# transferia/transferia

Hardware: AMD Instinct MI355X
Metric: ChangeItems/sec through CSV parse -> mask(ClientIP)+filter(EventDate) -> devnull, ClickBench hits, HBM-resident input (the PCIe-inclusive rate is `pcie_inclusive`) (higher is better)
Workload: dtype u8; 1 GPU; ClickBench hits-1M CSV parse -> mask(ip)+filter(EventDate) -> devnull (BASELINE.json configs[1]); columns=105, parallelism=row-range shard x1, no collective, rows_per_pass=1048576, csv_bytes_per_pass=838371857

## Files before the change

transferia_amd/csrc/tf_common.hpp:

```cpp
#pragma once
#include <hip/hip_runtime.h>

#include <cstdint>
#include <cstdio>
#include <cstring>
#include <memory>
#include <mutex>
#include <unordered_map>
#include <stdexcept>
#include <string>
#include <vector>

#include "../../include/tfgpu.h"

#ifndef TF_DYNAMIC_LDS
#define TF_DYNAMIC_LDS(type, name) extern __shared__ type name[]
#endif

#ifndef TF_GLOBAL_PTR
#define TF_GLOBAL_PTR(T, p) ((T *)(__attribute__((address_space(1))) T *)(p))
#endif

#ifndef TF_LOAD16_STREAM
__device__ __forceinline__ uint4 tf_load16_stream(const void *p) {
  typedef uint32_t v4u __attribute__((ext_vector_type(4)));
  const v4u t = __builtin_nontemporal_load(reinterpret_cast<const v4u *>(p));
  return make_uint4(t[0], t[1], t[2], t[3]);
}
#define TF_LOAD16_STREAM(p) tf_load16_stream(p)
#endif

#ifndef TF_CONST_PTR
#define TF_CONST_PTR(T, p) ((const __attribute__((address_space(4))) T *)(p))
#endif

#ifndef TF_KEEP
#define TF_KEEP(x) asm volatile("" ::"v"(x))
#endif
#ifndef TF_OPAQUE
#define TF_OPAQUE(x) asm volatile("" : "+v"(x))
#endif

struct tfgpu_dbatch;

namespace tf {

struct Error : std::runtime_error {
  int code;
  Error(int c, const std::string &m) : std::runtime_error(m), code(c) {}
};
void set_last_error(const std::string &m);
int fail(int code, const std::string &m);

#define TF_HIP(expr)                                                                              \
  do {                                                                                            \
    hipError_t e__ = (expr);                                                                      \
    if (e__ != hipSuccess)                                                                        \
      throw ::tf::Error(TFGPU_ERR_DEVICE, std::string(#expr) + ": " + hipGetErrorString(e__));    \
  } while (0)

struct ProfEntry {
  std::string name;
  int64_t launches = 0;
  double total_ms = 0;
  int64_t units = 0;
};

struct BlockCache {
  std::mutex mu;
  std::unordered_map<size_t, std::vector<void *>> free_;
  size_t cached = 0;
  void *get(size_t cls);
  void put(void *p, size_t cls);
  void trim();
};

struct Context {
  int device = -1;
  hipStream_t stream = nullptr;
  hipStream_t copy_stream = nullptr;
  BlockCache blocks;
  void *pin_base = nullptr;
  size_t pin_cap = 0, pin_off = 0;
  void *pin(size_t bytes);
  template <class T> T *pin_n(size_t n) { return reinterpret_cast<T *>(pin(n * sizeof(T))); }
  bool prof_on = false;
  std::vector<ProfEntry> prof;
  struct Pending { int idx; hipEvent_t a, b; int64_t units = 0; };
  std::vector<Pending> pending;
  std::vector<hipEvent_t> free_events;
  hipEvent_t dense_event = nullptr;
  std::mutex mu;
  int num_cus = 256;
  std::shared_ptr<struct DevMem> pow10tab;
  struct ConstEntry { uint64_t hash; std::vector<uint8_t> bytes; std::shared_ptr<struct DevMem> mem; uint64_t stamp; };
  std::vector<ConstEntry> consts;
  uint64_t const_clock = 0;
  double csv_hint_bpl = 0.0;
  int csv_hint_ncols = -1;

  hipEvent_t get_event();
  void prof_begin(const char *name, Pending &p);
  void prof_end(Pending &p);
  void prof_flush();
};
Context &ctx();
int bind_lane(int lane);
int current_lane();
int lane_device(int lane);
struct LaneScope {
  int prev;
  explicit LaneScope(int lane) : prev(bind_lane(lane)) {}
  ~LaneScope() { try { bind_lane(prev); } catch (...) {} }
};

struct KernelTimer {
  Context::Pending p{-1, nullptr, nullptr};
  bool on;
  explicit KernelTimer(const char *name, int64_t units = 0) : on(ctx().prof_on) { if (on) { ctx().prof_begin(name, p); p.units = units; } }
  ~KernelTimer() { if (on) ctx().prof_end(p); }
};

struct DevMem {
  void *p = nullptr;
  size_t bytes = 0, cls = 0;
  std::shared_ptr<DevMem> parent;
  struct BlockCache *owner = nullptr;
  int device = -1;
  explicit DevMem(size_t n);
  DevMem(std::shared_ptr<DevMem> owner, size_t off, size_t n);
  ~DevMem();
  DevMem(const DevMem &) = delete;
  DevMem &operator=(const DevMem &) = delete;
};
using Buf = std::shared_ptr<DevMem>;
Buf dalloc(size_t bytes);
Buf subbuf(const Buf &owner, size_t off, size_t bytes);
Buf dalloc_zero(size_t bytes);
template <class T> inline T *ptr(const Buf &b) { return b ? reinterpret_cast<T *>(b->p) : nullptr; }

void h2d(void *dst, const void *src, size_t n);
void h2d_small(void *dst, const void *src, size_t n);
Buf upload_small(const void *src, size_t n);
void dbatch_drop_src_row(struct ::tfgpu_dbatch *b);
Buf upload_const(const void *src, size_t n);
const uint32_t *d2h_u32(const void *dev, size_t n = 1);
struct PinScope { PinScope() {} };
void d2h(void *dst, const void *src, size_t n);
void d2d(void *dst, const void *src, size_t n);
void sync();

inline bool repr_is_var(int r) { return r == TFGPU_R_STRING || r == TFGPU_R_BYTES || r == TFGPU_R_JSONNUM || r == TFGPU_R_JSON; }
// ... 34 lines not shown
void ensure_text_offsets(const struct ::tfgpu_dbatch &b);
void dense(const struct ::tfgpu_dbatch *b, bool absent_ok = false);
void dense_locked(const struct ::tfgpu_dbatch &b);
int lanes_created();
uint64_t lane_generation();
std::unique_ptr<struct ::tfgpu_dbatch> snapshot(const struct ::tfgpu_dbatch &b);
bool has_absent(const struct ::tfgpu_dbatch &b);
Buf validity_minus_absent(const Buf &validity, const Buf &absent, int64_t nrows);
Buf find_device_block(const void *p);
void register_device_block(const Buf &b);

}

namespace tf {
struct PendingRows {
  std::shared_ptr<const struct ::tfgpu_dbatch> src;
  Buf sel;
};
}

struct tfgpu_dbatch {
  int64_t nrows = 0;
  std::vector<tf::DColumn> cols;
  std::shared_ptr<tf::PendingRows> pending;
  void *dense_done = nullptr;
  int dense_lane = -1;
  uint64_t dense_gen = 0;
  std::vector<tf::DColumn> replaced;
  std::vector<std::pair<std::string, int>> schema;
  std::vector<std::string> key_names;
  std::vector<tf::DColumn> old_keys;
  tf::Buf old_present;
  std::string ns, table;
  tf::Buf kind, src_row, part_id;
  tf::Buf col_order;
};

struct tfgpu_dbuf {
  tf::Buf mem;
  uint64_t size = 0;
};

namespace tf {
inline std::unique_ptr<tfgpu_dbatch> shallow_copy(const tfgpu_dbatch &in) { return std::make_unique<tfgpu_dbatch>(in); }
template <class F> void materialize_where(const tfgpu_dbatch &b, F pred) {
  std::vector<const DColumn *> need;
  for (auto &c : b.cols) if (pred(c)) need.push_back(&c);
  materialize(b, &need);
}
void exclusive_scan_u32(const uint32_t *in, uint32_t *out, int64_t n, bool with_total);
void exclusive_scan_u32_segments(uint32_t *inout, int64_t seg_len, int nseg, int64_t seg_stride);
void exclusive_scan_u32_segments(const uint32_t *in, uint32_t *out, int64_t seg_len, int nseg, int64_t seg_stride);
bool select_kept_u32(const uint32_t *keep, int64_t n, int32_t *sel, uint32_t *count);
const uint32_t *any_nonzero_to_host(const uint32_t *v, int64_t n);
const uint32_t *segment_totals_to_host(const uint32_t *scanned, int64_t seg_len, int nseg, int64_t seg_stride);
void sum_u32_segments_u64(const uint32_t *in, int64_t seg_len, int nseg, int64_t seg_stride, unsigned long long *totals);

}
```

transferia_amd/csrc/tf_csv.hip:

```cpp
#include <algorithm>
#include <cmath>
#include <cstdio>
#include <type_traits>

#include "tf_devfmt.hpp"
#include "tf_devparse.hpp"
#include "tf_devfloat.hpp"
#include "tf_segcopy.hpp"
#include "tf_textview.hpp"
#include "tf_wave.hpp"
#include "tf_swar.hpp"
#include "tf_gotime.hpp"
#include "tf_f64range.hpp"
#include "tf_plan.hpp"
#include "tf_strictcell.hpp"

#ifdef TF_CSV_ABLATE_BUILD
#define CSV_ABL(x) ((x).ablate)
#else
#define CSV_ABL(x) 0
#endif
namespace tf {

std::unique_ptr<tfgpu_dbatch> compact_rows(const tfgpu_dbatch &in, Buf keep);
// ... 74 lines not shown
  const int lane = threadIdx.x & 63, wv = threadIdx.x >> 6;
  for (int it = 0; it < NL_ITERS; it++) {
    uint64_t pos = tile + ((uint64_t)it * NL_THREADS + threadIdx.x) * 16;
    uint32_t m = pos < len ? nl_mask16(load16_guard(data, pos, len)) : 0;
    uint32_t c = __popc(m), inc = c;
    for (int d = 1; d < 64; d <<= 1) { uint32_t t = __shfl_up(inc, d, 64); if (lane >= d) inc += t; }
    if (lane == 63) wsum[wv] = inc;
    __syncthreads();
    uint32_t wbase = 0, tot = 0;
    for (int i = 0; i < NL_THREADS / 64; i++) { uint32_t s = wsum[i]; if (i < wv) wbase += s; tot += s; }
    __syncthreads();
    uint32_t k = base + wbase + inc - c;
    while (m) { int b = __ffs(m) - 1; m &= m - 1; row_start[++k] = (uint32_t)(pos + b + 1); }
    base += tot;
  }
}


template <class F> __device__ __forceinline__ uint32_t space_prefix(const F &f, uint32_t i, uint32_t end) {
  uint32_t c = f[i];
  if (c == ' ' || (c >= 9 && c <= 13)) return 1;
  if (c < 0xC2) return 0;
  uint32_t r = end - i;
  if (c == 0xC2 && r >= 2) { uint32_t d = f[i + 1]; return (d == 0x85 || d == 0xA0) ? 2 : 0; }
  if (r >= 3 && (c == 0xE1 || c == 0xE2 || c == 0xE3)) {
    uint32_t d = f[i + 1], e = f[i + 2];
    if (c == 0xE1) return (d == 0x9A && e == 0x80) ? 3 : 0;
    if (c == 0xE3) return (d == 0x80 && e == 0x80) ? 3 : 0;
    if (d == 0x80 && ((e >= 0x80 && e <= 0x8A) || e == 0xA8 || e == 0xA9 || e == 0xAF)) return 3;
    if (d == 0x81 && e == 0x9F) return 3;
  }
  return 0;
}
template <class F> __device__ __forceinline__ uint32_t space_suffix(const F &f, uint32_t a, uint32_t b) {
  uint32_t c = f[b - 1];
  if (c == ' ' || (c >= 9 && c <= 13)) return 1;
  if (c < 0x80) return 0;
  if (b - a >= 2 && f[b - 2] == 0xC2 && (c == 0x85 || c == 0xA0)) return 2;
  if (b - a >= 3 && space_prefix(f, b - 3, b) == 3) return 3;
  return 0;
}

struct CsvOpts {
  uint8_t delim, quote, escape, double_quote, include_missing, strings_can_be_null, quoted_strings_can_be_null, pad;
  int32_t n_null, n_true, n_false;
  const uint32_t *list_off;
  const uint8_t *list_data;
  GtSet user_tp;
  GtSet cast_tp;
  const uint8_t *dp;
  uint32_t dp_len;
  uint32_t multiline;
  const uint64_t *p128;
};

__device__ __forceinline__ bool any_quote(const uint32_t *qmask, uint32_t lo, uint32_t hi) {
  if (lo >= hi) return false;
  const uint32_t w0 = lo >> 5, w1 = (hi - 1) >> 5;
  for (uint32_t w = w0; w <= w1; w++) {
    uint32_t m = qmask[w];
    if (w == w0) m &= ~0u << (lo & 31);
    if (w == w1) m &= ~0u >> (31 - ((hi - 1) & 31));
    if (m) return true;
  }
  return false;
}

template <class F> __device__ __forceinline__ int sanitize(const CsvOpts &o, const F &f, uint32_t &a, uint32_t &b, uint32_t &npairs,
                                                           const uint32_t *qmask = nullptr, uint32_t qbase = 0) {
  a = 0; b = f.n; npairs = 0;
  uint32_t k;
  while (a < b && (k = space_prefix(f, a, b)) > 0) a += k;
  while (a < b && (k = space_suffix(f, a, b)) > 0) b -= k;
  if (o.quote == 0) return 0;
  if (b - a >= 1) {
    if (b - a == 1 && f[a] == o.quote) return TFGPU_ROW_QUOTE;
    if (f[a] == o.quote && f[b - 1] == o.quote) { a++; b--; }
  }
  if (qmask && !any_quote(qmask, qbase + a, qbase + b)) return 0;
  for (uint32_t i = a; i + 1 < b;) {
    if (f[i] == o.quote && f[i + 1] == o.quote) { npairs++; i += 2; } else i++;
  }
  if (!o.double_quote && npairs) return TFGPU_ROW_DOUBLE_QUOTE;
  return 0;
}

template <class F> __device__ __forceinline__ bool field_equals(const F &f, uint32_t a, uint32_t b, const uint8_t *s, uint32_t n) {
  if (b - a != n) return false;
  for (uint32_t i = 0; i < n; i++) if (f[a + i] != s[i]) return false;
  return true;
}
template <class F> __device__ __forceinline__ bool in_list(const CsvOpts &o, int first, int count, const F &f, uint32_t a, uint32_t b) {
  for (int i = 0; i < count; i++) {
    uint32_t s = o.list_off[first + i], e = o.list_off[first + i + 1];
    if (field_equals(f, a, b, o.list_data + s, e - s)) return true;
  }
  return false;
}

enum CsvKind : int32_t { CK_INT = SK_INT, CK_UINT = SK_UINT, CK_STR = SK_STR, CK_JSONNUM = SK_JSONNUM, CK_DATE = SK_TIME, CK_TIMESTAMP, CK_BOOL = SK_BOOL, CK_F32 = SK_F32, CK_DEFAULT,
                         CK_INTERVAL = SK_INTERVAL, CK_SYS  };
static_assert(CK_TIMESTAMP == 5 && CK_DEFAULT == 8 && CK_SYS == 10, "the tile kernels sort columns by these values");

struct CsvCol {
  int32_t field;
  int32_t kind;
  int32_t width;
  int32_t next;
  int64_t lo; uint64_t hi;
  void *values;
  int32_t *nanos;
  uint32_t *lens;
  uint32_t *fstart;
  uint32_t *patch;
};
static constexpr uint32_t PATCH_NONE = 0xFFFFFFFFu;

struct TCol {
  void *p0;
  void *p1;
  int16_t field;
  uint8_t kind;
  uint8_t width;
  int32_t ci;
};
static_assert(sizeof(TCol) == 24, "TCol is staged as three 8-byte words");

struct CsvParams {
  const uint8_t *data;
  uint64_t len;
  const uint32_t *row_start;
  const uint32_t *row_end;
  int64_t nrows;
  CsvOpts o;
  const CsvCol *cols;
  int32_t ncols;
  const int32_t *field_first;
  int32_t nfields_used;
  int32_t has_unmapped;
  const TCol *tcols;
  unsigned long long *dbg_phase;
  int32_t null_checks;
  uint8_t *err;
  int32_t *err_col;
  uint32_t *nerr;
  const uint32_t *gran_pre;
  int64_t ngran;
  uint32_t tile_bytes;
  int64_t ntiles;
  int64_t skip_rows;
  uint32_t *slow_n;
  uint32_t *slow_row;
  uint32_t *slow_end;
  uint32_t *last_end;
  int32_t ablate;
  uint32_t *gen_n;
  uint32_t *gen_tile;
  int32_t force_general;
  const struct CsvRun *runs;
  int32_t nruns;
  const struct CsvTask *tasks;
  const int32_t *wave_task;
  int32_t col_lanes;
  uint8_t *arena;
  const uint32_t *lcols;
  const uint32_t *lwave_ncols;
  uint32_t tile_cpt;
  uint32_t *spec;
  uint32_t cap_lines;
  uint32_t *ovf;
};

static constexpr uint32_t SP_AGG = 1u << 30, SP_INC = 2u << 30, SP_VAL = (1u << 30) - 1u;
__device__ __forceinline__ uint32_t spec_lookback(uint32_t *state, int64_t t, uint32_t own, int lane) {
  if (t == 0) { if (lane == 0) __atomic_store_n(&state[0], SP_INC | own, __ATOMIC_RELAXED); return 0u; }
  if (lane == 0) __atomic_store_n(&state[t], SP_AGG | own, __ATOMIC_RELAXED);
  uint32_t excl = 0;
  int64_t base = t - 1;
  for (;;) {
    const int64_t idx = base - lane;
    const uint32_t w = idx >= 0 ? __atomic_load_n(&state[idx], __ATOMIC_RELAXED) : SP_INC;
    const uint64_t inc = __ballot((w >> 30) == 2u), empty = __ballot((w >> 30) == 0u);
    const int fi = inc ? __ffsll((long long)inc) - 1 : 63;
    const uint64_t need = fi == 63 ? ~0ull : ((2ull << fi) - 1ull);
    if (empty & need) { __builtin_amdgcn_s_sleep(1); continue; }
    uint32_t v = lane <= fi ? (w & SP_VAL) : 0u;
    v = wave_scan_add(v);
    excl += (uint32_t)__shfl((int)v, 63, 64);
    if (inc) break;
    base -= 64;
  }
  if (lane == 0) __atomic_store_n(&state[t], SP_INC | ((excl + own) & SP_VAL), __ATOMIC_RELAXED);
  return excl;
}

__device__ __forceinline__ StrictOut strict_out(const CsvCol &c, int32_t kind) { return StrictOut{kind, c.width, c.lo, c.hi, c.values, c.nanos}; }
__device__ __forceinline__ void store_int(const CsvCol &c, int64_t r, int64_t v) { store_int(strict_out(c, c.kind), r, v); }

__device__ __forceinline__ void store_default(const CsvCol &c, int64_t r) {
  switch (c.kind) {
    case CK_SYS: break;
    case CK_STR: case CK_JSONNUM: c.lens[r] = (c.kind == CK_JSONNUM) ? 1u : 0u; c.fstart[r] = 0x7FFFFFFFu; if (c.kind == CK_JSONNUM) c.fstart[-1] = 1u; break;
    case CK_DATE: case CK_TIMESTAMP: store_default(strict_out(c, SK_TIME), r); break;
    default: store_default(strict_out(c, c.kind), r);
  }
}

template <class F>
__device__ __forceinline__ bool cell_is_null(const CsvOpts &o, const F &fv, uint32_t a, uint32_t b, uint32_t npairs) {
  if (o.quoted_strings_can_be_null) {
    uint32_t ta = a, tb = b;
    if (tb > ta && ((fv[ta] == '"' && fv[tb - 1] == '"') || (fv[ta] == '\'' && fv[tb - 1] == '\''))) { ta++; tb = tb > ta ? tb - 1 : ta; }
    return npairs == 0 && in_list(o, 0, o.n_null, fv, ta, tb);
  }
  if (o.strings_can_be_null) return npairs == 0 && in_list(o, 0, o.n_null, fv, a, b);
  return false;
}

template <class F> struct Patched {
  const F &f; uint32_t a, k, skip;
  __device__ __forceinline__ uint32_t operator[](uint32_t i) const { return i < k ? f[a + i] : i == k ? (uint32_t)'.' : f[a + i + skip - 1]; }
};
template <class T> __device__ int parsefloat_err(const T &t, uint32_t n) {
  if (n == 0) return 1;
  uint32_t p = 0;
  if (t[0] == '+' || t[0] == '-') p = 1;
  const uint32_t w = n - p;
  auto word = [&](const char *s, uint32_t l) { if (w != l) return false; for (uint32_t i = 0; i < l; i++) if (lower_(t[p + i]) != (uint32_t)s[i]) return false; return true; };
  if (word("inf", 3) || word("infinity", 8)) return 0;
  if (p == 0 && word("nan", 3)) return 0;
  for (uint32_t i = p; i < n; i++) if (t[i] == '_') return 2;
  if (w >= 2 && t[p] == '0' && lower_(t[p + 1]) == 'x') return 2;
  uint32_t nd = 0;
  while (p < n && dg(t[p])) { nd++; p++; }
  if (p < n && t[p] == '.') { p++; while (p < n && dg(t[p])) { nd++; p++; } }
  if (!nd) return 1;
  if (p < n && lower_(t[p]) == 'e') {
    p++;
    if (p < n && (t[p] == '+' || t[p] == '-')) p++;
    if (p >= n || !dg(t[p])) return 1;
    while (p < n && dg(t[p])) p++;
  }
  if (p != n) return 1;
  return jsonnum_overflow(t, n) ? 1 : 0;
}

template <class F>
__device__ int parse_cell(const CsvOpts &o, const CsvCol &c, int64_t r, const F &fv, uint32_t a, uint32_t b, uint32_t npairs, uint64_t abs_start) {
  switch (c.kind) {
    case CK_INT: case CK_UINT: case CK_INTERVAL:
      if (cell_is_null(o, fv, a, b, npairs)) { store_default(c, r); return 0; }
      if (npairs) return TFGPU_ROW_CAST;
      return strict_cell(strict_out(c, c.kind), o.cast_tp, o.p128, r, fv, a, b);
    case CK_STR: case CK_JSONNUM: {
      if (c.kind == CK_STR && cell_is_null(o, fv, a, b, npairs)) { c.lens[r] = 0; c.fstart[r] = 0x7FFFFFFFu; return 0; }
      if (c.kind == CK_JSONNUM && o.dp_len && !npairs && b - a >= o.dp_len) {
        uint32_t k = PATCH_NONE;
        for (uint32_t i = a; i + o.dp_len <= b && k == PATCH_NONE; i++) {
          bool eq = true;
          for (uint32_t j = 0; j < o.dp_len && eq; j++) eq = fv[i + j] == o.dp[j];
          if (eq) k = i - a;
        }
        if (k != PATCH_NONE) {
          const Patched<F> pt{fv, a, k, o.dp_len};
          const uint32_t pn = (b - a) - o.dp_len + 1;
          const int pe = parsefloat_err(pt, pn);
          if (pe == 2) return TFGPU_ROW_HOST_FALLBACK;
          if (pe == 0) {
            struct View { const Patched<F> &t; __device__ uint32_t operator[](uint32_t i) const { return t[i]; } } v{pt};
            if (!json_number_ok(v, 0, pn)) return TFGPU_ROW_CAST;
            c.lens[r] = pn; c.fstart[r] = (uint32_t)(abs_start + a); c.patch[r] = k;
            return 0;
          }
        }
      }
      if (c.kind == CK_JSONNUM && (npairs || !json_number_ok(fv, a, b))) return TFGPU_ROW_CAST;
      c.lens[r] = (b - a) - npairs;
      c.fstart[r] = (uint32_t)(abs_start + a) | (npairs ? 0x80000000u : 0u);
      if (npairs) c.fstart[-1] = 1u;
      return 0;
    }
    case CK_DATE: case CK_TIMESTAMP: {
      if (npairs) return TFGPU_ROW_CAST;
      int64_t sec = 0; int32_t ns = 0;
      if (c.kind == CK_TIMESTAMP ? parse_int64(fv, a, b, false, &sec) == 0
                                 : (o.user_tp.n && gotime_parse_any(o.user_tp, fv, a, b, &sec, &ns))) {
        ((int64_t *)c.values)[r] = sec;
        c.nanos[r] = ns;
        return 0;
      }
      return strict_cell(strict_out(c, SK_TIME), o.cast_tp, o.p128, r, fv, a, b);
    }
    case CK_BOOL: {
      int v;
      if (npairs) return TFGPU_ROW_CAST;
      if (o.strings_can_be_null && in_list(o, 0, o.n_null, fv, a, b)) v = 0;
      else if (in_list(o, o.n_null, o.n_true, fv, a, b)) v = 1;
      else if (in_list(o, o.n_null + o.n_true, o.n_false, fv, a, b)) v = 0;
      else return strict_cell(strict_out(c, c.kind), o.cast_tp, o.p128, r, fv, a, b);
      ((uint8_t *)c.values)[r] = (uint8_t)v;
      return 0;
    }
    case CK_F32: {
      if (npairs) return TFGPU_ROW_CAST;
      if (o.dp_len && b - a >= o.dp_len) {
        uint32_t k = PATCH_NONE;
        for (uint32_t i = a; i + o.dp_len <= b && k == PATCH_NONE; i++) {
          bool eq = true;
          for (uint32_t j = 0; j < o.dp_len && eq; j++) eq = fv[i + j] == o.dp[j];
          if (eq) k = i - a;
        }
        if (k != PATCH_NONE) {
          const Patched<F> pt{fv, a, k, o.dp_len};
          const uint32_t pn = (b - a) - o.dp_len + 1;
          const int pe = parsefloat_err(pt, pn);
          if (pe == 2) return TFGPU_ROW_HOST_FALLBACK;
          if (pe == 0) return strict_cell(strict_out(c, c.kind), o.cast_tp, o.p128, r, pt, 0, pn);
        }
      }
      return strict_cell(strict_out(c, c.kind), o.cast_tp, o.p128, r, fv, a, b);
    }
    default:
      return TFGPU_ROW_HOST_FALLBACK;
  }
}

__device__ void parse_line_hbm(const CsvParams &p, const bool have_row, const int64_t r, uint64_t pos, const uint64_t end ) {
  const uint64_t row0 = pos;
  MemBytes scan(p.data), fld(p.data);
  const CsvOpts &o = p.o;
  int rerr = 0, rerr_col = -1, miss_col = 0x7FFFFFFF, cerr = 0, cerr_col = 0x7FFFFFFF;
  const bool nil_line = have_row && (end - pos) <= 1;
  if (have_row && o.quote == 0) {
    for (uint64_t q = pos; q < end; q++) if (scan.at(q) == '"') { rerr = TFGPU_ROW_QUOTING_DISABLED; rerr_col = -1; break; }
  }
  if (have_row && o.multiline) {
    for (uint64_t q = pos; q + 2 < end; q++) if (scan.at(q) == '\n' && scan.at(q + 1) == '\n') { rerr = TFGPU_ROW_HOST_FALLBACK; rerr_col = -1; break; }
  }
  bool active = have_row && !nil_line;
  bool in_quotes = false; uint32_t prev = 0xFFFFFFFFu;
  int32_t nfields = 0;
  bool seen_delim = false;
  for (int32_t f = 0;; f++) {
    uint64_t fs = pos, fe = pos; bool last = false;
    if (active) {
      while (true) {
        if (pos >= end) { last = true; fe = end; break; }
        uint32_t ch = scan.at(pos);
        if (o.escape != 0 && prev == o.escape && in_quotes) { prev = ch; pos++; continue; }
        if (o.quote != 0 && ch == o.quote) { in_quotes = !in_quotes; prev = ch; pos++; continue; }
        if (ch == o.delim && !in_quotes) { fe = pos; pos++; seen_delim = true; prev = ch; break; }
        prev = ch; pos++;
      }
      if (last && !seen_delim) fs = row0 + 1 <= end ? row0 + 1 : end;
    }
    const bool has_field = active;
    if (!__any(has_field) && f >= p.nfields_used) break;
    Field fv{&fld, fs, (uint32_t)(fe - fs)};
    uint32_t a = 0, b = 0, npairs = 0;
    const int32_t first_col = f < p.nfields_used ? p.field_first[f] : -1;
    if (has_field) {
      int e = sanitize(o, fv, a, b, npairs);
      if (e && !rerr) { rerr = e; rerr_col = first_col; }
      nfields = f + 1;
    }
    for (int32_t ci = first_col; ci >= 0; ci = p.cols[ci].next) {
      const CsvCol &c = p.cols[ci];
      if (!have_row || rerr) continue;
      if (!has_field) {
        if (o.include_missing) store_default(c, r); else if (ci < miss_col) miss_col = ci;
        continue;
      }
      int err = parse_cell(o, c, r, fv, a, b, npairs, fs);
      if (err && ci < cerr_col) { cerr = err; cerr_col = ci; }
    }
    if (last) active = false;
  }
  if (!have_row) return;
  if (!rerr) {
    for (int32_t ci = 0; ci < p.ncols; ci++) {
      const CsvCol &c = p.cols[ci];
      if (c.field < 0) { store_default(c, r); continue; }
      if (c.field >= nfields) {
        if (c.field < p.nfields_used && !nil_line) continue;
        if (o.include_missing) store_default(c, r); else { if (ci < miss_col) miss_col = ci; break; }
      }
    }
  }
  int err = rerr, err_col = rerr_col;
  if (!err && miss_col != 0x7FFFFFFF) { err = TFGPU_ROW_MISSING_CELL; err_col = miss_col; }
  if (!err && cerr) { err = cerr; err_col = cerr_col; }
  p.err[r] = (uint8_t)err;
  if (err) { p.err_col[r] = err_col; atomicAdd(p.nerr, 1u); }
}

__global__ void __launch_bounds__(256) csv_parse_rows(CsvParams p) {
  const int64_t r = (int64_t)blockIdx.x * blockDim.x + threadIdx.x;
  const bool have_row = r < p.nrows;
  parse_line_hbm(p, have_row, r, have_row ? p.row_start[r] : 0, have_row ? (p.row_end ? p.row_end[r] : p.row_start[r + 1]) : 0);
}

__global__ void __launch_bounds__(64) csv_parse_listed(CsvParams p) {
  const uint32_t n = *p.slow_n;
  for (uint64_t base = (uint64_t)blockIdx.x * 64; base < n; base += (uint64_t)gridDim.x * 64) {
    const uint64_t i = base + threadIdx.x;
    const int64_t line = i < n ? (int64_t)p.slow_row[i] : -1;
    const bool have_row = i < n && line >= p.skip_rows;
    uint64_t end = 0, pos = 0;
    if (have_row) {
      end = (uint64_t)p.slow_end[i] + 1;
      pos = end - 1;
      MemBytes back(p.data);
      while (pos > 0 && back.at(pos - 1) != '\n') pos--;
    }
    parse_line_hbm(p, have_row, line - p.skip_rows, pos, end);
  }
}

#ifndef TF_CT_THREADS
#define TF_CT_THREADS 512
#endif
static constexpr int CT_THREADS = TF_CT_THREADS;
static constexpr uint32_t CT_WAVES = CT_THREADS / 64;
static_assert((CT_WAVES & (CT_WAVES - 1)) == 0, "wave count must be a power of two");
static constexpr int CT_T = NL_TILE;
static constexpr int CT_SPILL = 4096;
static constexpr int CT_BYTES = CT_T + CT_SPILL;
static constexpr int CT_CPT = CT_BYTES / 16 / CT_THREADS;
static constexpr int CT_FCAP = 4096;
static constexpr int CT_RCAP = 256;
static constexpr int CT_LCOLS = 192;
static_assert(CT_CPT * 16 * CT_THREADS == CT_BYTES, "tile must divide evenly");
static_assert(CT_BYTES <= 32768, "positions are 15-bit");

__device__ __forceinline__ bool starts_plain(const uint8_t *sb, uint32_t a, uint32_t end, uint32_t c, uint32_t quote) {
  if (c < 0x80) return c > 0x20 && c != 0x7F && c != quote;
  if (c != 0xC2 && c != 0xE1 && c != 0xE2 && c != 0xE3) return true;
  const uint32_t d = a + 1 < end ? sb[a + 1] : 0u, e = a + 2 < end ? sb[a + 2] : 0u;
  if (c == 0xC2) return !(d == 0x85 || d == 0xA0);
  if (c == 0xE1) return !(d == 0x9A && e == 0x80);
  if (c == 0xE3) return !(d == 0x80 && e == 0x80);
  return !((d == 0x80 && ((e >= 0x80 && e <= 0x8A) || e == 0xA8 || e == 0xA9 || e == 0xAF)) || (d == 0x81 && e == 0x9F));
}
__device__ __forceinline__ bool ends_plain(const uint8_t *sb, uint32_t a, uint32_t b, uint32_t c, uint32_t quote) {
  if (c < 0x80) return c > 0x20 && c != 0x7F && c != quote;
  if (c >= 0xC0) return true;
  const uint32_t d = b - a >= 2 ? sb[b - 2] : 0u, e = b - a >= 3 ? sb[b - 3] : 0u;
  if (d == 0xC2) return !(c == 0x85 || c == 0xA0);
  if (e == 0xE1) return !(d == 0x9A && c == 0x80);
  if (e == 0xE3) return !(d == 0x80 && c == 0x80);
  if (e == 0xE2) return !((d == 0x80 && ((c >= 0x80 && c <= 0x8A) || c == 0xA8 || c == 0xA9 || c == 0xAF)) || (d == 0x81 && c == 0x9F));
  return true;
}
__device__ __forceinline__ uint32_t count_quote_pairs(const uint32_t *qmask, uint32_t lo, uint32_t hi) {
  if (lo >= hi) return 0;
  uint32_t pairs = 0, prev = 0xFFFFFFF0u;
// ... 239 lines not shown
        }
      }
    }
    for (uint32_t i = tid; i < nr; i += CT_THREADS) slowf[i] = 0;
    __syncthreads();
    }
    if (CSV_ABL(p) == 3) { if (fpos[tid] == 0xFFFF && rowend[0] == 0xFFFF) p.err[0] = 1; return; }

    uint32_t next_bstart;
    if (skip_first) {
      uint32_t k = k_thread;
#pragma unroll
      for (int q = 0; q < CT_CPT; q++) {
        uint32_t m = fe[q];
        const int cpos = (base_chunk + q) * 16;
        while (m) {
          const int b = __ffs((int)m) - 1; m &= m - 1;
          if (k == kend) {
            fpos[0] = (uint16_t)(cpos + b);
            uint32_t slot = atomicAdd(p.slow_n, 1u);
            p.slow_row[slot] = line0 + jb;
            p.slow_end[slot] = (uint32_t)(g0 + cpos + b);
          }
          k++;
        }
      }
      __syncthreads();
      next_bstart = (uint32_t)fpos[0] + 1;
    } else {
      for (uint32_t jj = tid; jj < nr; jj += CT_THREADS) {
        const uint32_t k0 = jj ? (uint32_t)rowend[jj - 1] + 1 : kb, ke = rowend[jj];
        const uint32_t row_start = jj ? (uint32_t)(fpos[k0 - 1 - kb] & 0x7FFFu) + 1 : bstart;
        const uint32_t nl_pos = fpos[ke - kb] & 0x7FFFu;
        const uint32_t nf = (nl_pos == row_start) ? 0u : ke - k0 + 1;
        rinfo[jj] = (uint64_t)(k0 - kb) | ((uint64_t)nf << 16) | ((uint64_t)row_start << 32);
      }
      __syncthreads();
      const uint32_t total = (uint32_t)p.ncols * nr;
      const uint32_t inv_nr = nr > 1 ? 0xFFFFFFFFu / nr + 1 : 0;
      for (uint32_t it = tid; it < total; it += CT_THREADS) {
        uint32_t oi = nr > 1 ? __umulhi(it, inv_nr) : it;
        uint32_t jj = it - oi * nr;
        if (jj >= nr) { oi++; jj -= nr; }
        const int64_t r = (int64_t)line0 + jb + jj - p.skip_rows;
        if (r < 0) continue;
        TCol tc;
        if (cols_in_lds) { const uint64_t *q = tcol_lds + oi * 3; tc.p0 = (void *)q[0]; tc.p1 = (void *)q[1]; uint64_t m = q[2]; tc.field = (int16_t)m; tc.kind = (uint8_t)(m >> 16); tc.width = (uint8_t)(m >> 24); tc.ci = (int32_t)(m >> 32); }
        else tc = p.tcols[oi];
        const uint64_t ri = rinfo[jj];
        const uint32_t k0r = (uint32_t)ri & 0xFFFFu, nf = (uint32_t)(ri >> 16) & 0xFFFFu, row_start = (uint32_t)(ri >> 32);
        if (tc.field < 0 || (uint32_t)tc.field >= nf) {
          if (tc.field < 0 || o.include_missing) {
            CsvCol c{}; c.kind = tc.kind; c.width = tc.width; c.values = tc.p0; c.nanos = (int32_t *)tc.p1; c.lens = (uint32_t *)tc.p0; c.fstart = (uint32_t *)tc.p1;
            store_default(c, r);
          } else slowf[jj] = 1;
          continue;
        }
        const uint32_t kr = k0r + (uint32_t)tc.field;
        uint32_t fs = tc.field ? (uint32_t)(fpos[kr - 1] & 0x7FFFu) + 1 : row_start;
        const uint32_t fend = fpos[kr] & 0x7FFFu;
        if (nf == 1) fs = row_start + 1;
        const uint32_t n = fend - fs;
        if (CSV_ABL(p) == 6) { if (n == 0x7FFF) p.err[0] = 1; continue; }
        bool done = false;
        if (n == 0) {
          if (tc.kind == CK_STR) { ((uint32_t *)tc.p0)[r] = 0; ((uint32_t *)tc.p1)[r] = (uint32_t)(g0 + fs); done = true; }
        } else {
          const uint32_t sh = (fs & 7u) * 8;
          const uint64_t *w = reinterpret_cast<const uint64_t *>(sb + (fs & ~7u));
          const uint64_t w0 = w[0], w1 = w[1];
          const uint64_t b0 = sh ? (w0 >> sh) | (w1 << (64 - sh)) : w0;
          const uint32_t c_first = (uint32_t)b0 & 0xFFu, c_last = sb[fend - 1];
          if (tc.kind == CK_STR) {
            uint32_t a = fs, b = fend;
            bool ok = false;
            if (c_first == o.quote && c_last == o.quote && n >= 2) { a++; b--; ok = true; }
            else ok = c_first != o.quote && c_last != o.quote && starts_plain(sb, fs, fend, c_first, o.quote) && ends_plain(sb, fs, fend, c_last, o.quote);
            if (ok) {
              const uint32_t npairs = any_quote(qmask, a, b) ? count_quote_pairs(qmask, a, b) : 0u;
              if (!(npairs && !o.double_quote)) {
                ((uint32_t *)tc.p0)[r] = (b - a) - npairs;
                ((uint32_t *)tc.p1)[r] = (uint32_t)(g0 + a) | (npairs ? 0x80000000u : 0u);
                if (npairs) ((uint32_t *)tc.p1)[-1] = 1u;
                done = true;
              }
            }
          } else if (tc.kind == CK_INT || tc.kind == CK_UINT) {
            if (n <= 20) {
              const bool neg = c_first == '-';
              const uint32_t i0 = (c_first == '-' || c_first == '+') ? 1u : 0u;
              const uint32_t nd = n - i0;
              bool ok = nd >= 1 && nd <= 19 && !(nd > 1 && ((uint32_t)(b0 >> (8 * i0)) & 0xFFu) == '0');
              if (tc.kind == CK_UINT && tc.width == 8 && i0) ok = false;
              uint64_t b1 = 0, b2 = 0;
              if (__any(n > 8)) { const uint64_t w2 = w[2]; b1 = sh ? (w1 >> sh) | (w2 << (64 - sh)) : w1; if (__any(n > 16)) { const uint64_t w3 = w[3]; b2 = sh ? (w2 >> sh) | (w3 << (64 - sh)) : w2; } }
              uint64_t v;
              ok = digits_u64(b0, b1, b2, i0, n, &v) && ok;
              const int bits = tc.width * 8;
              if (tc.kind == CK_INT) ok = ok && v <= (neg ? (1ull << (bits - 1)) : (1ull << (bits - 1)) - 1);
              else ok = ok && !(neg && v != 0) && (tc.width == 8 || v <= (1ull << bits) - 1);
              if (ok && CSV_ABL(p) != 5) {
                const int64_t sv = neg ? (int64_t)(0 - v) : (int64_t)v;
                switch (tc.width) {
                  case 1: ((int8_t *)tc.p0)[r] = (int8_t)sv; break;
                  case 2: ((int16_t *)tc.p0)[r] = (int16_t)sv; break;
                  case 4: ((int32_t *)tc.p0)[r] = (int32_t)sv; break;
                  default: ((int64_t *)tc.p0)[r] = sv;
                }
              }
              done = ok;
            }
          } else if (tc.kind == CK_DATE || tc.kind == CK_TIMESTAMP) {
            const uint64_t w2 = w[2], w3 = w[3];
            const uint64_t b1 = sh ? (w1 >> sh) | (w2 << (64 - sh)) : w1, b2 = sh ? (w2 >> sh) | (w3 << (64 - sh)) : w2;
            const uint32_t i0 = (c_first == '-' || c_first == '+') ? 1u : 0u;
            uint64_t v = 0;
            if (tc.kind == CK_TIMESTAMP && n - i0 >= 1 && n - i0 <= 18 && digits_u64(b0, b1, b2, i0, n, &v)) {
              ((int64_t *)tc.p0)[r] = c_first == '-' ? -(int64_t)v : (int64_t)v; ((int32_t *)tc.p1)[r] = 0; done = true;
            } else if (n == 10 || n == 19) {
              bool ok = true;
              const uint32_t y = two_digits(b0, 0, &ok) * 100 + two_digits(b0, 2, &ok);
              const uint32_t mo = two_digits(b0, 5, &ok), d = two_digits(b1, 0, &ok);
              ok = ok && (((uint32_t)(b0 >> 32) & 0xFFu) == '-') && (((uint32_t)(b0 >> 56) & 0xFFu) == '-');
              uint32_t h = 0, mi = 0, se = 0;
              if (n == 19) {
                const uint32_t sep = (uint32_t)(b1 >> 16) & 0xFFu;
                ok = ok && (sep == ' ' || sep == 'T') && (((uint32_t)(b1 >> 40) & 0xFFu) == ':') && (((uint32_t)b2 & 0xFFu) == ':');
                h = two_digits(b1, 3, &ok); mi = two_digits(b1, 6, &ok); se = two_digits(b2, 1, &ok);
              }
              ok = ok && mo >= 1 && mo <= 12 && d >= 1 && d <= (uint32_t)dev::days_in_month((int)mo, (int64_t)y) && h <= 23 && mi <= 59 && se <= 59;
              if (ok) {
                ((int64_t *)tc.p0)[r] = dev::days_from_civil((int64_t)y, (int)mo, (int)d) * 86400 + h * 3600 + mi * 60 + se;
                ((int32_t *)tc.p1)[r] = 0;
                done = true;
              }
            }
// ... 16 lines not shown
          const uint32_t fend = fpos[kk] & 0x7FFFu;
          if (fend > fs && !(starts_plain(sb, fs, fend, sb[fs], o.quote) && ends_plain(sb, fs, fend, sb[fend - 1], o.quote) && !any_quote(qmask, fs, fend))) slowf[jj] = 1;
        }
      }
      __syncthreads();
      for (uint32_t jj = tid; jj < nr; jj += CT_THREADS) {
        const int64_t r = (int64_t)line0 + jb + jj - p.skip_rows;
        if (r < 0) continue;
        if (slowf[jj] || p.null_checks) {
          const uint32_t slot = atomicAdd(p.slow_n, 1u);
          p.slow_row[slot] = line0 + jb + jj;
          p.slow_end[slot] = (uint32_t)(g0 + (fpos[rowend[jj] - kb] & 0x7FFFu));
        } else p.err[r] = 0;
      }
      next_bstart = (uint32_t)(fpos[kend - kb] & 0x7FFFu) + 1;
    }
    __syncthreads();
    bstart = next_bstart;
    jb += nr; kb = kend + 1;
  }
  if (tid == 0) {
    atomicMax(p.last_end, (uint32_t)(g0 + bstart));
    if (p.spec) p.spec[2 + p.ntiles + gstart / (CT_T / CSV_GRAN)] = (uint32_t)(g0 + bstart);
  }
}

__global__ void __launch_bounds__(CT_THREADS, 6) csv_parse_tiles_general(CsvParams p) {
  const uint32_t n = *p.gen_n;
  for (uint32_t i = blockIdx.x; i < n; i += gridDim.x) {
    const bool sp = p.spec != nullptr;
    const uint32_t *e = p.gen_tile + (size_t)(sp ? 4 : 2) * i;
    parse_tile_general(p, (int64_t)e[0], (int64_t)e[1], sp ? e[2] : 0u, sp ? e[3] : 0u);
    __syncthreads();
  }
}

__device__ __forceinline__ int32_t days_from_civil32(uint32_t y, uint32_t m, uint32_t d) {
  const uint32_t yy = y + 400u - (m <= 2 ? 1u : 0u);
  const uint32_t era = yy / 400u, yoe = yy - era * 400u;
  const uint32_t doy = (153u * (m > 2 ? m - 3 : m + 9) + 2u) / 5u + d - 1u;
  const uint32_t doe = yoe * 365u + yoe / 4u - yoe / 100u + doy;
  return (int32_t)(era * 146097u + doe) - 719468 - 146097;
}
__device__ __forceinline__ uint32_t days_in_month32(uint32_t m, uint32_t y) {
  const uint32_t leap = ((y & 3u) == 0 && (y % 100u != 0 || y % 400u == 0)) ? 1u : 0u;
  return m == 2 ? 28u + leap : 30u + ((0x15AAu >> m) & 1u);
}

#ifndef TF_CR_FCAP
#define TF_CR_FCAP 4608
#endif
static constexpr int CR_FCAP = TF_CR_FCAP;
static constexpr int CR_LCOLS = 128;
static constexpr uint32_t CR_KDUMMY = CR_FCAP + 2;
struct CsvRun { int32_t kind, width, first, ncols; };
struct CsvTask { int32_t kind, width, first, ncols; };

struct RegTile {
  const uint8_t *sb; const uint16_t *fposx; const uint32_t *qmask; const uint16_t *qpre; const uint2 *keeptab; uint8_t *slowf; const uint64_t *colp0, *colp1; const uint16_t *colfield;
  uint32_t nr, NF, step_q, step_r; float inv_nr; int32_t row0; uint32_t g0; uint32_t quote; bool double_quote; int32_t ablate; int32_t col_mode;
};
struct RegCell { bool on; uint32_t col, jj, fs, fend; int32_t r; };
struct ItemIter { uint32_t it, oi, jj; };
__device__ __forceinline__ ItemIter item_first(const RegTile &t, uint32_t it) {
  uint32_t oi = (uint32_t)(__uint2float_rz(it) * t.inv_nr);
  uint32_t jj = it - __umul24(oi, t.nr);
  if (jj >= t.nr) { oi++; jj -= t.nr; }
  return ItemIter{it, oi, jj};
}
__device__ __forceinline__ void item_next(const RegTile &t, ItemIter &x) {
  x.it += 64u * CT_WAVES; x.oi += t.step_q; x.jj += t.step_r;
  if (x.jj >= t.nr) { x.jj -= t.nr; x.oi++; }
}
__device__ __forceinline__ RegCell reg_cell(const RegTile &t, uint32_t first_col, const ItemIter &x, uint32_t items) {
  RegCell c;
  c.col = first_col + x.oi; c.jj = x.jj;
  c.r = t.row0 + (int32_t)x.jj;
  c.on = x.it < items && c.r >= 0;
  const uint32_t kr = c.on ? __umul24(x.jj, t.NF) + (uint32_t)t.colfield[c.col] : CR_KDUMMY;
  uint32_t kr1 = kr + 1;
  TF_OPAQUE(kr1);
  c.fs = (uint32_t)t.fposx[kr] + 1; c.fend = t.fposx[kr1];
  return c;
}
#ifndef TF_CSV_PREFETCH
#define TF_CSV_PREFETCH 0
#endif
template <class Body> __device__ __forceinline__ void for_slots(const RegTile &t, const CsvRun &run, uint32_t sbase, int wv, int lane, Body body) {
  const uint32_t items = (uint32_t)run.ncols * t.nr, nslots = (items + 63) >> 6, end = sbase + nslots;
  const uint32_t s0 = sbase + (((uint32_t)wv - sbase) & (CT_WAVES - 1u));
  if (s0 >= end) return;
  ItemIter x = item_first(t, (s0 - sbase) * 64 + (uint32_t)lane);
#if TF_CSV_PREFETCH
  RegCell c = reg_cell(t, (uint32_t)run.first, x, items);
  for (uint32_t s = s0; s < end; s += CT_WAVES) {
    RegCell cn = c;
    if (s + CT_WAVES < end) { item_next(t, x); cn = reg_cell(t, (uint32_t)run.first, x, items); }
    body(c);
    c = cn;
  }
#else
  for (uint32_t s = s0; s < end; s += CT_WAVES, item_next(t, x)) body(reg_cell(t, (uint32_t)run.first, x, items));
#endif
}
template <class T> __device__ __forceinline__ T *global_ptr(uint64_t p) { return TF_GLOBAL_PTR(T, p); }
__device__ __forceinline__ uint32_t quotes_in(const RegTile &t, uint32_t a, uint32_t b) {
  const uint32_t ca = (uint32_t)t.qpre[a >> 5] + (uint32_t)__popc(t.qmask[a >> 5] & ((1u << (a & 31)) - 1u));
  const uint32_t cb = (uint32_t)t.qpre[b >> 5] + (uint32_t)__popc(t.qmask[b >> 5] & ((1u << (b & 31)) - 1u));
  return cb - ca;
}

template <int KIND, int W, class T> __device__ __forceinline__ void reg_int_body(const RegTile &t, const RegCell &c, T *const out) {
// ... 22 lines not shown
    const uint2 keep = t.keeptab[c.on ? n : 0u];
    const uint32_t tlo = (wlo ^ 0x30303030u) & keep.x, thi = (whi ^ 0x30303030u) & keep.y;
    bad = (((tlo + 0x76767676u) | tlo | (thi + 0x76767676u) | thi) & 0x80808080u) != 0;
    uint32_t v;
    if constexpr (W < 4) {
      v = __umul24(tlo >> 24, 10000u) + four_dot(thi);
      if constexpr (KIND == CK_INT) bad = bad || v > (1u << (W * 8 - 1)) - 1u; else bad = bad || v > (1u << (W * 8)) - 1u;
    } else v = __umul24(four_dot(tlo), 10000u) + four_dot(thi);
    if (c.on && !bad) out[c.r] = (T)v;
  } else if constexpr (W >= 4) {
    const bool neg = c0 == '-', sgn = neg || c0 == '+';
    const uint32_t nd = n - (sgn ? 1u : 0u);
    const uint32_t fd = sgn ? (uint32_t)t.sb[c.fs + 1] : c0;
    bool ok = nd - 1u < 19u && !(nd > 1 && fd == '0');
    if constexpr (KIND == CK_UINT && W == 8) ok = ok && !sgn;
    const uint32_t y = c.fend;
    const uint32_t *w = reinterpret_cast<const uint32_t *>(t.sb + (int)((y - 24u) & ~3u));
    const uint32_t d0 = w[0], d1 = w[1], d2 = w[2], d3 = w[3], d4 = w[4];
    const uint32_t w2lo = __builtin_amdgcn_alignbyte(d1, d0, y), w2hi = __builtin_amdgcn_alignbyte(d2, d1, y);
    const uint32_t w1lo = __builtin_amdgcn_alignbyte(d3, d2, y), w1hi = __builtin_amdgcn_alignbyte(d4, d3, y);
    const uint32_t ndc = min(nd, 24u), n0 = min(ndc, 8u), n1d = min(ndc - n0, 8u), n2d = min(ndc - n0 - n1d, 8u);
    const uint2 k0 = t.keeptab[n0], k1 = t.keeptab[n1d], k2 = t.keeptab[n2d];
    const uint32_t a0 = (wlo ^ 0x30303030u) & k0.x, b0 = (whi ^ 0x30303030u) & k0.y;
    const uint32_t a1 = (w1lo ^ 0x30303030u) & k1.x, b1 = (w1hi ^ 0x30303030u) & k1.y;
    const uint32_t a2 = (w2lo ^ 0x30303030u) & k2.x, b2 = (w2hi ^ 0x30303030u) & k2.y;
    const uint32_t nondigit = ((a0 + 0x76767676u) | a0 | (b0 + 0x76767676u) | b0 | (a1 + 0x76767676u) | a1 | (b1 + 0x76767676u) | b1 |
                               (a2 + 0x76767676u) | a2 | (b2 + 0x76767676u) | b2) & 0x80808080u;
    ok = ok && nondigit == 0;
    const uint32_t g0v = __umul24(four_dot(a0), 10000u) + four_dot(b0), g1v = __umul24(four_dot(a1), 10000u) + four_dot(b1);
    const uint32_t g2v = __umul24(four_dot(a2), 10000u) + four_dot(b2);
    const uint64_t v = ((uint64_t)g2v * 100000000ull + g1v) * 100000000ull + g0v;
    if constexpr (KIND == CK_INT) ok = ok && v <= (neg ? (1ull << (W * 8 - 1)) : (1ull << (W * 8 - 1)) - 1);
    else ok = ok && !(neg && v != 0) && (W == 8 || v <= (1ull << (W * 8 % 64)) - 1);
    if (c.on && ok) out[c.r] = (T)(neg ? (int64_t)(0 - v) : (int64_t)v);
    bad = !ok;
  } else {
    const bool neg = c0 == '-', sgn = neg || c0 == '+';
    const uint32_t nd = n - (sgn ? 1u : 0u);
    bool ok = nd - 1u < 19u && !(nd > 1 && t.sb[c.fend - min(nd, 24u)] == '0');
    uint32_t g0v = 0;
    ok = digits8_window<true>(wlo, whi, min(nd, 8u), &g0v) && ok;
    if constexpr (KIND == CK_INT) ok = ok && nd <= 5 && g0v <= (1u << (W * 8 - 1)) - (neg ? 0u : 1u);
    else ok = ok && nd <= 5 && g0v <= (1u << (W * 8)) - 1u && !(neg && g0v != 0);
    if (c.on && ok) out[c.r] = (T)(neg ? -(int32_t)g0v : (int32_t)g0v);
    bad = !ok;
  }
  if (c.on && bad) t.slowf[c.jj] = 1;
}
template <int KIND, int W> __device__ __forceinline__ void reg_cells_int(const RegTile &t, const CsvRun &run, uint32_t sbase, int wv, int lane) {
  using T = std::conditional_t<W == 1, int8_t, std::conditional_t<W == 2, int16_t, std::conditional_t<W == 4, int32_t, int64_t>>>;
  for_slots(t, run, sbase, wv, lane, [&](const RegCell &c) { reg_int_body<KIND, W, T>(t, c, global_ptr<T>(t.colp0[c.on ? c.col : (uint32_t)run.first])); });
}

__device__ __forceinline__ void reg_str_body(const RegTile &t, const RegCell &c, uint32_t *const lens, uint32_t *const fstart) {
  const uint32_t n = c.fend - c.fs;
  const uint32_t c_first = t.sb[c.fs], c_last = t.sb[c.fend - 1];
  const uint32_t qn = quotes_in(t, c.fs, c.fend);
  const bool plain = qn == 0 && c_first - 0x21u < 0x5Eu && c_last - 0x21u < 0x5Eu;
  const bool quoted = qn == 2 && c_first == t.quote && c_last == t.quote;
  if (wave_all(n == 0 || plain || quoted || !c.on)) {
    const uint32_t q1 = quoted ? 1u : 0u;
    if (c.on) { lens[c.r] = n - 2u * q1; fstart[c.r] = t.g0 + c.fs + q1; }
    return;
  }
  if (!c.on) return;
  if (n == 0) { lens[c.r] = 0; fstart[c.r] = t.g0 + c.fs; return; }
  bool done = false;
  if (n <= 0x7FFFu) {
    uint32_t a = c.fs, b = c.fend;
    bool ok = false;
    if (c_first == t.quote && c_last == t.quote && n >= 2) { a++; b--; ok = true; }
    else ok = c_first != t.quote && c_last != t.quote && starts_plain(t.sb, c.fs, c.fend, c_first, t.quote) && ends_plain(t.sb, c.fs, c.fend, c_last, t.quote);
    if (ok) {
      const uint32_t npairs = quotes_in(t, a, b) ? count_quote_pairs(t.qmask, a, b) : 0u;
      if (!(npairs && !t.double_quote)) {
        lens[c.r] = (b - a) - npairs;
        fstart[c.r] = (t.g0 + a) | (npairs ? 0x80000000u : 0u);
        if (npairs) fstart[-1] = 1u;
        done = true;
      }
    }
  }
  if (!done) t.slowf[c.jj] = 1;
}
__device__ __forceinline__ void reg_cells_str(const RegTile &t, const CsvRun &run, uint32_t sbase, int wv, int lane) {
  for_slots(t, run, sbase, wv, lane, [&](const RegCell &c) {
    const uint32_t col = c.on ? c.col : (uint32_t)run.first;
    reg_str_body(t, c, global_ptr<uint32_t>(t.colp0[col]), global_ptr<uint32_t>(t.colp1[col]));
  });
}

__device__ __forceinline__ uint32_t dig2(uint32_t w, int byte, uint32_t *bad) {
  const uint32_t a = ((w >> (8 * byte)) & 0xFFu) - '0', b = ((w >> (8 * byte + 8)) & 0xFFu) - '0';
  *bad |= (a > 9u) | (b > 9u);
  return a * 10 + b;
}
template <int KIND> __device__ __forceinline__ void reg_time_body(const RegTile &t, const RegCell &c, int64_t *const sec, int32_t *const nanos) {
  if (!c.on) return;
  const uint32_t n = c.fend - c.fs;
  bool done = false;
  if ((n == 10 || n == 19) && t.sb[c.fs + 4] == '-') {
    const uint32_t *w = reinterpret_cast<const uint32_t *>(t.sb + (c.fs & ~3u));
    const uint32_t x0 = w[0], x1 = w[1], x2 = w[2], x3 = w[3], x4 = w[4], x5 = w[5];
    const uint32_t w0 = __builtin_amdgcn_alignbyte(x1, x0, c.fs), w1 = __builtin_amdgcn_alignbyte(x2, x1, c.fs), w2 = __builtin_amdgcn_alignbyte(x3, x2, c.fs);
    uint32_t bad = 0;
    const uint32_t y = dig2(w0, 0, &bad) * 100 + dig2(w0, 2, &bad);
    const uint32_t mo = dig2(w1, 1, &bad), d = dig2(w2, 0, &bad);
    bad |= (w1 & 0xFF0000FFu) != 0x2D00002Du;
    uint32_t h = 0, mi = 0, se = 0;
    if (n == 19) {
      const uint32_t w3 = __builtin_amdgcn_alignbyte(x4, x3, c.fs), w4 = __builtin_amdgcn_alignbyte(x5, x4, c.fs);
      const uint32_t sep = (w2 >> 16) & 0xFFu;
      bad |= !(sep == ' ' || sep == 'T') | (((w3 >> 8) & 0xFFu) != ':') | ((w4 & 0xFFu) != ':');
      h = (((w2 >> 24) & 0xFFu) - '0') * 10 + ((w3 & 0xFFu) - '0');
      bad |= (((w2 >> 24) & 0xFFu) - '0' > 9u) | ((w3 & 0xFFu) - '0' > 9u);
      mi = dig2(w3, 2, &bad); se = dig2(w4, 1, &bad);
    }
    const bool ok = !bad && mo >= 1 && mo <= 12 && d >= 1 && d <= days_in_month32(mo, y) && h <= 23 && mi <= 59 && se <= 59;
    if (ok) {
      sec[c.r] = (int64_t)days_from_civil32(y, mo, d) * 86400 + (int64_t)(h * 3600 + mi * 60 + se);
      nanos[c.r] = 0;
      done = true;
    }
  } else if (KIND == CK_TIMESTAMP && n - 1u < 19u) {
    const uint32_t c0 = t.sb[c.fs];
    const bool neg = c0 == '-', sgn = neg || c0 == '+';
    const uint32_t nd = n - (sgn ? 1u : 0u);
    uint32_t g0v = 0, g1v = 0, g2v = 0;
    bool ok = nd - 1u < 18u;
    ok = digits8_end(t.sb, c.fend, min(nd, 8u), &g0v) && ok;
    if (nd > 8) ok = digits8_end(t.sb, c.fend - 8, min(nd - 8, 8u), &g1v) && ok;
    if (nd > 16) ok = digits8_end(t.sb, c.fend - 16, nd - 16, &g2v) && ok;
    if (ok) {
      const uint64_t v = ((uint64_t)g2v * 100000000ull + g1v) * 100000000ull + g0v;
      sec[c.r] = neg ? -(int64_t)v : (int64_t)v; nanos[c.r] = 0; done = true;
    }
  }
  if (!done) t.slowf[c.jj] = 1;
}
template <int KIND> __device__ __forceinline__ void reg_cells_time(const RegTile &t, const CsvRun &run, uint32_t sbase, int wv, int lane) {
  for_slots(t, run, sbase, wv, lane, [&](const RegCell &c) {
    if (!c.on) return;
    reg_time_body<KIND>(t, c, global_ptr<int64_t>(t.colp0[c.col]), global_ptr<int32_t>(t.colp1[c.col]));
  });
}

struct LaneCol { uint32_t g, ph, P; bool live; };
__device__ __forceinline__ LaneCol lane_col(const CsvTask &k, int lane, int mode) {
  const uint32_t G = (uint32_t)__builtin_amdgcn_readfirstlane(k.ncols), P = 64u / G;
  if (mode == 2) {
    const uint32_t g = (uint32_t)((uint32_t)lane * (65536u / P + 1u)) >> 16;
    return LaneCol{g, (uint32_t)lane - g * P, P, g < G};
  }
  const uint32_t ph = (uint32_t)((uint32_t)lane * (65536u / G + 1u)) >> 16;
  return LaneCol{(uint32_t)lane - ph * G, ph, P, ph < P};
}
__device__ __forceinline__ RegCell lane_cell(const RegTile &t, const LaneCol &lc, uint32_t jj0, uint32_t colfield) {
  RegCell c;
  c.jj = jj0 + lc.ph; c.col = 0;
  c.r = t.row0 + (int32_t)c.jj;
  c.on = lc.live && c.jj < t.nr && c.r >= 0;
  const uint32_t kr = c.on ? __umul24(c.jj, t.NF) + colfield : CR_KDUMMY;
  uint32_t kr1 = kr + 1;
  TF_OPAQUE(kr1);
  c.fs = (uint32_t)t.fposx[kr] + 1; c.fend = t.fposx[kr1];
  return c;
}
template <int KIND, int W> __device__ __forceinline__ void task_cells_int(const RegTile &t, const CsvTask &k, int lane) {
  using T = std::conditional_t<W == 1, int8_t, std::conditional_t<W == 2, int16_t, std::conditional_t<W == 4, int32_t, int64_t>>>;
  const LaneCol lc = lane_col(k, lane, t.col_mode);
  const uint32_t col = (uint32_t)k.first + (lc.live ? lc.g : 0u);
  const uint32_t colfield = t.colfield[col];
  T *const out = global_ptr<T>(t.colp0[col]);
  for (uint32_t jj0 = 0; jj0 < t.nr; jj0 += lc.P) reg_int_body<KIND, W, T>(t, lane_cell(t, lc, jj0, colfield), out);
}
__device__ __forceinline__ void task_cells_str(const RegTile &t, const CsvTask &k, int lane) {
  const LaneCol lc = lane_col(k, lane, t.col_mode);
  const uint32_t col = (uint32_t)k.first + (lc.live ? lc.g : 0u);
  const uint32_t colfield = t.colfield[col];
  uint32_t *const lens = global_ptr<uint32_t>(t.colp0[col]), *const fstart = global_ptr<uint32_t>(t.colp1[col]);
  for (uint32_t jj0 = 0; jj0 < t.nr; jj0 += lc.P) reg_str_body(t, lane_cell(t, lc, jj0, colfield), lens, fstart);
}
template <int KIND> __device__ __forceinline__ void task_cells_time(const RegTile &t, const CsvTask &k, int lane) {
  const LaneCol lc = lane_col(k, lane, t.col_mode);
  const uint32_t col = (uint32_t)k.first + (lc.live ? lc.g : 0u);
  const uint32_t colfield = t.colfield[col];
  int64_t *const sec = global_ptr<int64_t>(t.colp0[col]); int32_t *const nanos = global_ptr<int32_t>(t.colp1[col]);
  for (uint32_t jj0 = 0; jj0 < t.nr; jj0 += lc.P) reg_time_body<KIND>(t, lane_cell(t, lc, jj0, colfield), sec, nanos);
}
__device__ __forceinline__ bool task_kind(int kind) { return kind == CK_INT || kind == CK_UINT || kind == CK_STR || kind == CK_DATE || kind == CK_TIMESTAMP; }

template <bool COLS> __device__ __forceinline__ void csv_parse_regular_body(const CsvParams &p) {
  static_assert(CT_SPILL == 64 * CT_CPT * 16, "the look-behind window is exactly wave 0's bytes");
  __shared__ __attribute__((aligned(16))) uint8_t sbuf[32 + CT_BYTES + 48];
  __shared__ uint16_t fposx[CR_FCAP + 4];
  __shared__ uint2 keeptab[9];
  __shared__ uint32_t qmask[CT_BYTES / 32];
  __shared__ uint32_t nlbits[(CR_FCAP + 32) / 32];
  __shared__ uint16_t qpre[CT_BYTES / 32 + 2];
  __shared__ uint32_t wqc[CT_THREADS / 64];
  __shared__ uint8_t slowf[CT_RCAP];
  __shared__ uint64_t colp0[CR_LCOLS], colp1[CR_LCOLS];
  __shared__ uint16_t colfield[CR_LCOLS];
  __shared__ uint32_t wpar[CT_THREADS / 64];
  __shared__ uint32_t wcnt[CT_THREADS / 64];
  __shared__ uint32_t misc[4];
  __shared__ uint32_t spec_sh[2];
  uint8_t *const sb = sbuf + 32;
  const int tid = threadIdx.x, lane = tid & 63, wv = tid >> 6;
  const bool spec = p.spec != nullptr;

  int64_t tile;
  if (spec) {
    if (tid == 0) spec_sh[0] = atomicAdd(p.spec, 1u);
    __syncthreads();
    tile = (int64_t)spec_sh[0];
  } else {
    const int64_t per_xcd = (p.ntiles + 7) / 8;
    tile = (int64_t)(blockIdx.x & 7) * per_xcd + (blockIdx.x >> 3);
  }
  if (tile >= p.ntiles) return;
  constexpr int64_t GPT = CT_T / CSV_GRAN;
  const int64_t gr0 = tile * GPT, gr1 = min(gr0 + GPT, p.ngran);
  const auto *gpre = TF_CONST_PTR(uint32_t, p.gran_pre);
  uint32_t line0 = 0, line1 = 0, lines_all = 0, nlines = 0;
  if (!spec) {
    line0 = gpre[gr0]; line1 = gpre[gr1]; lines_all = gpre[p.ngran];
    nlines = line1 - line0;
    if (nlines == 0) return;
    if (p.ovf && line1 > p.cap_lines) { if (tid == 0) *p.ovf = 1u; return; }
  }
  const CsvOpts &o = p.o;
  const int64_t g0 = tile * CT_T - CT_SPILL;
  auto give_up = [&]() {
// ... 125 lines not shown
  {
    const uint32_t cex = cpre + cinc - cnt;
    uint32_t k = cex & 0xFFFFu;
#pragma unroll
    for (int h = 0; h < CT_CPT; h += 2) {
      uint32_t m = fe[h] | (fe[h + 1] << 16);
      const uint32_t nlh = nl[h] | (nl[h + 1] << 16);
      const uint32_t cpos = (uint32_t)(base_chunk + h) * 16;
      if (nlh) {
        uint32_t mm = nlh, j = (cex >> 16) + (h ? (uint32_t)__popc(nl[0] | (nl[1] << 16)) : 0u);
        while (mm) {
          const uint32_t b = (uint32_t)__ffs((int)mm) - 1; mm &= mm - 1;
          const uint32_t kk = k + (uint32_t)__popc(m & ((2u << b) - 1u));
          atomicOr(&nlbits[kk >> 5], 1u << (kk & 31));
          if (j == 0) misc[2] = kk;
          j++;
        }
      }
      while (m) {
        const uint32_t b = (uint32_t)__ffs((int)m) - 1; m &= m - 1;
        fposx[++k] = (uint16_t)(cpos + b);
      }
      if (o.escape != 0) {
        uint32_t mm = qm[h] | (qm[h + 1] << 16);
        while (mm) {
          const uint32_t b = (uint32_t)__ffs((int)mm) - 1; mm &= mm - 1;
          if (sb[(int)(cpos + b) - 1] == o.escape) misc[1] = 1u;
        }
      }
    }
    if (tid == 0) fposx[0] = (uint16_t)(frs - 1);
    for (uint32_t i = tid; i < nr; i += CT_THREADS) slowf[i] = 0;
    uint32_t qb = qinc - qc;
    for (int i = 0; i < wv; i++) qb += wqc[i];
    qpre[tid * 2] = (uint16_t)qb; qpre[tid * 2 + 1] = (uint16_t)(qb + qlo);
    if (tid == CT_THREADS - 1) qpre[CT_BYTES / 32] = (uint16_t)(qb + qc);
  }
  __syncthreads();
  phase(3);
  if (CSV_ABL(p) == 4) return;
  if (spec) {
    line0 = spec_sh[1]; line1 = line0 + nr;
    if (line1 > p.cap_lines) { if (tid == 0) p.spec[1] = 1u; return; }
  }
  const uint32_t NF = misc[2];
  if (NF < 2 || NF < (uint32_t)p.nfields_used || nr * NF > nfe) { give_up(); return; }
  for (uint32_t jj = tid; jj < nr; jj += CT_THREADS) {
    const uint32_t idx = (jj + 1) * NF;
    if (idx > nfe || !((nlbits[idx >> 5] >> (idx & 31)) & 1u)) misc[1] = 1u;
  }

  {
    RegTile t;
    t.sb = sb; t.fposx = fposx; t.qmask = qmask; t.qpre = qpre; t.keeptab = keeptab; t.slowf = slowf; t.colp0 = colp0; t.colp1 = colp1; t.colfield = colfield;
    t.nr = nr; t.NF = NF; t.step_q = 64u * CT_WAVES / nr; t.step_r = 64u * CT_WAVES - t.step_q * nr; t.inv_nr = __uint_as_float(__float_as_uint(1.0f / (float)nr) - 2u);
    t.row0 = (int32_t)((int64_t)line0 - p.skip_rows); t.g0 = (uint32_t)g0; t.quote = o.quote; t.double_quote = o.double_quote != 0; t.ablate = CSV_ABL(p); t.col_mode = p.col_lanes;
    if constexpr (COLS) {
      for (int ti = p.wave_task[wv]; ti < p.wave_task[wv + 1]; ti++) {
        const CsvTask k = p.tasks[ti];
        if (CSV_ABL(p) >= 10) {
          const int grp = (k.kind == CK_INT || k.kind == CK_UINT) ? 11 : k.kind == CK_STR ? 12 : 13;
          if (CSV_ABL(p) != grp && !(CSV_ABL(p) == 31 && grp == 11)) continue;
        }
        switch (k.kind) {
          case CK_INT:
            if (k.width == 1) task_cells_int<CK_INT, 1>(t, k, lane); else if (k.width == 2) task_cells_int<CK_INT, 2>(t, k, lane);
            else if (k.width == 4) task_cells_int<CK_INT, 4>(t, k, lane); else task_cells_int<CK_INT, 8>(t, k, lane);
            break;
          case CK_UINT:
            if (k.width == 1) task_cells_int<CK_UINT, 1>(t, k, lane); else if (k.width == 2) task_cells_int<CK_UINT, 2>(t, k, lane);
            else if (k.width == 4) task_cells_int<CK_UINT, 4>(t, k, lane); else task_cells_int<CK_UINT, 8>(t, k, lane);
            break;
          case CK_STR: task_cells_str(t, k, lane); break;
          case CK_DATE: task_cells_time<CK_DATE>(t, k, lane); break;
          default: task_cells_time<CK_TIMESTAMP>(t, k, lane);
        }
      }
    }
    uint32_t sbase = 0;
    for (int ri = 0; ri < p.nruns; ri++) {
      const CsvRun run = p.runs[ri];
      if (COLS && task_kind(run.kind)) continue;
      const uint32_t items = (uint32_t)run.ncols * nr, nslots = (items + 63) >> 6;
      if (CSV_ABL(p) >= 10) {
        const int grp = (run.kind == CK_INT || run.kind == CK_UINT) ? 11 : run.kind == CK_STR ? 12 : 13;
        if (CSV_ABL(p) != grp && !(CSV_ABL(p) == 31 && grp == 11)) { sbase += nslots; continue; }
      }
      switch (run.kind) {
        case CK_INT:
          if (run.width == 1) reg_cells_int<CK_INT, 1>(t, run, sbase, wv, lane); else if (run.width == 2) reg_cells_int<CK_INT, 2>(t, run, sbase, wv, lane);
          else if (run.width == 4) reg_cells_int<CK_INT, 4>(t, run, sbase, wv, lane); else reg_cells_int<CK_INT, 8>(t, run, sbase, wv, lane);
          break;
        case CK_UINT:
          if (run.width == 1) reg_cells_int<CK_UINT, 1>(t, run, sbase, wv, lane); else if (run.width == 2) reg_cells_int<CK_UINT, 2>(t, run, sbase, wv, lane);
          else if (run.width == 4) reg_cells_int<CK_UINT, 4>(t, run, sbase, wv, lane); else reg_cells_int<CK_UINT, 8>(t, run, sbase, wv, lane);
          break;
        case CK_STR: reg_cells_str(t, run, sbase, wv, lane); break;
        case CK_DATE: reg_cells_time<CK_DATE>(t, run, sbase, wv, lane); break;
        case CK_TIMESTAMP: reg_cells_time<CK_TIMESTAMP>(t, run, sbase, wv, lane); break;
        default:
          for (uint32_t s = sbase + (((uint32_t)wv - sbase) & (CT_WAVES - 1u)); s < sbase + nslots; s += CT_WAVES) {
            const uint32_t it = (s - sbase) * 64 + (uint32_t)lane;
            if (it >= items) continue;
            const uint32_t oi = it / nr, jj = it - oi * nr;
            const int32_t r = t.row0 + (int32_t)jj;
            if (r < 0) continue;
            if (run.kind < 0) {
              const TCol tc = p.tcols[run.first + oi];
              CsvCol c{}; c.kind = tc.kind; c.width = tc.width; c.values = tc.p0; c.nanos = (int32_t *)tc.p1; c.lens = (uint32_t *)tc.p0; c.fstart = (uint32_t *)tc.p1;
              store_default(c, r);
            } else slowf[jj] = 1;
          }
      }
      sbase += nslots;
    }
    if (p.has_unmapped || NF != (uint32_t)p.nfields_used) {
      const uint32_t tot2 = nr * NF;
      const uint32_t inv_nf = 0xFFFFFFFFu / NF + 1;
      for (uint32_t it = tid; it < tot2; it += CT_THREADS) {
        uint32_t jj = __umulhi(it, inv_nf);
        uint32_t f = it - jj * NF;
        if (f >= NF) { jj++; f -= NF; }
        if (t.row0 + (int32_t)jj < 0) continue;
        if (f < (uint32_t)p.nfields_used && p.field_first[f] >= 0) continue;
        const uint32_t fs = (uint32_t)fposx[it] + 1, fend = fposx[it + 1];
        if (fend > fs && !(starts_plain(sb, fs, fend, sb[fs], o.quote) && ends_plain(sb, fs, fend, sb[fend - 1], o.quote) && !any_quote(qmask, fs, fend))) slowf[jj] = 1;
      }
    }
  }
  phase(4);
  __syncthreads();
  phase(5);
  if (misc[1]) { give_up(); return; }
  for (uint32_t jj = tid; jj < nr; jj += CT_THREADS) {
    const int64_t r = (int64_t)line0 + jj - p.skip_rows;
    if (r < 0) continue;
    if (slowf[jj] || p.null_checks) {
      const uint32_t slot = atomicAdd(p.slow_n, 1u);
      p.slow_row[slot] = line0 + jj;
      p.slow_end[slot] = (uint32_t)(g0 + fposx[(jj + 1) * NF]);
    } else p.err[r] = 0;
  }
  if (tid == 0) { if (spec) p.spec[2 + p.ntiles + tile] = (uint32_t)(g0 + fposx[nr * NF] + 1); else if (line1 == lines_all) atomicMax(p.last_end, (uint32_t)(g0 + fposx[nr * NF] + 1)); }
  phase(6);
}

__global__ void __launch_bounds__(CT_THREADS, 6) csv_parse_regular(CsvParams p) { csv_parse_regular_body<false>(p); }
__global__ void __launch_bounds__(CT_THREADS, 6) csv_parse_cols(CsvParams p) { csv_parse_regular_body<true>(p); }

#include "tf_csv_lanes.inc"

__global__ void csv_zero_err_lens(const uint8_t *err, int64_t nrows, const CsvCol *cols, int32_t ncols, const uint32_t *lines_total, int64_t skip) {
  int64_t r = (int64_t)blockIdx.x * blockDim.x + threadIdx.x;
  if (lines_total) nrows = min(nrows, max((int64_t)*lines_total - skip, (int64_t)0));
  if (r >= nrows || !err[r]) return;
  for (int32_t ci = 0; ci < ncols; ci++) if (cols[ci].lens) cols[ci].lens[r] = 0;
}

static constexpr int FS_HDR = 4;
struct CopyCol { const uint32_t *offsets; const uint32_t *fstart; uint8_t *out; int32_t is_jsonnum; const uint32_t *patch; uint32_t dp_len; };
struct CopyParams { const uint8_t *data; int64_t nrows; const CopyCol *cols; int32_t ncols; uint8_t quote; };

__global__ void __launch_bounds__(256) csv_copy_strings(CopyParams p) {
// ... 215 lines not shown
  hipStream_t st = ctx().stream;
  const int64_t ntiles = (int64_t)((len + NL_TILE - 1) / NL_TILE), ngran = (int64_t)((len + CSV_GRAN - 1) / CSV_GRAN);
  uint32_t n = 0;
  Buf tile_counts = dalloc((size_t)(ngran + 1) * 4);
  if (ntiles) {
    { KernelTimer t("csv_count_newlines"); csv_count_newlines<<<(unsigned)ntiles, NL_THREADS, 0, st>>>(data, len, ptr<uint32_t>(tile_counts), ngran); }
    exclusive_scan_u32(ptr<uint32_t>(tile_counts), ptr<uint32_t>(tile_counts), ngran, true);
    const uint32_t *h = d2h_u32(ptr<uint32_t>(tile_counts) + ngran);
    tf::sync();
    n = *h;
  }
  *out = dalloc_zero((size_t)(n + 2) * 4);
  if (n) { KernelTimer t("csv_line_index"); csv_line_index<<<(unsigned)ntiles, NL_THREADS, 0, st>>>(data, len, ptr<uint32_t>(tile_counts), ptr<uint32_t>(*out)); }
  return n;
}

static void materialize_cols(const tfgpu_dbatch &b, const std::vector<const DColumn *> *only, const uint8_t *text) {
  hipStream_t st = ctx().stream;
  const int64_t nrows = b.nrows;
  struct Grp { const uint8_t *src; uint8_t quote; std::vector<CopyCol> all, lng, sht; };
  std::vector<Grp> groups;
  {
    bool need = false;
    auto look = [&](const DColumn &d) { if (d.lens_only() && !(only && std::find(only->begin(), only->end(), &d) == only->end())) need = true; };
    for (auto &d : b.cols) look(d);
    for (auto &d : b.old_keys) look(d);
    if (need) ensure_text_offsets(b);
  }
  auto visit = [&](const DColumn &d) {
    if (!d.lazy()) return;
    if (only && std::find(only->begin(), only->end(), &d) == only->end()) return;
    TextView &v = *d.view;
    const uint8_t *src = text ? text : ptr<uint8_t>(v.src);
    if (!src) throw Error(TFGPU_ERR_INVALID, "internal: text column " + d.name + " lost its source text");
    v.packed = dalloc(d.data_len + 8);
    CopyCol c{ptr<uint32_t>(d.offsets), ptr<uint32_t>(v.fstart), ptr<uint8_t>(v.packed), v.jsonnum ? 1 : 0, nullptr, 0};
    Grp *g = nullptr;
    for (auto &x : groups) if (x.src == src && x.quote == v.quote) g = &x;
    if (!g) { groups.push_back(Grp{src, v.quote, {}, {}, {}}); g = &groups.back(); }
    if (v.has_special) g->all.push_back(c);
    ((d.data_len >= (uint64_t)nrows * 8) ? g->lng : g->sht).push_back(c);
  };
  for (auto &d : b.cols) visit(d);
  for (auto &d : b.old_keys) visit(d);
  if (!nrows) return;
  for (auto &g : groups) {
    Buf ball = upload_small(g.all.data(), g.all.size() * sizeof(CopyCol));
    Buf blng = upload_small(g.lng.data(), g.lng.size() * sizeof(CopyCol)), bsht = upload_small(g.sht.data(), g.sht.size() * sizeof(CopyCol));
    KernelTimer t("csv_copy_words");
    if (!g.lng.empty()) { CopyParams cp{g.src, nrows, ptr<CopyCol>(blng), (int32_t)g.lng.size(), g.quote}; csv_copy_words<1><<<dim3((unsigned)((nrows + 255) / 256), (unsigned)g.lng.size()), 256, 0, st>>>(cp); }
    if (!g.sht.empty()) { CopyParams cp{g.src, nrows, ptr<CopyCol>(bsht), (int32_t)g.sht.size(), g.quote}; csv_copy_cells<<<dim3((unsigned)((nrows + 255) / 256), (unsigned)((g.sht.size() + CC_GROUP - 1) / CC_GROUP)), 256, 0, st>>>(cp); }
    if (!g.all.empty()) {
      CopyParams cp{g.src, nrows, ptr<CopyCol>(ball), (int32_t)g.all.size(), g.quote};
      csv_copy_special<<<dim3((unsigned)((nrows + 255) / 256), (unsigned)g.all.size()), 256, 0, st>>>(cp);
    }
  }
}
void materialize(const tfgpu_dbatch &b, const std::vector<const DColumn *> *only) { materialize_cols(b, only, nullptr); }
static void materialize_from(const tfgpu_dbatch &b, const uint8_t *text) { materialize_cols(b, nullptr, text); }

}

using namespace tf;

#define TF_API_BEGIN try {
#define TF_API_END                                                        \
  }                                                                       \
  catch (const tf::Error &e) { return tf::fail(e.code, e.what()); }       \
  catch (const std::bad_alloc &) { return tf::fail(TFGPU_ERR_NOMEM, "out of host memory"); } \
  catch (const std::exception &e) { return tf::fail(TFGPU_ERR_INVALID, e.what()); }

static inline unsigned blocks_for(int64_t n, int t) { return (unsigned)std::max<int64_t>(1, (n + t - 1) / t); }

namespace tf {
__global__ void __launch_bounds__(256) csv_split_count(const uint8_t *data, const uint32_t *row_start, int64_t nlines, uint32_t *quotes) {
  const int64_t i = (int64_t)blockIdx.x * blockDim.x + threadIdx.x;
  if (i >= nlines) return;
  MemBytes m(data);
  uint32_t c = 0;
  for (uint64_t k = row_start[i]; k < row_start[i + 1]; k++) c += m.at(k) == '"';
  quotes[i] = c;
}
__global__ void __launch_bounds__(256) csv_split_keep(const uint32_t *quotes_excl, const uint32_t *quotes, int64_t nlines, uint32_t *keep) {
  const int64_t i = (int64_t)blockIdx.x * blockDim.x + threadIdx.x;
  if (i < nlines) keep[i] = ((quotes_excl[i] + quotes[i]) & 1u) ? 0u : 1u;
}
__global__ void __launch_bounds__(256) csv_split_scatter(const uint32_t *keep_scan, const uint32_t *row_start, int64_t nlines, uint32_t *out) {
  const int64_t i = (int64_t)blockIdx.x * blockDim.x + threadIdx.x;
  if (i < nlines && keep_scan[i] != keep_scan[i + 1]) out[keep_scan[i]] = row_start[i + 1];
}
}

extern "C" int tfgpu_csv_split_rows(const void *bytes, uint64_t len, int mem, tfgpu_dbuf **row_ends, int64_t *nrows) {
  TF_API_BEGIN
  if (!row_ends || !nrows) return tf::fail(TFGPU_ERR_INVALID, "tfgpu_csv_split_rows: null argument");
  if (len >= 0x7FFFFFF0ull) return tf::fail(TFGPU_ERR_UNSUPPORTED, "tfgpu_csv_split_rows: chunk must be < 2 GiB");
  Context &cx = ctx();
  std::lock_guard<std::mutex> lk(cx.mu);
  hipStream_t st = cx.stream;
  Buf staged;
  const uint8_t *data;
  if (mem == TFGPU_MEM_HOST) {
    staged = dalloc(len + 64);
    h2d(staged->p, bytes, len);
    TF_HIP(hipMemsetAsync((char *)staged->p + len, 0, 64, st));
    data = ptr<uint8_t>(staged);
// ... 164 lines not shown
  auto carve = [&](size_t bytes) { Buf b = subbuf(arena, arena_off, bytes); arena_off += a256(bytes + 64); return b; };
  Buf lens_all = carve((size_t)std::max(nstr, 1) * (size_t)seg_stride * 4 + 16);
  const int64_t fstride = ((std::max<int64_t>(nrows, 1) + 3) / 4) * 4 + FS_HDR;
  Buf fstart_all = carve((size_t)std::max(nstr, 1) * (size_t)fstride * 4);
  int max_field = -1;
  int si = 0;
  std::vector<int> str_col_index;
  std::vector<int> sys_cols;
  for (int i = 0; i < ncols; i++) {
    const tfgpu_colschema &sc = schema->cols[i];
    CsvCol &c = cols[(size_t)i];
    std::memset(&c, 0, sizeof c);
    const std::string cname = sc.name ? sc.name : "";
    const int sys = cname == "__file_name" ? 1 : cname == "__row_index" ? 2 : 0;
    if (sys) {
      c.field = -1; c.next = -1; c.kind = CK_SYS;
      DColumn d;
      d.name = cname; d.dtype = sc.dtype; d.repr = sys == 1 ? TFGPU_R_STRING : TFGPU_R_UINT64;
      sys_cols.push_back(i);
      db->cols.push_back(std::move(d));
      continue;
    }
    const char *path = sc.path ? sc.path : "";
    char *endp = nullptr;
    long idx = std::strtol(path, &endp, 10);
    if (endp == path || *endp) return tf::fail(TFGPU_ERR_CONFIG, std::string("csv: column ") + (sc.name ? sc.name : "") + ": ColSchema.Path is not an integer (strconv.Atoi)");
    c.field = (int32_t)idx; c.next = -1;
    DColumn d;
    d.name = sc.name ? sc.name : ""; d.dtype = sc.dtype;
    StrictOut so{};
    d.repr = strict_describe(sc.dtype, so);
    if (d.repr == TFGPU_R_INVALID) return tf::fail(TFGPU_ERR_CONFIG, "csv: cannot strictify value of unknown type");
    c.kind = sc.dtype == TFGPU_T_TIMESTAMP ? (int32_t)CK_TIMESTAMP : so.kind; c.width = so.width; c.lo = so.lo; c.hi = so.hi;
    if (c.kind == CK_STR || c.kind == CK_JSONNUM) {
      c.lens = ptr<uint32_t>(lens_all) + (int64_t)si * seg_stride;
      c.fstart = ptr<uint32_t>(fstart_all) + (int64_t)si * fstride + FS_HDR;
      str_col_index.push_back(i);
      si++;
    } else {
      d.values = carve((size_t)std::max<int64_t>(nrows, 1) * (size_t)c.width);
      c.values = d.values->p;
      if (d.repr == TFGPU_R_TIME) { d.nanos = carve((size_t)std::max<int64_t>(nrows, 1) * 4); c.nanos = ptr<int32_t>(d.nanos); }
    }
    if (c.field > max_field) max_field = c.field;
    db->cols.push_back(std::move(d));
  }
  std::vector<int32_t> field_first((size_t)std::max(max_field + 1, 1), -1);
  for (int i = ncols - 1; i >= 0; i--) {
    int f = cols[(size_t)i].field;
    if (f < 0) continue;
    cols[(size_t)i].next = field_first[(size_t)f];
    field_first[(size_t)f] = i;
  }
  std::vector<uint32_t> loff{0}; std::string ldata;
  auto add_list = [&](int n, const char *const *v) { for (int i = 0; i < n; i++) { ldata += v[i] ? v[i] : ""; loff.push_back((uint32_t)ldata.size()); } };
  add_list(opts->n_null_values, opts->null_values); add_list(opts->n_true_values, opts->true_values); add_list(opts->n_false_values, opts->false_values);
  auto up = [&](const void *src, size_t bytes) { return upload_const(src, bytes); };
  Buf bcols = up(cols.data(), cols.size() * sizeof(CsvCol)), bff = up(field_first.data(), field_first.size() * 4);
  Buf bloff = up(loff.data(), loff.size() * 4), bldata = up(ldata.data(), ldata.size());
  std::vector<GtOp> gops; std::string glits; std::vector<uint16_t> gstart_user{0}, gstart_cast;
  for (int i = 0; i < opts->n_timestamp_parsers; i++) { gotime_compile(opts->timestamp_parsers[i] ? opts->timestamp_parsers[i] : "", gops, glits); gstart_user.push_back((uint16_t)gops.size()); }
  append_cast_layouts(gops, glits, gstart_cast);
  Buf bgops = up(gops.data(), gops.size() * sizeof(GtOp)), bglits = up(glits.data(), glits.size());
  Buf bgsu = up(gstart_user.data(), gstart_user.size() * 2), bgsc = up(gstart_cast.data(), gstart_cast.size() * 2), bdp = up(dp.data(), dp.size());
  Buf patch_all;
  if (!dp.empty()) {
    int nf = 0;
    for (auto &c : cols) if (c.kind == CK_JSONNUM) nf++;
    patch_all = dalloc((size_t)std::max(nf, 1) * (size_t)std::max<int64_t>(nrows, 1) * 4);
    TF_HIP(hipMemsetAsync(patch_all->p, 0xFF, patch_all->bytes, st));
    int k = 0;
    for (auto &c : cols) if (c.kind == CK_JSONNUM) c.patch = ptr<uint32_t>(patch_all) + (size_t)(k++) * (size_t)std::max<int64_t>(nrows, 1);
    bcols = up(cols.data(), cols.size() * sizeof(CsvCol));
  }
  Buf err = dalloc((size_t)nrows + 16), err_col = dalloc((size_t)nrows * 4 + 16), nerr = dalloc(4);

  const int64_t slow_cap = (int64_t)nlines + 5 * (ngran + 1) + 8;
  Buf slow = dalloc((size_t)(2 * slow_cap + 2) * 4);
  Buf gen = dalloc((size_t)(4 * (ngran + 2) + 2) * 4);
  const uint32_t tile_bytes = CT_T;
  const int64_t rtiles = (int64_t)((len + tile_bytes - 1) / tile_bytes);
  Buf spec_state;
  if (spec) { spec_state = dalloc((size_t)(2 * rtiles + 2) * 4); TF_HIP(hipMemsetAsync(spec_state->p, 0, (size_t)(2 * rtiles + 2) * 4, st)); }
  CsvParams pp;
  std::memset(&pp, 0, sizeof pp);
  pp.data = data; pp.len = len; pp.row_start = rs; pp.nrows = nrows;
  pp.row_end = multiline ? ptr<uint32_t>(ml_end) + skip : nullptr;
  pp.gran_pre = ptr<uint32_t>(tile_counts); pp.ngran = ngran; pp.tile_bytes = tile_bytes; pp.ntiles = rtiles; pp.skip_rows = skip;
  pp.slow_n = ptr<uint32_t>(slow); pp.last_end = ptr<uint32_t>(slow) + 1;
  pp.slow_row = ptr<uint32_t>(slow) + 2; pp.slow_end = ptr<uint32_t>(slow) + 2 + slow_cap;
  pp.o.delim = opts->delimiter; pp.o.quote = opts->quote_char; pp.o.escape = opts->escape_char; pp.o.double_quote = opts->double_quote;
  pp.o.include_missing = opts->include_missing_columns; pp.o.strings_can_be_null = opts->strings_can_be_null;
  pp.o.quoted_strings_can_be_null = opts->quoted_strings_can_be_null; pp.o.pad = 0;
  pp.o.n_null = opts->n_null_values; pp.o.n_true = opts->n_true_values; pp.o.n_false = opts->n_false_values;
  pp.o.list_off = ptr<uint32_t>(bloff); pp.o.list_data = ptr<uint8_t>(bldata);
  pp.o.user_tp = GtSet{ptr<GtOp>(bgops), ptr<uint8_t>(bglits), ptr<uint16_t>(bgsu), opts->n_timestamp_parsers};
  pp.o.cast_tp = GtSet{ptr<GtOp>(bgops), ptr<uint8_t>(bglits), ptr<uint16_t>(bgsc), N_CAST_LAYOUTS};
  pp.o.dp = ptr<uint8_t>(bdp); pp.o.dp_len = (uint32_t)dp.size(); pp.o.multiline = multiline ? 1u : 0u;
  pp.o.p128 = nullptr;
  for (auto &c : cols) if (c.kind == CK_F32) pp.o.p128 = reinterpret_cast<const uint64_t *>(pow10_table() + 632);
  pp.cols = ptr<CsvCol>(bcols); pp.ncols = ncols; pp.field_first = ptr<int32_t>(bff); pp.nfields_used = max_field + 1;
  pp.err = ptr<uint8_t>(err); pp.err_col = ptr<int32_t>(err_col); pp.nerr = ptr<uint32_t>(nerr);
#ifdef TF_CSV_ABLATE_BUILD
  static const int ablate = [] { const char *e = std::getenv("TFGPU_CSV_ABLATE"); return e ? std::atoi(e) : 0; }();
#else
  static const int ablate = [] { const char *e = std::getenv("TFGPU_CSV_ABLATE"); if (e && std::atoi(e)) std::fprintf(stderr, "tfgpu: TFGPU_CSV_ABLATE needs the ablate build of tf_csv.hip (tools/build_variant.sh ablate tf_csv.hip -DTF_CSV_ABLATE_BUILD=1); ignored\n"); return 0; }();
#endif
  pp.ablate = ablate;
  static const bool force_general = [] { const char *e = std::getenv("TFGPU_CSV_GENERAL"); return e && e[0] == '1'; }();
  pp.gen_n = ptr<uint32_t>(gen); pp.gen_tile = ptr<uint32_t>(gen) + 1; pp.force_general = force_general ? 1 : 0;
  pp.spec = spec ? ptr<uint32_t>(spec_state) : nullptr; pp.cap_lines = cap_lines;
  Buf ahead_ovf;
  if (ahead) { ahead_ovf = dalloc(4); pp.ovf = ptr<uint32_t>(ahead_ovf); }
  csv_zero_flags<<<1, 64, 0, st>>>(ptr<uint32_t>(fstart_all), fstride, nstr, ptr<uint32_t>(slow), ptr<uint32_t>(gen), ptr<uint32_t>(nerr), pp.ovf);
  pp.has_unmapped = 0;
  for (int f = 0; f <= max_field; f++) if (field_first[(size_t)f] < 0) pp.has_unmapped = 1;
  std::vector<int32_t> order((size_t)ncols);
  for (int i = 0; i < ncols; i++) order[(size_t)i] = i;
  std::stable_sort(order.begin(), order.end(), [&](int x, int y) {
    const CsvCol &a = cols[(size_t)x], &b = cols[(size_t)y];
    return a.kind != b.kind ? a.kind < b.kind : a.width != b.width ? a.width < b.width : a.field < b.field;
  });
  std::vector<TCol> tcols((size_t)ncols);
  for (int i = 0; i < ncols; i++) {
    const CsvCol &c = cols[(size_t)order[(size_t)i]];
    TCol &t = tcols[(size_t)i];
    const bool text = c.kind == CK_STR || c.kind == CK_JSONNUM;
    t.p0 = text ? (void *)c.lens : c.values; t.p1 = text ? (void *)c.fstart : (void *)c.nanos;
    if (c.field > 32767) return tf::fail(TFGPU_ERR_UNSUPPORTED, "csv: ColSchema.Path above 32767");
    t.field = (int16_t)c.field; t.kind = (uint8_t)c.kind; t.width = (uint8_t)c.width; t.ci = order[(size_t)i];
  }
  Buf btcols = up(tcols.data(), tcols.size() * sizeof(TCol));
  pp.tcols = ptr<TCol>(btcols);
  static const bool phases = [] { const char *e = std::getenv("TFGPU_CSV_PHASES"); return e && e[0] == '1'; }();
  Buf bphase;
  if (phases) { bphase = dalloc_zero(8 * 8); pp.dbg_phase = ptr<unsigned long long>(bphase); }
  std::vector<CsvRun> runs;
  for (int i = 0; i < ncols; i++) {
    const TCol &t = tcols[(size_t)i];
    const int kind = t.field < 0 ? -1 : (int)t.kind, width = t.field < 0 ? 0 : (int)t.width;
    if (!runs.empty() && runs.back().kind == kind && runs.back().width == width && runs.back().first + runs.back().ncols == i) runs.back().ncols++;
    else runs.push_back(CsvRun{kind, width, i, 1});
  }
  Buf bruns = up(runs.data(), runs.size() * sizeof(CsvRun));
  pp.runs = ptr<CsvRun>(bruns); pp.nruns = (int32_t)runs.size();
  static const int col_lanes = [] { const char *e = std::getenv("TFGPU_CSV_COL_LANES"); return e ? std::atoi(e) : 0; }();
  std::vector<CsvTask> tasks; std::vector<int32_t> wave_task(CT_THREADS / 64 + 1, 0);
  if (col_lanes) {
    struct Pending { CsvTask k; int cost; };
    std::vector<Pending> pend;
    for (auto &r : runs) {
      if (!(r.kind == CK_INT || r.kind == CK_UINT || r.kind == CK_STR || r.kind == CK_DATE || r.kind == CK_TIMESTAMP)) continue;
      const int unit = (r.kind == CK_INT || r.kind == CK_UINT) ? (r.width == 8 ? 5 : r.width == 4 ? 3 : 2) : r.kind == CK_STR ? 4 : 6;
      static const int piece = [] { const char *e = std::getenv("TFGPU_CSV_COL_PIECE"); return e ? std::max(1, std::min(64, std::atoi(e))) : 16; }();
      const int pieces = r.ncols <= piece + piece / 3 ? 1 : (r.ncols + piece - 1) / piece;
      for (int q = 0, at = 0; q < pieces; q++) {
        const int n = (r.ncols - at + (pieces - q) - 1) / (pieces - q);
        pend.push_back({CsvTask{r.kind, r.width, r.first + at, n}, n * unit});
        at += n;
      }
    }
    std::stable_sort(pend.begin(), pend.end(), [](const Pending &a, const Pending &b) { return a.cost > b.cost; });
    const int nw = CT_THREADS / 64;
    std::vector<int> load((size_t)nw, 0); std::vector<std::vector<CsvTask>> per((size_t)nw);
    for (auto &q : pend) { int w = 0; for (int i = 1; i < nw; i++) if (load[(size_t)i] < load[(size_t)w]) w = i; load[(size_t)w] += q.cost; per[(size_t)w].push_back(q.k); }
    for (int w = 0; w < nw; w++) { wave_task[(size_t)w] = (int32_t)tasks.size(); for (auto &k : per[(size_t)w]) tasks.push_back(k); }
    wave_task[(size_t)nw] = (int32_t)tasks.size();
  }
  if (tasks.empty()) tasks.push_back(CsvTask{0, 0, 0, 1});
  Buf btasks = up(tasks.data(), std::max<size_t>(tasks.size(), 1) * sizeof(CsvTask)), bwt = up(wave_task.data(), wave_task.size() * 4);
  pp.tasks = ptr<CsvTask>(btasks); pp.wave_task = ptr<int32_t>(bwt); pp.col_lanes = col_lanes;
  pp.null_checks = (opts->strings_can_be_null || opts->quoted_strings_can_be_null) ? 1 : 0;

  static const bool lanes_on = [] { const char *e = std::getenv("TFGPU_CSV_LANES"); return e && e[0] == '1'; }();
  bool use_lanes = lanes_on && !rowpath && ncols <= CL_MAXCOLS && nlines > 0;
// ... 8 lines not shown
    for (int w = 0; w < CL_WAVES && ci < ncols; w++) {
      const int share = (total - spent + (CL_WAVES - w) - 1) / (CL_WAVES - w);
      int got = 0, s = 0;
      while (ci < ncols && s < CL_WCOLS && (s == 0 || got + cost(tcols[(size_t)ci]) <= share || ncols - ci > (CL_WAVES - w - 1) * CL_WCOLS)) {
        const TCol &t = tcols[(size_t)ci];
        const uint64_t o0 = t.p0 ? (uint64_t)((uint8_t *)t.p0 - (uint8_t *)arena->p) : 0, o1 = t.p1 ? (uint64_t)((uint8_t *)t.p1 - (uint8_t *)arena->p) : 0;
        if ((o0 | o1) & 3) { use_lanes = false; break; }
        lcols[(size_t)w * 64 + 4 * s] = (uint32_t)(o0 >> 2); lcols[(size_t)w * 64 + 4 * s + 1] = (uint32_t)(o1 >> 2);
        lcols[(size_t)w * 64 + 4 * s + 2] = (uint32_t)(uint16_t)t.field | ((uint32_t)t.kind << 16) | ((uint32_t)t.width << 24);
        got += cost(t); s++; ci++;
      }
      lwn[(size_t)w] = (uint32_t)s; spent += got;
    }
    if (ci < ncols) use_lanes = false;
    if (use_lanes) {
      const double avg_row = (double)len / (double)nlines, nf_est = std::max<double>(max_field + 1, 1);
      uint32_t cpt = 1;
      for (uint32_t c = CL_CPT_MAX; c >= 1; c--) {
        const double lines = cl_tile(c) / avg_row;
        if (lines * nf_est <= 0.88 * CL_FCAP && lines <= 0.88 * CL_RCAP) { cpt = c; break; }
      }
      pp.tile_cpt = cpt;
      ltiles = (int64_t)((len + cl_tile(cpt) - 1) / cl_tile(cpt));
      pp.ntiles = ltiles;
      pp.arena = (uint8_t *)arena->p;
      blcols = up(lcols.data(), lcols.size() * 4); blwn = up(lwn.data(), lwn.size() * 4);
      pp.lcols = ptr<uint32_t>(blcols); pp.lwave_ncols = ptr<uint32_t>(blwn);
    }
  }

  if (ablate) {
    TF_HIP(hipMemsetAsync(lens_all->p, 0, (size_t)std::max(nstr, 1) * (size_t)seg_stride * 4, st));
    TF_HIP(hipMemsetAsync(fstart_all->p, 0, (size_t)std::max(nstr, 1) * (size_t)fstride * 4, st));
    TF_HIP(hipMemsetAsync(err->p, 0, (size_t)nrows + 16, st));
    for (auto &d : db->cols) { if (d.values) TF_HIP(hipMemsetAsync(d.values->p, 0, d.values->bytes, st)); if (d.nanos) TF_HIP(hipMemsetAsync(d.nanos->p, 0, d.nanos->bytes, st)); }
  }
  if (nrows && rowpath) {
    KernelTimer t("csv_parse_rows");
    csv_parse_rows<<<blocks_for(nrows, 256), 256, 0, st>>>(pp);
  } else if (nlines) {
    if (use_lanes) {
      const int64_t per_xcd = (ltiles + 7) / 8;
      KernelTimer t("csv_parse_lanes");
      csv_parse_lanes<<<(unsigned)(per_xcd * 8), CL_THREADS, 0, st>>>(pp);
    } else {
      const int64_t per_xcd = (rtiles + 7) / 8;
      KernelTimer t("csv_parse_regular");
      if (pp.col_lanes) csv_parse_cols<<<(unsigned)(spec ? rtiles : per_xcd * 8), CT_THREADS, 0, st>>>(pp);
      else csv_parse_regular<<<(unsigned)(spec ? rtiles : per_xcd * 8), CT_THREADS, 0, st>>>(pp);
    }
    { KernelTimer t("csv_parse_tiles_general"); csv_parse_tiles_general<<<(unsigned)std::min<int64_t>(ntiles + rtiles, 2048), CT_THREADS, 0, st>>>(pp); }
    { KernelTimer t("csv_parse_listed"); csv_parse_listed<<<(unsigned)std::min<int64_t>(blocks_for(slow_cap, 64), 1024), 64, 0, st>>>(pp); }
  }
  Buf src_block = staged ? staged : find_device_block(data);
  static const bool force_eager = [] { const char *e = std::getenv("TFGPU_CSV_EAGER"); return e && e[0] == '1'; }();
  static const bool scan_eager = [] { const char *e = std::getenv("TFGPU_CSV_SCAN_EAGER"); return e && e[0] == '1'; }();
  const bool lens_state = !rowpath && src_block && !force_eager && !scan_eager;
  if (lens_state) {
  } else if (nrows && nstr) {
    csv_zero_err_lens<<<blocks_for(nrows, 256), 256, 0, st>>>(ptr<uint8_t>(err), nrows, ptr<CsvCol>(bcols), ncols, ahead ? ptr<uint32_t>(tile_counts) + ngran : nullptr, skip);
    exclusive_scan_u32_segments(ptr<uint32_t>(lens_all), nrows, nstr, seg_stride);
  } else if (nstr) {
    TF_HIP(hipMemsetAsync(lens_all->p, 0, (size_t)nstr * (size_t)seg_stride * 4, st));
  }
  Buf summary = dalloc((size_t)(2 * nstr + 4) * 4);
  csv_collect<<<1, 64, 0, st>>>(ptr<uint32_t>(nerr), rowpath ? ptr<uint32_t>(row_start) + nlines : pp.last_end, lens_state ? nullptr : ptr<uint32_t>(lens_all),
                                seg_stride, nrows, nstr, ptr<uint32_t>(fstart_all), fstride, ptr<uint32_t>(summary), pp.spec, rtiles, skip,
                                ptr<uint32_t>(tile_counts) + (spec ? 0 : ngran), pp.ovf);
  const uint32_t *hsum = d2h_u32(summary->p, (size_t)(2 * nstr) + 4);
  tf::sync();
  const uint32_t hnerr = hsum[0], last = hsum[1];
  if (spec || ahead) {
    const uint32_t nl_true = hsum[2 + 2 * nstr], overflow = hsum[3 + 2 * nstr];
    if (overflow || nl_true > cap_lines || (int64_t)nl_true < skip || (nl_true && !last)) { *retry = true; return TFGPU_OK; }
    nlines = nl_true; nlogical = nl_true; nrows = (int64_t)nl_true - skip;
    db->nrows = nrows;
  }
  if (!rowpath && nlines >= 16 && last) { cx.csv_hint_bpl = (double)last / (double)nlines; cx.csv_hint_ncols = schema->ncols; }
  if (phases && !rowpath) {
    unsigned long long ph[8]; d2h(ph, bphase->p, sizeof ph); tf::sync();
    std::fprintf(stderr, "tfgpu csv phases (s_memtime ticks per workgroup, %lld tiles): stage %.0f classify %.0f fields %.0f index %.0f cells(wave 0) %.0f cells-barrier %.0f epilogue %.0f\n", (long long)rtiles,
                 (double)ph[0] / rtiles, (double)ph[1] / rtiles, (double)ph[2] / rtiles, (double)ph[3] / rtiles, (double)ph[4] / rtiles, (double)ph[5] / rtiles, (double)ph[6] / rtiles);
  }
  static const bool debug = [] { const char *e = std::getenv("TFGPU_CSV_DEBUG"); return e && e[0] == '1'; }();
  if (debug && !rowpath) {
    uint32_t g = 0, sl = 0;
    d2h(&g, gen->p, 4); d2h(&sl, slow->p, 4);
    tf::sync();
    std::fprintf(stderr, "tfgpu csv: %s, %lld tiles of %u KiB, %u general pieces; %u lines, %u per-row\n", use_lanes ? "lanes" : "regular", (long long)(use_lanes ? ltiles : rtiles), (use_lanes ? cl_tile(pp.tile_cpt) : tile_bytes) / 1024u, g, nlines, sl);
  }

  for (int s = 0; s < nstr; s++) {
    DColumn &d = db->cols[(size_t)str_col_index[(size_t)s]];
    if (!lens_state) {
      d.data_len = hsum[2 + s];
      d.offsets = subbuf(lens_all, (size_t)s * (size_t)seg_stride * 4, (size_t)(nrows + 1) * 4);
    }
    if (rowpath) continue;
    auto v = std::make_shared<TextView>();
    v->src = src_block ? src_block : nullptr;
    v->fstart = subbuf(fstart_all, ((size_t)s * (size_t)fstride + FS_HDR) * 4, (size_t)std::max<int64_t>(nrows, 1) * 4);
    v->has_special = hsum[2 + nstr + s] != 0;
    v->quote = opts->quote_char; v->jsonnum = d.repr == TFGPU_R_JSONNUM;
    if (lens_state) v->lens = subbuf(lens_all, (size_t)s * (size_t)seg_stride * 4, (size_t)nrows * 4);
    d.view = std::move(v);
  }
  if (nstr && rowpath) {
    std::vector<CopyCol> cc;
    for (int s = 0; s < nstr; s++) {
      DColumn &d = db->cols[(size_t)str_col_index[(size_t)s]];
      d.data = dalloc(d.data_len + 8);
      const CsvCol &hc = cols[(size_t)str_col_index[(size_t)s]];
      cc.push_back(CopyCol{ptr<uint32_t>(d.offsets), hc.fstart, ptr<uint8_t>(d.data), d.repr == TFGPU_R_JSONNUM ? 1 : 0, hc.patch, dp.empty() ? 0u : (uint32_t)dp.size()});
    }
    Buf bcc = up(cc.data(), cc.size() * sizeof(CopyCol));
    if (nrows) {
      CopyParams cp{data, nrows, ptr<CopyCol>(bcc), nstr, opts->quote_char};
      KernelTimer t("csv_copy_strings");
      csv_copy_strings<<<blocks_for(nrows, 256), 256, 0, st>>>(cp);
    }
  } else if (nstr && (!src_block || force_eager)) {
    materialize_from(*db, data);
  }

  for (int i : sys_cols) {
    std::string detail;
    const int rc = fill_system_column(db->cols[(size_t)i], nrows, opts->file_name, opts->row_number_base, nullptr, opts->hide_system_cols, &detail);
    if (rc) return tf::fail(rc, "csv: " + detail);
  }

  std::unique_ptr<tfgpu_dbatch> result;
  int64_t ne = 0;
  if (hnerr) {
    std::vector<uint8_t> he((size_t)nrows); std::vector<int32_t> hc((size_t)nrows);
    d2h(he.data(), err->p, (size_t)nrows); d2h(hc.data(), err_col->p, (size_t)nrows * 4);
    Buf keep = dalloc((size_t)(nrows + 1) * 4);
    csv_keep_from_err<<<blocks_for(nrows, 256), 256, 0, st>>>(ptr<uint8_t>(err), nrows, ptr<uint32_t>(keep));
    tf::sync();
    for (int64_t r = 0; r < nrows; r++)
      if (he[(size_t)r]) { if (errs && ne < errs_cap) errs[ne] = tfgpu_row_error{r, he[(size_t)r], 0, hc[(size_t)r]}; ne++; }
    result = compact_rows(*db, keep);
  } else {
    result = std::move(db);
  }
  uint64_t consumed_raw = last;
  if (decoded) {
    Buf lp = dalloc_zero(4);
    if (raw_len) csv_last_newline<<<blocks_for((int64_t)raw_len, 256), 256, 0, st>>>(raw_data, raw_len, ptr<uint32_t>(lp));
    const uint32_t *h = d2h_u32(lp->p);
    tf::sync();
    consumed_raw = *h;
  }
  if (consumed) *consumed = consumed_raw;
  if (nerrs) *nerrs = ne;
  *out = result.release();
// ... 12 lines not shown
```

transferia_amd/csrc/tf_csv_lanes.inc:

```
static constexpr int CL_THREADS = 1024;
static constexpr int CL_WAVES = CL_THREADS / 64;
static constexpr int CL_CPT_MAX = 3;
static constexpr int CL_BYTES = CL_CPT_MAX * 16 * CL_THREADS;
static constexpr int CL_FCAP = 7168;
static constexpr int CL_RCAP = 512;
static constexpr uint32_t CL_KDUMMY = CL_FCAP + 2;
static constexpr int CL_WCOLS = 16;
static constexpr int CL_MAXCOLS = CL_WAVES * CL_WCOLS;
static_assert(CL_BYTES <= 65536, "positions are 16-bit");
__host__ __device__ constexpr uint32_t cl_staged(uint32_t cpt) { return cpt * 16u * CL_THREADS; }
__host__ __device__ constexpr uint32_t cl_behind(uint32_t cpt) { return cpt * 16u * 64u; }
__host__ __device__ constexpr uint32_t cl_tile(uint32_t cpt) { return cl_staged(cpt) - cl_behind(cpt); }
static_assert(cl_tile(1) % CSV_GRAN == 0, "tiles are whole granules");

struct LaneTile {
  const uint8_t *sb; const uint16_t *fposx; const uint2 *qinfo; const uint2 *keeptab;
  uint32_t g0, quote; bool double_quote;
};
template <class T> __device__ __forceinline__ void lane_store(uint8_t *base, uint32_t byte_off, T v) {
  *reinterpret_cast<T *>(TF_GLOBAL_PTR(uint8_t, base) + (uint64_t)byte_off) = v;
}
__device__ __forceinline__ uint32_t window4(const uint8_t *sb, uint32_t y) {
  const uint32_t *w = reinterpret_cast<const uint32_t *>(sb + (int)((y & ~3u) - 4u));
  return __builtin_amdgcn_alignbyte(w[1], w[0], y);
// ... 365 lines not shown
  const uint32_t NF = misc[2];
  if (NF < 2 || NF < (uint32_t)p.nfields_used || nr * NF > nfe) { give_up(); return; }
  for (uint32_t jj = tid; jj < nr; jj += CL_THREADS) {
    const uint32_t idx = (jj + 1) * NF;
    if (idx > nfe || !((nlbits[idx >> 5] >> (idx & 31)) & 1u)) misc[1] = 1u;
  }

  {
    LaneTile t;
    t.sb = sb; t.fposx = fposx; t.qinfo = qinfo; t.keeptab = keeptab;
    t.g0 = (uint32_t)g0; t.quote = o.quote; t.double_quote = o.double_quote != 0;
    const int32_t row0 = (int32_t)((int64_t)line0 - p.skip_rows);
    uint8_t *const arena = p.arena;
    for (uint32_t jb = 0; jb < nr; jb += 64) {
      const uint32_t jown = jb + (uint32_t)lane;
      const uint64_t am = __ballot(jown < nr && row0 + (int32_t)jown >= 0);
      if (!am) continue;
      const uint32_t jj = ((am >> lane) & 1ull) ? jown : jb + (uint32_t)(__ffsll((long long)am) - 1);
      const uint32_t row = (uint32_t)(row0 + (int32_t)jj), k0 = __umul24(jj, NF);
      uint32_t slow = 0, yprev = 0;
      int fprev = -2;
      for (uint32_t s = 0; s < wave_ncols; s++) {
        const uint32_t o0 = (uint32_t)__builtin_amdgcn_readlane((int)vtab, (int)(4 * s)), o1 = (uint32_t)__builtin_amdgcn_readlane((int)vtab, (int)(4 * s + 1));
        const uint32_t meta = (uint32_t)__builtin_amdgcn_readlane((int)vtab, (int)(4 * s + 2));
        uint8_t *const p0 = arena + ((uint64_t)o0 << 2), *const p1 = arena + ((uint64_t)o1 << 2);
        const int f = (int)(int16_t)(uint16_t)meta, kind = f < 0 ? -1 : (int)((meta >> 16) & 0xFFu), width = (int)(meta >> 24);
        if (CSV_ABL(p) >= 10) {
          const int grp = (kind == CK_INT || kind == CK_UINT) ? 11 : kind == CK_STR ? 12 : 13;
          if (CSV_ABL(p) != grp) continue;
        }
        uint32_t x = yprev, y = 0;
        if (f >= 0) {
          const uint32_t ka = k0 + (uint32_t)f;
          uint32_t kb = ka + 1;
          TF_OPAQUE(kb);
          if (f != fprev + 1) x = fposx[ka];
          y = fposx[kb];
          yprev = y; fprev = f;
        }
        switch (kind) {
          case CK_INT:
            if (width == 1) lane_cells_int<CK_INT, 1>(t, p0, x, y, row, slow); else if (width == 2) lane_cells_int<CK_INT, 2>(t, p0, x, y, row, slow);
            else if (width == 4) lane_cells_int<CK_INT, 4>(t, p0, x, y, row, slow); else lane_cells_int<CK_INT, 8>(t, p0, x, y, row, slow);
            break;
          case CK_UINT:
            if (width == 1) lane_cells_int<CK_UINT, 1>(t, p0, x, y, row, slow); else if (width == 2) lane_cells_int<CK_UINT, 2>(t, p0, x, y, row, slow);
            else if (width == 4) lane_cells_int<CK_UINT, 4>(t, p0, x, y, row, slow); else lane_cells_int<CK_UINT, 8>(t, p0, x, y, row, slow);
            break;
          case CK_STR: lane_cells_str(t, p0, p1, x, y, row, slow); break;
          case CK_DATE: lane_cells_time<CK_DATE>(t, p0, p1, x, y, row, slow); break;
          case CK_TIMESTAMP: lane_cells_time<CK_TIMESTAMP>(t, p0, p1, x, y, row, slow); break;
          default:
            if (kind < 0) {
              CsvCol c{}; c.kind = (int32_t)((meta >> 16) & 0xFFu); c.width = width; c.values = (void *)p0; c.nanos = (int32_t *)p1; c.lens = (uint32_t *)p0; c.fstart = (uint32_t *)p1;
              store_default(c, (int64_t)row);
            } else slow |= 0x80000000u;
        }
      }
      if (slow & 0x80808080u) slowf[jj] = 1;
    }
    if (p.has_unmapped || NF != (uint32_t)p.nfields_used) {
      const uint32_t tot2 = nr * NF;
      const uint32_t inv_nf = 0xFFFFFFFFu / NF + 1;
      for (uint32_t it = tid; it < tot2; it += CL_THREADS) {
        uint32_t jj = __umulhi(it, inv_nf);
        uint32_t f = it - jj * NF;
        if (f >= NF) { jj++; f -= NF; }
        if (row0 + (int32_t)jj < 0) continue;
        if (f < (uint32_t)p.nfields_used && p.field_first[f] >= 0) continue;
        const uint32_t fs = (uint32_t)fposx[it] + 1, fend = fposx[it + 1];
        if (fend > fs && !(starts_plain(sb, fs, fend, sb[fs], o.quote) && ends_plain(sb, fs, fend, sb[fend - 1], o.quote) && quotes_before(t, fend) == quotes_before(t, fs))) slowf[jj] = 1;
      }
    }
  }
  __syncthreads();
  if (misc[1]) { give_up(); return; }
  for (uint32_t jj = tid; jj < nr; jj += CL_THREADS) {
    const int64_t r = (int64_t)line0 + jj - p.skip_rows;
    if (r < 0) continue;
    if (slowf[jj] || p.null_checks) {
      const uint32_t slot = atomicAdd(p.slow_n, 1u);
      p.slow_row[slot] = line0 + jj;
      p.slow_end[slot] = (uint32_t)(g0 + fposx[(jj + 1) * NF]);
    } else p.err[r] = 0;
  }
  if (tid == 0 && line1 == lines_all) atomicMax(p.last_end, (uint32_t)(g0 + fposx[nr * NF] + 1));
}
```

transferia_amd/csrc/tf_rows.hip:

```cpp
#include <chrono>
#include <thread>

#include "tf_rows.hpp"
#include "tf_devrow.hpp"
#include "tf_segcopy.hpp"
#include "tf_textview.hpp"

namespace tf {
__global__ void __launch_bounds__(256) build_selection_kernel(const uint32_t *__restrict__ keep_scan, int64_t n, int32_t *__restrict__ sel) {
  int64_t i = (int64_t)blockIdx.x * blockDim.x + threadIdx.x;
  if (i >= n) return;
  uint32_t a = keep_scan[i], b = keep_scan[i + 1];
  if (a != b) sel[a] = (int32_t)i;
}

struct GFix { const void *in; void *out; int32_t width; int32_t pad; };
template <class T> __device__ __forceinline__ void gather_run(const GFix *__restrict__ a, int lo, int hi, int32_t s, int64_t k) {
  constexpr int U = 8;
  int i = lo;
  for (; i + U <= hi; i += U) {
    T v[U];
#pragma unroll
    for (int q = 0; q < U; q++) v[q] = TF_GLOBAL_PTR(const T, a[i + q].in)[s];
#pragma unroll
// ... 204 lines not shown
  std::vector<DColumn *> cols;
  for (auto &c : b.cols) if (c.lens_only()) cols.push_back(const_cast<DColumn *>(&c));
  for (auto &c : b.old_keys) if (c.lens_only()) cols.push_back(const_cast<DColumn *>(&c));
  if (cols.empty()) return;
  std::lock_guard<std::mutex> tl(g_text_mu);
  const int64_t n = b.nrows;
  std::vector<TextView *> todo;
  for (auto *c : cols) {
    TextView *v = c->view.get();
    if ((int64_t)(v->lens->bytes / 4) != n) throw Error(TFGPU_ERR_INVALID, "internal: text column " + c->name + " holds lengths of another row count");
    if (!v->offsets && std::find(todo.begin(), todo.end(), v) == todo.end()) todo.push_back(v);
  }
  if (!todo.empty() && n == 0) {
    for (auto *v : todo) { v->total = 0; v->offsets = dalloc_zero(16); }
  } else if (!todo.empty()) {
    std::sort(todo.begin(), todo.end(), [](const TextView *x, const TextView *y) { return x->lens->p < y->lens->p; });
    struct Run { size_t first; int nseg; int64_t stride; Buf out; const uint32_t *tot; };
    std::vector<Run> runs;
    const int64_t own_stride = ((n + 1 + 3) / 4) * 4;
    for (size_t i = 0; i < todo.size();) {
      Run r{i, 1, own_stride, nullptr, nullptr};
      if (i + 1 < todo.size()) {
        const int64_t d = ptr<uint32_t>(todo[i + 1]->lens) - ptr<uint32_t>(todo[i]->lens);
        if (d >= n + 1 && d % 4 == 0 && d <= 2 * own_stride + 64) {
          r.stride = d;
          while (r.first + (size_t)r.nseg < todo.size() && ptr<uint32_t>(todo[r.first + (size_t)r.nseg]->lens) - ptr<uint32_t>(todo[r.first + (size_t)r.nseg - 1]->lens) == d) r.nseg++;
        }
      }
      i += (size_t)r.nseg;
      runs.push_back(r);
    }
    for (auto &r : runs) {
      r.out = dalloc((size_t)r.nseg * (size_t)r.stride * 4 + 16);
      exclusive_scan_u32_segments(ptr<uint32_t>(todo[r.first]->lens), ptr<uint32_t>(r.out), n, r.nseg, r.stride);
      r.tot = segment_totals_to_host(ptr<uint32_t>(r.out), n, r.nseg, r.stride);
    }
    sync();
    for (auto &r : runs)
      for (int s = 0; s < r.nseg; s++) {
        TextView *v = todo[r.first + (size_t)s];
        v->total = r.tot[s];
        v->offsets = subbuf(r.out, (size_t)s * (size_t)r.stride * 4, (size_t)(n + 1) * 4);
      }
  }
  for (auto *c : cols) { c->data_len = c->view->total; c->offsets = c->view->offsets; }
}

std::unique_ptr<tfgpu_dbatch> gather_rows(const tfgpu_dbatch &in, const Buf &sel, int64_t m) { return gather_batch(in, sel, m); }

static bool lazy_rows_on() {
  static const bool off = [] { const char *e = std::getenv("TFGPU_LAZY_ROWS"); return e && e[0] == '0'; }();
  return !off;
}
std::unique_ptr<tfgpu_dbatch> compact(const tfgpu_dbatch &in, Buf keep , bool lazy) {
  int64_t n = in.nrows;
  Buf sel = dalloc((size_t)n * 4 + 4);
  const uint32_t *hm;
  if (select_kept_u32(ptr<uint32_t>(keep), n, ptr<int32_t>(sel), ptr<uint32_t>(keep) + n)) hm = d2h_u32(ptr<uint32_t>(keep) + n);
  else {
    exclusive_scan_u32(ptr<uint32_t>(keep), ptr<uint32_t>(keep), n, true);
    hm = d2h_u32(ptr<uint32_t>(keep) + n);
    if (n) build_selection_kernel<<<grid_for(n, 256), 256, 0, ctx().stream>>>(ptr<uint32_t>(keep), n, ptr<int32_t>(sel));
  }
  sync();
  const uint32_t m = *hm;
  if ((int64_t)m == n) return shallow_copy(in);
  if (lazy && lazy_rows_on() && !in.pending && m) {
    auto out = std::make_unique<tfgpu_dbatch>();
    out->nrows = m; out->ns = in.ns; out->table = in.table; out->schema = in.schema; out->key_names = in.key_names;
    auto pr = std::make_shared<PendingRows>();
    pr->src = std::make_shared<const tfgpu_dbatch>(in);
    pr->sel = sel;
    out->pending = std::move(pr);
    return out;
  }
  return gather_batch(in, sel, m);
}

static std::mutex g_dense_mu;
static void dense_hold() {
  static const int ms = [] { const char *e = std::getenv("TFGPU_DENSE_HOLD_MS"); return e ? std::atoi(e) : 0; }();
  if (ms > 0) std::this_thread::sleep_for(std::chrono::milliseconds(ms));
}
static void wait_dense_nolock(const tfgpu_dbatch &b) {
  if (b.dense_done && b.dense_lane != current_lane() && b.dense_gen == lane_generation()) TF_HIP(hipStreamWaitEvent(ctx().stream, (hipEvent_t)b.dense_done, 0));
}
std::unique_ptr<tfgpu_dbatch> snapshot(const tfgpu_dbatch &b) {
  std::unique_ptr<tfgpu_dbatch> c;
  { std::lock_guard<std::mutex> dl(g_dense_mu); c = std::make_unique<tfgpu_dbatch>(b); }
  if (c->pending) dense_hold();
  return c;
}
void dense_locked(const tfgpu_dbatch &b) {
  std::lock_guard<std::mutex> dl(g_dense_mu);
  if (!b.pending) { wait_dense_nolock(b); return; }
  tfgpu_dbatch &mb = const_cast<tfgpu_dbatch &>(b);
  std::shared_ptr<PendingRows> pr = b.pending;
  std::unique_ptr<tfgpu_dbatch> g = gather_batch(*pr->src, pr->sel, b.nrows, b.replaced.empty() ? nullptr : &b.replaced);
  mb.cols = std::move(g->cols); mb.old_keys = std::move(g->old_keys); mb.old_present = g->old_present;
  mb.kind = g->kind; mb.src_row = g->src_row; mb.part_id = g->part_id;
  mb.replaced.clear();
  if (lanes_created() > 1) {
    Context &cx = ctx();
    if (!cx.dense_event) TF_HIP(hipEventCreateWithFlags(&cx.dense_event, hipEventDisableTiming));
    TF_HIP(hipEventRecord(cx.dense_event, cx.stream));
    mb.dense_done = (void *)cx.dense_event;
    mb.dense_lane = current_lane();
    mb.dense_gen = lane_generation();
  }
  mb.pending.reset();
}
bool has_absent(const tfgpu_dbatch &b) {
  std::lock_guard<std::mutex> dl(g_dense_mu);
  if (b.col_order) return true;
  for (auto &c : (b.pending ? b.pending->src->cols : b.cols)) if (c.absent) return true;
  return false;
}
void wait_dense(const tfgpu_dbatch &b) { std::lock_guard<std::mutex> dl(g_dense_mu); wait_dense_nolock(b); }
// ... 48 lines not shown
```

transferia_amd/csrc/tf_rows.hpp:

```cpp
#pragma once
#include "tf_common.hpp"

namespace tf {
std::unique_ptr<tfgpu_dbatch> gather_rows(const tfgpu_dbatch &in, const Buf &sel, int64_t m);
std::unique_ptr<tfgpu_dbatch> compact(const tfgpu_dbatch &in, Buf keep, bool lazy = false);
std::unique_ptr<tfgpu_dbatch> compact_rows(const tfgpu_dbatch &in, Buf keep);
std::unique_ptr<tfgpu_dbatch> partition_rows(const tfgpu_dbatch &in, int nparts, int64_t *counts);
void refuse_absent(const tfgpu_dbatch &b);
void wait_dense(const tfgpu_dbatch &b);
}
```

transferia_amd/csrc/tf_runtime.hip:

```cpp
#include <algorithm>
#include <atomic>
#include <cstdlib>

#include "tf_common.hpp"

namespace tf {

void executor_shutdown();
static thread_local std::string g_last_error;
static constexpr int MAX_LANES = 32;
static std::unique_ptr<Context> g_lanes[MAX_LANES];
static thread_local int g_lane = 0;
static std::vector<int> g_devices;
static std::vector<int> g_device_cus;
static std::mutex g_init_mu;
static std::atomic<int> g_lane_count{0};
static std::atomic<uint64_t> g_generation{1};
uint64_t lane_generation() { return g_generation.load(std::memory_order_acquire); }
static int lane_device_index(int lane) { return g_devices.empty() ? 0 : lane % (int)g_devices.size(); }
#define g_ctx g_lanes[0]

void set_last_error(const std::string &m) { g_last_error = m; }
int fail(int code, const std::string &m) { g_last_error = m; return code; }

static thread_local int t_device = -1;
static void ensure_device(int device) {
  if (t_device == device) return;
  TF_HIP(hipSetDevice(device));
  t_device = device;
}
Context &ctx() {
  if (!g_ctx) throw Error(TFGPU_ERR_DEVICE, "tfgpu_init() has not been called (or no gfx950 device): no CPU fallback exists");
  Context *c = g_lanes[g_lane].get();
  if (!c) throw Error(TFGPU_ERR_INVALID, "this thread is bound to a lane that no longer exists");
  ensure_device(c->device);
  return *c;
}
static std::unique_ptr<Context> make_lane(int lane) {
  auto c = std::make_unique<Context>();
  c->device = g_devices[(size_t)lane_device_index(lane)];
  c->num_cus = g_device_cus[(size_t)lane_device_index(lane)];
  ensure_device(c->device);
  TF_HIP(hipStreamCreateWithFlags(&c->stream, hipStreamNonBlocking));
  c->pin_cap = 8u << 20;
  TF_HIP(hipHostMalloc(&c->pin_base, c->pin_cap, g_devices.size() > 1 ? hipHostMallocPortable : hipHostMallocDefault));
  return c;
}
int bind_lane(int lane) {
  if (lane < 0 || lane >= MAX_LANES) throw Error(TFGPU_ERR_INVALID, "lane out of range");
  std::lock_guard<std::mutex> lk(g_init_mu);
  if (!g_ctx) throw Error(TFGPU_ERR_DEVICE, "tfgpu_init() has not been called");
  if (!g_lanes[lane]) {
    g_lanes[lane] = make_lane(lane);
    g_lane_count.fetch_add(1);
    for (int i = 0; i < MAX_LANES; i++)
      if (i != lane && g_lanes[i]) { ensure_device(g_lanes[i]->device); TF_HIP(hipStreamSynchronize(g_lanes[i]->stream)); }
  }
  ensure_device(g_lanes[lane]->device);
  const int prev = g_lane;
  g_lane = lane;
  return prev;
}
int current_lane() { return g_lane; }
int lane_device(int lane) { return (lane < 0 || g_devices.empty()) ? -1 : g_devices[(size_t)lane_device_index(lane)]; }
static void destroy_lane(std::unique_ptr<Context> &c) {
  if (!c) return;
  t_device = -1;
  hipSetDevice(c->device);
  hipStreamSynchronize(c->stream);
  for (auto &p : c->pending) { hipEventDestroy(p.a); hipEventDestroy(p.b); }
  for (auto e : c->free_events) hipEventDestroy(e);
  if (c->dense_event) hipEventDestroy(c->dense_event);
  c->pow10tab.reset();
  c->consts.clear();
  c->blocks.trim();
  if (c->pin_base) hipHostFree(c->pin_base);
  hipStreamDestroy(c->stream);
  c.reset();
}

hipEvent_t Context::get_event() {
  if (!free_events.empty()) { hipEvent_t e = free_events.back(); free_events.pop_back(); return e; }
  hipEvent_t e;
  TF_HIP(hipEventCreate(&e));
  return e;
}
void Context::prof_begin(const char *name, Pending &p) {
  int idx = -1;
  for (size_t i = 0; i < prof.size(); i++) if (prof[i].name == name) { idx = (int)i; break; }
  if (idx < 0) { prof.push_back(ProfEntry{name, 0, 0, 0}); idx = (int)prof.size() - 1; }
  p.idx = idx; p.a = get_event(); p.b = get_event();
  TF_HIP(hipEventRecord(p.a, stream));
}
void Context::prof_end(Pending &p) {
  hipEventRecord(p.b, stream);
  pending.push_back(p);
  if (pending.size() > 4096) prof_flush();
}
void Context::prof_flush() {
  if (pending.empty()) return;
  hipStreamSynchronize(stream);
  for (auto &p : pending) {
    float ms = 0;
    if (hipEventElapsedTime(&ms, p.a, p.b) == hipSuccess) { prof[p.idx].launches++; prof[p.idx].total_ms += ms; prof[p.idx].units += p.units; }
    free_events.push_back(p.a); free_events.push_back(p.b);
  }
  pending.clear();
}

static inline size_t size_class(size_t n) {
  if (n <= 256) return 256;
  int hi = 63 - __builtin_clzll((unsigned long long)n);
  size_t step = (size_t)1 << (hi > 3 ? hi - 3 : 0);
  return (n + step - 1) & ~(step - 1);
}
void *BlockCache::get(size_t cls) {
  {
    std::lock_guard<std::mutex> lk(mu);
    auto it = free_.find(cls);
    if (it != free_.end() && !it->second.empty()) { void *p = it->second.back(); it->second.pop_back(); cached -= cls; return p; }
  }
  void *p = nullptr;
  hipError_t e = hipMalloc(&p, cls);
  if (e != hipSuccess) {
    (void)hipGetLastError();
    trim();
    e = hipMalloc(&p, cls);
  }
  if (e != hipSuccess) throw Error(TFGPU_ERR_NOMEM, std::string("hipMalloc(") + std::to_string(cls) + "): " + hipGetErrorString(e));
// ... 468 lines not shown
```

transferia_amd/csrc/tf_scan.hip:

```cpp
#include "tf_common.hpp"
#include "tf_wave.hpp"

namespace tf {

static constexpr int SCAN_THREADS = 256;
static constexpr int SCAN_WAVES = SCAN_THREADS / 64;
static constexpr int SCAN_ITEMS = 16;
static constexpr int SCAN_TILE = SCAN_THREADS * SCAN_ITEMS;
static constexpr int64_t RAW_SUMS_MAX = 1024;

__device__ __forceinline__ void scan_load16(const uint32_t *__restrict__ src, int64_t base, int64_t n, bool fast, uint32_t v[SCAN_ITEMS]) {
  if (fast) {
    const uint4 *p = reinterpret_cast<const uint4 *>(src + base);
#pragma unroll
    for (int i = 0; i < SCAN_ITEMS / 4; i++) { uint4 q = p[i]; v[4 * i] = q.x; v[4 * i + 1] = q.y; v[4 * i + 2] = q.z; v[4 * i + 3] = q.w; }
  } else {
#pragma unroll
    for (int i = 0; i < SCAN_ITEMS; i++) v[i] = (base + i < n) ? src[base + i] : 0;
  }
}

__global__ void __launch_bounds__(SCAN_THREADS) scan_reduce_kernel(const uint32_t *__restrict__ in, uint32_t *__restrict__ sums,
                                                                  int64_t n, int64_t seg_stride, int64_t nblocks) {
  __shared__ uint32_t lds[SCAN_WAVES];
  const uint32_t *src = in + (int64_t)blockIdx.y * seg_stride;
  const int lane = threadIdx.x & 63, w = threadIdx.x >> 6;
  const int64_t base = (int64_t)blockIdx.x * SCAN_TILE + (int64_t)threadIdx.x * SCAN_ITEMS;
  uint32_t v[SCAN_ITEMS];
  scan_load16(src, base, n, base + SCAN_ITEMS <= n && ((reinterpret_cast<uintptr_t>(src + base) & 15) == 0), v);
  uint32_t s = 0;
#pragma unroll
  for (int i = 0; i < SCAN_ITEMS; i++) s += v[i];
  s = wave_scan_add(s);
  if (lane == 63) lds[w] = s;
  __syncthreads();
  if (threadIdx.x == 0) {
    uint32_t tot = 0;
#pragma unroll
    for (int i = 0; i < SCAN_WAVES; i++) tot += lds[i];
    sums[(int64_t)blockIdx.y * nblocks + blockIdx.x] = tot;
  }
}

template <bool SELECT>
__global__ void __launch_bounds__(SCAN_THREADS) scan_apply_kernel(const uint32_t *__restrict__ in, uint32_t *__restrict__ out,
                                                                 const uint32_t *__restrict__ block_base, int64_t n,
                                                                 int64_t seg_stride, int64_t nblocks, int write_total, int raw_sums, uint32_t *__restrict__ count) {
  __shared__ uint32_t lds[2][SCAN_WAVES];
  const int lane = threadIdx.x & 63, w = threadIdx.x >> 6;
  const uint32_t *src = in + (int64_t)blockIdx.y * seg_stride;
  uint32_t *dst = out + (int64_t)blockIdx.y * seg_stride;
  const int64_t base = (int64_t)blockIdx.x * SCAN_TILE + (int64_t)threadIdx.x * SCAN_ITEMS;
  uint32_t v[SCAN_ITEMS];
  const bool fast = base + SCAN_ITEMS <= n && ((reinterpret_cast<uintptr_t>(src + base) & 15) == 0);
  scan_load16(src, base, n, fast, v);
  uint32_t part = 0;
  if (block_base) {
    const uint32_t *bs = block_base + (int64_t)blockIdx.y * nblocks;
    if (raw_sums) { for (int64_t i = threadIdx.x; i < (int64_t)blockIdx.x; i += SCAN_THREADS) part += bs[i]; }
    else if (threadIdx.x == 0) part = bs[blockIdx.x];
  }
  uint32_t s = 0;
#pragma unroll
  for (int i = 0; i < SCAN_ITEMS; i++) s += v[i];
  const uint32_t inc = wave_scan_add(s);
  part = wave_scan_add(part);
  if (lane == 63) { lds[0][w] = inc; lds[1][w] = part; }
  __syncthreads();
  uint32_t ex = inc - s;
#pragma unroll
  for (int i = 0; i < SCAN_WAVES; i++) { ex += lds[1][i]; if (i < w) ex += lds[0][i]; }
  if (SELECT) {
#pragma unroll
    for (int i = 0; i < SCAN_ITEMS; i++) { const uint32_t t = v[i]; if (t) out[ex] = (uint32_t)(base + i); ex += t; }
    if (base <= n - 1 && n - 1 < base + SCAN_ITEMS) *count = ex;
    return;
  }
#pragma unroll
  for (int i = 0; i < SCAN_ITEMS; i++) { uint32_t t = v[i]; v[i] = ex; ex += t; }
  if (fast) {
    uint4 *p = reinterpret_cast<uint4 *>(dst + base);
#pragma unroll
    for (int i = 0; i < SCAN_ITEMS / 4; i++) p[i] = make_uint4(v[4 * i], v[4 * i + 1], v[4 * i + 2], v[4 * i + 3]);
  } else {
#pragma unroll
    for (int i = 0; i < SCAN_ITEMS; i++) if (base + i < n) dst[base + i] = v[i];
  }
  if (write_total && base <= n - 1 && n - 1 < base + SCAN_ITEMS) dst[n] = ex;
}

static void scan_impl(const uint32_t *in, uint32_t *out, int64_t n, int64_t seg_stride, int nseg, bool with_total) {
  if (n <= 0) {
    if (with_total) for (int s = 0; s < nseg; s++) TF_HIP(hipMemsetAsync(out + (int64_t)s * seg_stride, 0, 4, ctx().stream));
    return;
  }
  hipStream_t st = ctx().stream;
  int64_t nblocks = (n + SCAN_TILE - 1) / SCAN_TILE;
  dim3 grid((unsigned)nblocks, (unsigned)nseg);
  if (nblocks == 1) {
    scan_apply_kernel<false><<<grid, SCAN_THREADS, 0, st>>>(in, out, nullptr, n, seg_stride, 1, with_total ? 1 : 0, 0, nullptr);
    return;
  }
  Buf sums = dalloc((size_t)nblocks * nseg * 4 + 4);
  scan_reduce_kernel<<<grid, SCAN_THREADS, 0, st>>>(in, ptr<uint32_t>(sums), n, seg_stride, nblocks);
  const bool raw = nblocks <= RAW_SUMS_MAX;
  if (!raw) scan_impl(ptr<uint32_t>(sums), ptr<uint32_t>(sums), nblocks, nblocks, nseg, false);
  scan_apply_kernel<false><<<grid, SCAN_THREADS, 0, st>>>(in, out, ptr<uint32_t>(sums), n, seg_stride, nblocks, with_total ? 1 : 0, raw ? 1 : 0, nullptr);
}

bool select_kept_u32(const uint32_t *keep, int64_t n, int32_t *sel, uint32_t *count) {
  const int64_t nblocks = (n + SCAN_TILE - 1) / SCAN_TILE;
  if (n <= 0 || nblocks > RAW_SUMS_MAX) return false;
  KernelTimer t("scan_u32");
  hipStream_t st = ctx().stream;
  Buf sums;
  if (nblocks > 1) {
    sums = dalloc((size_t)nblocks * 4 + 4);
    scan_reduce_kernel<<<(unsigned)nblocks, SCAN_THREADS, 0, st>>>(keep, ptr<uint32_t>(sums), n, 0, nblocks);
  }
  scan_apply_kernel<true><<<(unsigned)nblocks, SCAN_THREADS, 0, st>>>(keep, reinterpret_cast<uint32_t *>(sel), ptr<uint32_t>(sums), n, 0, nblocks, 0, 1, count);
  return true;
}

__global__ void __launch_bounds__(SCAN_THREADS) sum_u64_kernel(const uint32_t *__restrict__ in, int64_t n, int64_t seg_stride, unsigned long long *totals) {
  const uint32_t *src = in + (int64_t)blockIdx.y * seg_stride;
  unsigned long long s = 0;
  for (int64_t i = (int64_t)blockIdx.x * SCAN_THREADS + threadIdx.x; i < n; i += (int64_t)gridDim.x * SCAN_THREADS) s += src[i];
  for (int d = 32; d; d >>= 1) s += __shfl_down(s, d, 64);
  if ((threadIdx.x & 63) == 0 && s) atomicAdd(totals + blockIdx.y, s);
}

void sum_u32_segments_u64(const uint32_t *in, int64_t seg_len, int nseg, int64_t seg_stride, unsigned long long *totals) {
  if (nseg <= 0 || seg_len <= 0) return;
  const int64_t nb = std::min<int64_t>((seg_len + SCAN_THREADS * 8 - 1) / (SCAN_THREADS * 8), 1024);
  sum_u64_kernel<<<dim3((unsigned)nb, (unsigned)nseg), SCAN_THREADS, 0, ctx().stream>>>(in, seg_len, seg_stride, totals);
}

__global__ void segment_totals_kernel(const uint32_t *lens_all, int64_t seg_stride, int64_t n, int nseg, uint32_t *out) {
  for (int t = threadIdx.x; t < nseg; t += blockDim.x) out[t] = lens_all[(int64_t)t * seg_stride + n];
}
const uint32_t *segment_totals_to_host(const uint32_t *scanned, int64_t seg_len, int nseg, int64_t seg_stride) {
  if (nseg <= 0) return nullptr;
  Buf out = dalloc((size_t)nseg * 4);
  segment_totals_kernel<<<1, 256, 0, ctx().stream>>>(scanned, seg_stride, seg_len, nseg, ptr<uint32_t>(out));
  return d2h_u32(out->p, (size_t)nseg);
}

__global__ void __launch_bounds__(256) any_nonzero_kernel(const uint32_t *v, int64_t n, uint32_t *flag) {
  bool hit = false;
  for (int64_t i = (int64_t)blockIdx.x * 256 + threadIdx.x; i < n; i += (int64_t)gridDim.x * 256) hit |= v[i] != 0;
  if (__ballot(hit) && (threadIdx.x & 63) == 0) atomicOr(flag, 1u);
}
const uint32_t *any_nonzero_to_host(const uint32_t *v, int64_t n) {
  Buf flag = dalloc_zero(4);
  if (n > 0) any_nonzero_kernel<<<(unsigned)std::min<int64_t>((n + 255) / 256, 1024), 256, 0, ctx().stream>>>(v, n, ptr<uint32_t>(flag));
  return d2h_u32(flag->p, 1);
}

void exclusive_scan_u32(const uint32_t *in, uint32_t *out, int64_t n, bool with_total) {
  KernelTimer t("scan_u32");
  scan_impl(in, out, n, 0, 1, with_total);
}

void exclusive_scan_u32_segments(uint32_t *inout, int64_t seg_len, int nseg, int64_t seg_stride) {
  if (nseg <= 0) return;
  KernelTimer t("scan_u32_segments");
  scan_impl(inout, inout, seg_len, seg_stride, nseg, true);
}
void exclusive_scan_u32_segments(const uint32_t *in, uint32_t *out, int64_t seg_len, int nseg, int64_t seg_stride) {
  if (nseg <= 0) return;
  KernelTimer t("scan_u32_segments");
  scan_impl(in, out, seg_len, seg_stride, nseg, true);
}

// ... 2 lines not shown
```

transferia_amd/csrc/tf_transform.hip:

```cpp
#include "tf_plan.hpp"
#include "tf_rows.hpp"
#include "tf_devrow.hpp"

namespace tf {

std::vector<int> chain_sequence(const tfgpu_plan *const *plans, int n, std::vector<std::vector<int>> *hopped) {
  static const bool off = [] { const char *e = std::getenv("TFGPU_CHAIN_REORDER"); return e && e[0] == '0'; }();
  std::vector<int> seq((size_t)n);
  for (int i = 0; i < n; i++) seq[(size_t)i] = i;
  if (hopped) hopped->assign((size_t)n, {});
  if (off) return seq;
  for (int j = 1; j < n; j++) {
    if (plans[seq[(size_t)j]]->kind != PK_FILTER_ROWS) continue;
    const tfgpu_plan &f = *plans[seq[(size_t)j]];
    int k = j;
    std::vector<int> over;
    while (k > 0 && plans[seq[(size_t)k - 1]]->kind == PK_MASK) {
      const tfgpu_plan &m = *plans[seq[(size_t)k - 1]];
      bool reads = false;
      for (auto &e : f.exprs) for (auto &t : e.terms) if (m.mask_has(t.attr)) reads = true;
      if (reads) break;
      over.insert(over.begin(), seq[(size_t)k - 1]);
      std::swap(seq[(size_t)k - 1], seq[(size_t)k]);
      k--;
    }
    if (hopped) (*hopped)[(size_t)k] = over;
  }
  return seq;
}

struct DTerm {
  int32_t col;
  int32_t op, vtype, is_list;
  int32_t nvals;
  int32_t ioff;
  int32_t soff;
};
struct FilterParams {
  const DCol *cols;
  int32_t ncols;
  const DTerm *terms;
  const int32_t *expr_start;
  int32_t nexpr;
  const int64_t *ints;
  const double *floats;
  const uint32_t *str_off;
  const uint8_t *str_data;
  const uint8_t *kind;
  int64_t nrows;
  const uint8_t *const *absent;
  uint32_t *keep;
  uint8_t *err;
  int32_t *err_term;
  uint32_t *nerr;
};

__device__ __forceinline__ int cmp_op_i(int64_t a, int64_t b, int op) {
  switch (op) { case F_EQ: return a == b; case F_NE: return a != b; case F_LT: return a < b; case F_LE: return a <= b; case F_GT: return a > b; case F_GE: return a >= b; }
  return -1;
}
__device__ __forceinline__ int cmp_op_f(double a, double b, int op) {
  switch (op) { case F_EQ: return a == b; case F_NE: return a != b; case F_LT: return a < b; case F_LE: return a <= b; case F_GT: return a > b; case F_GE: return a >= b; }
  return -1;
}
__device__ __forceinline__ bool bytes_contains(const uint8_t *h, uint32_t hn, const uint8_t *n, uint32_t nn) {
  if (nn == 0) return true;
  if (nn > hn) return false;
  for (uint32_t i = 0; i + nn <= hn; i++) {
    uint32_t k = 0;
    while (k < nn && h[i + k] == n[k]) k++;
    if (k == nn) return true;
  }
  return false;
}

__device__ __forceinline__ bool is_dg(uint8_t c) { return c >= '0' && c <= '9'; }
__device__ int parse_time_subset(const uint8_t *s, uint32_t n, int64_t *sec, int32_t *nsec) {
  if (n < 10) return 0;
  if (!(is_dg(s[0]) && is_dg(s[1]) && is_dg(s[2]) && is_dg(s[3]) && s[4] == '-' && is_dg(s[5]) && is_dg(s[6]) && s[7] == '-' && is_dg(s[8]) && is_dg(s[9]))) return 0;
  int64_t y = (s[0] - '0') * 1000 + (s[1] - '0') * 100 + (s[2] - '0') * 10 + (s[3] - '0');
  int mo = (s[5] - '0') * 10 + (s[6] - '0'), d = (s[8] - '0') * 10 + (s[9] - '0');
  int h = 0, mi = 0, se = 0; int64_t ns = 0; int off = 0;
  uint32_t k = 10;
  if (n > 10) {
    if (!(s[10] == 'T' || s[10] == ' ')) return 0;
    bool tform = s[10] == 'T';
    if (n < 19) return 0;
    if (!(is_dg(s[11]) && is_dg(s[12]) && s[13] == ':' && is_dg(s[14]) && is_dg(s[15]) && s[16] == ':' && is_dg(s[17]) && is_dg(s[18]))) return 0;
    h = (s[11] - '0') * 10 + (s[12] - '0'); mi = (s[14] - '0') * 10 + (s[15] - '0'); se = (s[17] - '0') * 10 + (s[18] - '0');
    k = 19;
    if (k + 1 < n && (s[k] == '.' || s[k] == ',') && is_dg(s[k + 1])) {
      k++; int nd = 0;
      while (k < n && is_dg(s[k])) { if (nd < 9) { ns = ns * 10 + (s[k] - '0'); nd++; } k++; }
      while (nd < 9) { ns *= 10; nd++; }
    }
    if (k < n) {
      if (!tform) return 0;
      if (s[k] == 'Z') k++;
      else if ((s[k] == '+' || s[k] == '-') && k + 6 <= n && is_dg(s[k + 1]) && is_dg(s[k + 2]) && s[k + 3] == ':' && is_dg(s[k + 4]) && is_dg(s[k + 5])) {
        int hh = (s[k + 1] - '0') * 10 + (s[k + 2] - '0'), mm = (s[k + 4] - '0') * 10 + (s[k + 5] - '0');
        if (hh > 24 || mm > 60) return 0;
        off = (s[k] == '-' ? -1 : 1) * (hh * 3600 + mm * 60);
        k += 6;
      } else return 0;
      if (k != n) return 0;
    }
  }
// ... 40 lines not shown
        }
        res = cmp_op_f(float1, (double)p.ints[t.ioff], t.op); return res < 0 ? -TFGPU_ROW_TYPE_PAIR : res;
      }
      break;
    case FV_FLOAT:
      if (maybeFloat && !isInt1) return -TFGPU_ROW_HOST_FALLBACK;
      if (isInt1 || isFloat1) {
        double a = isInt1 ? (double)int1 : float1;
        if (is_set) { bool f = false; for (int i = 0; i < t.nvals; i++) f = f || p.floats[t.ioff + i] == a; return t.op == F_IN ? f : !f; }
        res = cmp_op_f(a, p.floats[t.ioff], t.op); return res < 0 ? -TFGPU_ROW_TYPE_PAIR : res;
      }
      break;
    case FV_BOOL:
      if (valid && c.repr == TFGPU_R_BOOL) {
        res = cmp_op_i(((const uint8_t *)c.values)[r] ? 1 : 0, p.ints[t.ioff], t.op); return res < 0 ? -TFGPU_ROW_TYPE_PAIR : res;
      }
      break;
    case FV_STRING:
      if (valid && (c.repr == TFGPU_R_BYTES || c.repr == TFGPU_R_STRING)) {
        const uint8_t *a = c.data + c.offsets[r]; uint32_t an = c.offsets[r + 1] - c.offsets[r];
        const uint32_t *so = p.str_off + t.soff;
        if (t.op == F_MATCH || t.op == F_NOTMATCH) { bool m = bytes_contains(a, an, p.str_data + so[0], so[1] - so[0]); return t.op == F_MATCH ? m : !m; }
        if (is_set) {
          bool f = false;
          for (int i = 0; i < t.nvals; i++) { uint32_t bn = so[i + 1] - so[i]; if (bn == an && bytes_compare(a, an, p.str_data + so[i], bn) == 0) f = true; }
          return t.op == F_IN ? f : !f;
        }
        int cr = bytes_compare(a, an, p.str_data + so[0], so[1] - so[0]);
        res = cmp_op_i(cr, 0, t.op); return res < 0 ? -TFGPU_ROW_TYPE_PAIR : res;
      }
      break;
    case FV_TIME: {
      int64_t us1 = 0; bool have = false;
      if (valid && c.repr == TFGPU_R_TIME) { us1 = ((const int64_t *)c.values)[r] * 1000000 + (c.nanos ? c.nanos[r] : 0) / 1000; have = true; }
      else if (valid && c.repr == TFGPU_R_STRING) {
        int64_t s; int32_t ns;
        if (!parse_time_subset(c.data + c.offsets[r], c.offsets[r + 1] - c.offsets[r], &s, &ns)) return -TFGPU_ROW_HOST_FALLBACK;
        us1 = s * 1000000 + ns / 1000; have = true;
      }
      if (have) {
        if (is_set) { bool f = false; for (int i = 0; i < t.nvals; i++) f = f || p.ints[t.ioff + i] == us1; return t.op == F_IN ? f : !f; }
        res = cmp_op_i(us1, p.ints[t.ioff], t.op); return res < 0 ? -TFGPU_ROW_TYPE_PAIR : res;
      }
      break;
    }
    case FV_NULL:
      if (t.op == F_EQ) return !valid;
      if (t.op == F_NE) return valid;
      break;
  }
  return -TFGPU_ROW_TYPE_PAIR;
}

__global__ void __launch_bounds__(256) filter_eval_kernel(FilterParams p) {
  int64_t r = (int64_t)blockIdx.x * blockDim.x + threadIdx.x;
  if (r >= p.nrows) return;
  int kind = p.kind ? p.kind[r] : TFGPU_K_INSERT;
  uint32_t keep = 0; int err = 0, eterm = -1;
  if (kind == TFGPU_K_UPDATE || kind == TFGPU_K_DELETE) err = TFGPU_ROW_UNSUPPORTED_KIND;
  else if (kind != TFGPU_K_INSERT || p.nexpr < 0) keep = 1;
  else {
    for (int e = 0; e < p.nexpr && !keep && !err; e++) {
      bool ok = true;
      for (int k = p.expr_start[e]; k < p.expr_start[e + 1] && ok && !err; k++) {
        const DTerm &t = p.terms[k];
        if (p.ncols == 0) continue;
        if (p.absent) {
          bool any = false;
          for (int c = 0; c < p.ncols && !any; c++) any = !(p.absent[c] && ((p.absent[c][r >> 3] >> (r & 7)) & 1));
          if (!any) continue;
          if (t.col >= 0 && p.absent[t.col] && ((p.absent[t.col][r >> 3] >> (r & 7)) & 1)) { err = TFGPU_ROW_COLUMN_NOT_FOUND; eterm = k; break; }
        }
        if (t.col < 0) { err = TFGPU_ROW_COLUMN_NOT_FOUND; eterm = k; break; }
        int m = match_value(p, t, r);
        if (m < 0) { err = -m; eterm = k; } else if (!m) ok = false;
      }
      if (!err && ok) keep = 1;
    }
  }
  p.keep[r] = err ? 0 : keep;
  p.err[r] = (uint8_t)err;
  if (err) { p.err_term[r] = eterm; atomicAdd(p.nerr, 1u); }
}

static void collect_row_errors(const Buf &err, const Buf &err_term, int64_t n, ApplyCtx &ax) {
  std::vector<uint8_t> he((size_t)n);
  std::vector<int32_t> ht((size_t)n);
  d2h(he.data(), err->p, (size_t)n);
  if (err_term) d2h(ht.data(), err_term->p, (size_t)n * 4);
  sync();
  for (int64_t r = 0; r < n; r++) if (he[(size_t)r]) ax.errs.push_back(tfgpu_row_error{r, he[(size_t)r], ax.step, err_term ? ht[(size_t)r] : -1});
}

static std::unique_ptr<tfgpu_dbatch> apply_filter_rows(const tfgpu_plan &p, const tfgpu_dbatch &in, ApplyCtx &ax) {
  if (!p.tables.match_table(in.ns, in.table) || is_system_table(in.table)) {
    if (!in.kind) return shallow_copy(in);
  }
  const bool table_applies = p.tables.match_table(in.ns, in.table) && !is_system_table(in.table);
  return run_filter(p.exprs, table_applies, true, in, ax);
}
std::unique_ptr<tfgpu_dbatch> run_filter(const std::vector<FExpr> &p_exprs, bool table_applies, bool check_kinds, const tfgpu_dbatch &in, ApplyCtx &ax) {
  int64_t n = in.nrows;
  hipStream_t st = ctx().stream;
  std::vector<DTerm> terms; std::vector<int32_t> expr_start{0};
  std::vector<int64_t> ints; std::vector<double> floats; std::vector<uint32_t> soff; std::string sdata;
  if (table_applies) {
    for (auto &e : p_exprs) {
      for (auto &t : e.terms) {
        DTerm d{};
        d.col = -1;
        for (size_t i = 0; i < in.cols.size(); i++) if (in.cols[i].name == t.attr) { d.col = (int32_t)i; break; }
        d.op = t.op; d.vtype = t.vtype; d.is_list = t.is_list;
        switch (t.vtype) {
          case FV_FLOAT: d.nvals = (int32_t)t.floats.size(); d.ioff = (int32_t)floats.size(); floats.insert(floats.end(), t.floats.begin(), t.floats.end()); break;
          case FV_STRING:
            d.nvals = (int32_t)t.strs.size(); d.soff = (int32_t)soff.size();
            for (auto &s : t.strs) { soff.push_back((uint32_t)sdata.size()); sdata += s; }
            soff.push_back((uint32_t)sdata.size());
            break;
          default: d.nvals = (int32_t)t.ints.size(); d.ioff = (int32_t)ints.size(); ints.insert(ints.end(), t.ints.begin(), t.ints.end());
        }
        terms.push_back(d);
      }
      expr_start.push_back((int32_t)terms.size());
    }
  }
  {
    std::vector<const DColumn *> need;
    for (auto &t : terms) if (t.col >= 0) need.push_back(&in.cols[(size_t)t.col]);
    materialize(in, &need);
  }
  std::vector<DCol> cols;
  for (auto &c : in.cols) {
    if (c.lazy() || c.lens_only()) { DColumn shell = c; shell.view = nullptr; cols.push_back(dcol_of(shell)); }
    else cols.push_back(dcol_of(c));
  }
  auto up = [&](const void *src, size_t bytes) { return upload_const(src, bytes); };
  Buf bcols = up(cols.data(), cols.size() * sizeof(DCol)), bterms = up(terms.data(), terms.size() * sizeof(DTerm));
  Buf bexpr = up(expr_start.data(), expr_start.size() * 4), bints = up(ints.data(), ints.size() * 8), bfl = up(floats.data(), floats.size() * 8);
  Buf bsoff = up(soff.data(), soff.size() * 4), bsd = up(sdata.data(), sdata.size());
  Buf keep = dalloc((size_t)(n + 1) * 4), err = dalloc((size_t)n + 1), eterm = dalloc((size_t)n * 4 + 4), nerr = dalloc_zero(4);
  FilterParams fp;
  fp.cols = ptr<DCol>(bcols); fp.ncols = (int32_t)cols.size(); fp.terms = ptr<DTerm>(bterms); fp.expr_start = ptr<int32_t>(bexpr);
  fp.nexpr = table_applies ? (int32_t)p_exprs.size() : 0;
  fp.ints = ptr<int64_t>(bints); fp.floats = ptr<double>(bfl); fp.str_off = ptr<uint32_t>(bsoff); fp.str_data = ptr<uint8_t>(bsd);
  fp.absent = nullptr;
  Buf babs;
  {
    std::vector<const uint8_t *> abs;
    bool any = false;
    for (auto &c : in.cols) { abs.push_back(ptr<uint8_t>(c.absent)); any = any || c.absent; }
    if (any) { babs = up(abs.data(), abs.size() * sizeof(const uint8_t *)); fp.absent = reinterpret_cast<const uint8_t *const *>(babs->p); }
  }
  fp.kind = check_kinds ? ptr<uint8_t>(in.kind) : nullptr; fp.nrows = n; fp.keep = ptr<uint32_t>(keep); fp.err = ptr<uint8_t>(err); fp.err_term = ptr<int32_t>(eterm); fp.nerr = ptr<uint32_t>(nerr);
  if (!table_applies) fp.nexpr = -1;
  {
    KernelTimer t("filter_rows_eval");
    if (n) filter_eval_kernel<<<grid_for(n, 256), 256, 0, st>>>(fp);
  }
  const uint32_t *hn = d2h_u32(nerr->p);
  auto out = compact(in, keep, true);
  if (*hn) collect_row_errors(err, eterm, n, ax);
  return out;
}

__global__ void kind_keep_kernel(const uint8_t *kind, int64_t n, uint32_t skip_mask, uint32_t *keep) {
  int64_t r = (int64_t)blockIdx.x * blockDim.x + threadIdx.x;
  if (r < n) keep[r] = ((skip_mask >> kind[r]) & 1u) ? 0u : 1u;
}
static std::unique_ptr<tfgpu_dbatch> apply_skip_events(const tfgpu_plan &p, const tfgpu_dbatch &in) {
  uint32_t mask = (p.skip[0] ? 1u : 0) | (p.skip[1] ? 2u : 0) | (p.skip[2] ? 4u : 0);
  int64_t n = in.nrows;
  if (!in.kind) {
    if (!(mask & 1u)) return shallow_copy(in);
    Buf sel = dalloc(4);
    return gather_rows(in, sel, 0);
  }
  Buf keep = dalloc((size_t)(n + 1) * 4);
  if (n) kind_keep_kernel<<<grid_for(n, 256), 256, 0, ctx().stream>>>(ptr<uint8_t>(in.kind), n, mask, ptr<uint32_t>(keep));
  return compact(in, keep, true);
}

__global__ void __launch_bounds__(256) tostring_len_kernel(DCol c, int64_t n, uint32_t *len, int nil_empty) {
  int64_t r = (int64_t)blockIdx.x * blockDim.x + threadIdx.x;
  if (r >= n) return;
  uint8_t buf[64]; const uint8_t *ext;
  if (nil_empty && c.validity && !((c.validity[r >> 3] >> (r & 7)) & 1)) { len[r] = 0; return; }
  len[r] = (uint32_t)serialize_small(c, r, buf, &ext);
}
__global__ void __launch_bounds__(256) tostring_write_kernel(DCol c, int64_t n, const uint32_t *off, uint8_t *data, int nil_empty) {
  int64_t r = (int64_t)blockIdx.x * blockDim.x + threadIdx.x;
  if (r >= n) return;
  uint8_t buf[64]; const uint8_t *ext;
  if (nil_empty && c.validity && !((c.validity[r >> 3] >> (r & 7)) & 1)) return;
  int len = serialize_small(c, r, buf, &ext);
  uint8_t *dst = data + off[r];
  const uint8_t *src = ext ? ext : buf;
  struct __attribute__((packed, aligned(1))) U64 { uint64_t v; };
  int i = 0;
  for (; i + 8 <= len; i += 8) reinterpret_cast<U64 *>(dst + i)->v = reinterpret_cast<const U64 *>(src + i)->v;
  for (; i < len; i++) dst[i] = src[i];
}

DColumn column_to_string(const DColumn &c, int64_t n, bool to_bytes, int max_len_hint, int nil_empty) {
  hipStream_t st = ctx().stream;
  DColumn o;
  o.name = c.name; o.dtype = to_bytes ? TFGPU_T_BYTES : TFGPU_T_UTF8; o.repr = to_bytes ? TFGPU_R_BYTES : TFGPU_R_STRING;
  o.offsets = dalloc((size_t)(n + 1) * 4);
  DCol dc = dcol_of(c);
  KernelTimer t("to_string");
  if (n) tostring_len_kernel<<<grid_for(n, 256), 256, 0, st>>>(dc, n, ptr<uint32_t>(o.offsets), nil_empty);
  exclusive_scan_u32(ptr<uint32_t>(o.offsets), ptr<uint32_t>(o.offsets), n, true);
  uint64_t cap = repr_is_var(c.repr) ? c.data_len + (uint64_t)n * 5 : (uint64_t)n * (uint64_t)max_len_hint;
  o.data = dalloc(cap);
  if (n) tostring_write_kernel<<<grid_for(n, 256), 256, 0, st>>>(dc, n, ptr<uint32_t>(o.offsets), ptr<uint8_t>(o.data), nil_empty);
// ... 302 lines not shown
```

Measured before the change: 1.038 billion rows/s.

## Fold CSV control flags and filter error counts into pinned readbacks and fused scans

```diff
diff --git a/transferia_amd/csrc/tf_common.hpp b/transferia_amd/csrc/tf_common.hpp
--- a/transferia_amd/csrc/tf_common.hpp
+++ b/transferia_amd/csrc/tf_common.hpp
@@ -75,6 +75,7 @@
   void trim();
 };
 
+#define TF_CSV_CTL_BYTES 2048
 struct Context {
   int device = -1;
   hipStream_t stream = nullptr;
@@ -98,6 +99,9 @@
   uint64_t const_clock = 0;
   double csv_hint_bpl = 0.0;
   int csv_hint_ncols = -1;
+  void *csv_ctl = nullptr;
+  int csv_ctl_set = 0;
+  bool csv_ctl_dirty = false;
 
   hipEvent_t get_event();
   void prof_begin(const char *name, Pending &p);
@@ -238,6 +242,9 @@
 void exclusive_scan_u32_segments(uint32_t *inout, int64_t seg_len, int nseg, int64_t seg_stride);
 void exclusive_scan_u32_segments(const uint32_t *in, uint32_t *out, int64_t seg_len, int nseg, int64_t seg_stride);
 bool select_kept_u32(const uint32_t *keep, int64_t n, int32_t *sel, uint32_t *count);
+static constexpr int KEPT_TOTALS_ROWS = 256;
+bool kept_totals_fit(int64_t n);
+void select_kept_totals_u32(const uint32_t *keep, int64_t n, int32_t *sel, const uint32_t *totals, uint32_t *host_pair);
 const uint32_t *any_nonzero_to_host(const uint32_t *v, int64_t n);
 const uint32_t *segment_totals_to_host(const uint32_t *scanned, int64_t seg_len, int nseg, int64_t seg_stride);
 void sum_u32_segments_u64(const uint32_t *in, int64_t seg_len, int nseg, int64_t seg_stride, unsigned long long *totals);
diff --git a/transferia_amd/csrc/tf_csv.hip b/transferia_amd/csrc/tf_csv.hip
--- a/transferia_amd/csrc/tf_csv.hip
+++ b/transferia_amd/csrc/tf_csv.hip
@@ -150,6 +150,7 @@
   uint32_t dp_len;
   uint32_t multiline;
   const uint64_t *p128;
+  uint32_t *flag_base;
 };
 
 __device__ __forceinline__ bool any_quote(const uint32_t *qmask, uint32_t lo, uint32_t hi) {
@@ -210,6 +211,8 @@
   int32_t *nanos;
   uint32_t *lens;
   uint32_t *fstart;
+  uint32_t *flag;
+  int64_t tpos;
   uint32_t *patch;
 };
 static constexpr uint32_t PATCH_NONE = 0xFFFFFFFFu;
@@ -267,7 +270,15 @@
   uint32_t *spec;
   uint32_t cap_lines;
   uint32_t *ovf;
+  uint32_t *ctl;
+  uint32_t *ctl_other;
+  uint32_t *colflags;
+  uint32_t *ctl_sum;
+  const uint32_t *lines_total;
 };
+enum CsvCtl : int { CTL_SLOW_N = 0, CTL_LAST_END, CTL_GEN_N, CTL_OVF, CTL_FLAGS, CTL_SET_WORDS = CTL_FLAGS + 128 };
+enum CsvSum : int { SUM_NERR = 0 , SUM_LAST, SUM_LINES, SUM_OVF, SUM_FLAGS };
+static_assert(2 * CTL_SET_WORDS * 4 <= TF_CSV_CTL_BYTES, "Context::csv_ctl holds both sets");
 
 static constexpr uint32_t SP_AGG = 1u << 30, SP_INC = 2u << 30, SP_VAL = (1u << 30) - 1u;
 __device__ __forceinline__ uint32_t spec_lookback(uint32_t *state, int64_t t, uint32_t own, int lane) {
@@ -295,10 +306,11 @@
 __device__ __forceinline__ StrictOut strict_out(const CsvCol &c, int32_t kind) { return StrictOut{kind, c.width, c.lo, c.hi, c.values, c.nanos}; }
 __device__ __forceinline__ void store_int(const CsvCol &c, int64_t r, int64_t v) { store_int(strict_out(c, c.kind), r, v); }
 
-__device__ __forceinline__ void store_default(const CsvCol &c, int64_t r) {
+__device__ __forceinline__ uint32_t *col_flag(const CsvOpts &o, const CsvCol &c) { return o.flag_base ? o.flag_base + c.tpos : c.flag; }
+__device__ __forceinline__ void store_default(const CsvCol &c, int64_t r, uint32_t *flag) {
   switch (c.kind) {
     case CK_SYS: break;
-    case CK_STR: case CK_JSONNUM: c.lens[r] = (c.kind == CK_JSONNUM) ? 1u : 0u; c.fstart[r] = 0x7FFFFFFFu; if (c.kind == CK_JSONNUM) c.fstart[-1] = 1u; break;
+    case CK_STR: case CK_JSONNUM: c.lens[r] = (c.kind == CK_JSONNUM) ? 1u : 0u; c.fstart[r] = 0x7FFFFFFFu; if (c.kind == CK_JSONNUM) *flag = 1u; break;
     case CK_DATE: case CK_TIMESTAMP: store_default(strict_out(c, SK_TIME), r); break;
     default: store_default(strict_out(c, c.kind), r);
   }
@@ -347,7 +359,7 @@
 __device__ int parse_cell(const CsvOpts &o, const CsvCol &c, int64_t r, const F &fv, uint32_t a, uint32_t b, uint32_t npairs, uint64_t abs_start) {
   switch (c.kind) {
     case CK_INT: case CK_UINT: case CK_INTERVAL:
-      if (cell_is_null(o, fv, a, b, npairs)) { store_default(c, r); return 0; }
+      if (cell_is_null(o, fv, a, b, npairs)) { store_default(c, r, col_flag(o, c)); return 0; }
       if (npairs) return TFGPU_ROW_CAST;
       return strict_cell(strict_out(c, c.kind), o.cast_tp, o.p128, r, fv, a, b);
     case CK_STR: case CK_JSONNUM: {
@@ -375,7 +387,7 @@
       if (c.kind == CK_JSONNUM && (npairs || !json_number_ok(fv, a, b))) return TFGPU_ROW_CAST;
       c.lens[r] = (b - a) - npairs;
       c.fstart[r] = (uint32_t)(abs_start + a) | (npairs ? 0x80000000u : 0u);
-      if (npairs) c.fstart[-1] = 1u;
+      if (npairs) *col_flag(o, c) = 1u;
       return 0;
     }
     case CK_DATE: case CK_TIMESTAMP: {
@@ -466,7 +478,7 @@
       const CsvCol &c = p.cols[ci];
       if (!have_row || rerr) continue;
       if (!has_field) {
-        if (o.include_missing) store_default(c, r); else if (ci < miss_col) miss_col = ci;
+        if (o.include_missing) store_default(c, r, col_flag(o, c)); else if (ci < miss_col) miss_col = ci;
         continue;
       }
       int err = parse_cell(o, c, r, fv, a, b, npairs, fs);
@@ -478,10 +490,10 @@
   if (!rerr) {
     for (int32_t ci = 0; ci < p.ncols; ci++) {
       const CsvCol &c = p.cols[ci];
-      if (c.field < 0) { store_default(c, r); continue; }
+      if (c.field < 0) { store_default(c, r, col_flag(o, c)); continue; }
       if (c.field >= nfields) {
         if (c.field < p.nfields_used && !nil_line) continue;
-        if (o.include_missing) store_default(c, r); else { if (ci < miss_col) miss_col = ci; break; }
+        if (o.include_missing) store_default(c, r, col_flag(o, c)); else { if (ci < miss_col) miss_col = ci; break; }
       }
     }
   }
@@ -489,7 +501,7 @@
   if (!err && miss_col != 0x7FFFFFFF) { err = TFGPU_ROW_MISSING_CELL; err_col = miss_col; }
   if (!err && cerr) { err = cerr; err_col = cerr_col; }
   p.err[r] = (uint8_t)err;
-  if (err) { p.err_col[r] = err_col; atomicAdd(p.nerr, 1u); }
+  if (err) { p.err_col[r] = err_col; if (p.ctl_sum) p.ctl_sum[SUM_NERR] = 1u; else atomicAdd(p.nerr, 1u); }
 }
 
 __global__ void __launch_bounds__(256) csv_parse_rows(CsvParams p) {
@@ -500,6 +512,14 @@
 
 __global__ void __launch_bounds__(64) csv_parse_listed(CsvParams p) {
   const uint32_t n = *p.slow_n;
+  if (p.ctl && blockIdx.x == 0) {
+    const int i = threadIdx.x;
+    if (i == SUM_LAST) p.ctl_sum[SUM_LAST] = p.ctl[CTL_LAST_END];
+    if (i == SUM_LINES) p.ctl_sum[SUM_LINES] = *p.lines_total;
+    if (i == SUM_OVF && p.ctl[CTL_OVF]) p.ctl_sum[SUM_OVF] = 1u;
+    for (int c = i; c < p.ncols; c += 64) if (p.colflags[c]) p.ctl_sum[SUM_FLAGS + c] = 1u;
+    for (int w = i; w < CTL_SET_WORDS; w += 64) p.ctl_other[w] = 0;
+  }
   for (uint64_t base = (uint64_t)blockIdx.x * 64; base < n; base += (uint64_t)gridDim.x * 64) {
     const uint64_t i = base + threadIdx.x;
     const int64_t line = i < n ? (int64_t)p.slow_row[i] : -1;
@@ -845,7 +865,8 @@
         if (tc.field < 0 || (uint32_t)tc.field >= nf) {
           if (tc.field < 0 || o.include_missing) {
             CsvCol c{}; c.kind = tc.kind; c.width = tc.width; c.values = tc.p0; c.nanos = (int32_t *)tc.p1; c.lens = (uint32_t *)tc.p0; c.fstart = (uint32_t *)tc.p1;
-            store_default(c, r);
+            c.flag = p.colflags ? p.colflags + oi : (uint32_t *)tc.p1 - 1;
+            store_default(c, r, c.flag);
           } else slowf[jj] = 1;
           continue;
         }
@@ -874,7 +895,7 @@
               if (!(npairs && !o.double_quote)) {
                 ((uint32_t *)tc.p0)[r] = (b - a) - npairs;
                 ((uint32_t *)tc.p1)[r] = (uint32_t)(g0 + a) | (npairs ? 0x80000000u : 0u);
-                if (npairs) ((uint32_t *)tc.p1)[-1] = 1u;
+                if (npairs) *(p.colflags ? p.colflags + oi : (uint32_t *)tc.p1 - 1) = 1u;
                 done = true;
               }
             }
@@ -997,12 +1018,13 @@
 #endif
 static constexpr int CR_FCAP = TF_CR_FCAP;
 static constexpr int CR_LCOLS = 128;
+static_assert(CTL_SET_WORDS - CTL_FLAGS >= CR_LCOLS, "a set of the control block holds a flag word for every column the tile parser stages");
 static constexpr uint32_t CR_KDUMMY = CR_FCAP + 2;
 struct CsvRun { int32_t kind, width, first, ncols; };
 struct CsvTask { int32_t kind, width, first, ncols; };
 
 struct RegTile {
-  const uint8_t *sb; const uint16_t *fposx; const uint32_t *qmask; const uint16_t *qpre; const uint2 *keeptab; uint8_t *slowf; const uint64_t *colp0, *colp1; const uint16_t *colfield;
+  const uint8_t *sb; const uint16_t *fposx; const uint32_t *qmask; const uint16_t *qpre; const uint2 *keeptab; uint8_t *slowf; const uint64_t *colp0, *colp1; const uint16_t *colfield; uint32_t *colflags;
   uint32_t nr, NF, step_q, step_r; float inv_nr; int32_t row0; uint32_t g0; uint32_t quote; bool double_quote; int32_t ablate; int32_t col_mode;
 };
 struct RegCell { bool on; uint32_t col, jj, fs, fend; int32_t r; };
@@ -1131,7 +1153,7 @@
   for_slots(t, run, sbase, wv, lane, [&](const RegCell &c) { reg_int_body<KIND, W, T>(t, c, global_ptr<T>(t.colp0[c.on ? c.col : (uint32_t)run.first])); });
 }
 
-__device__ __forceinline__ void reg_str_body(const RegTile &t, const RegCell &c, uint32_t *const lens, uint32_t *const fstart) {
+__device__ __forceinline__ void reg_str_body(const RegTile &t, const RegCell &c, uint32_t *const lens, uint32_t *const fstart, const uint32_t col) {
   const uint32_t n = c.fend - c.fs;
   const uint32_t c_first = t.sb[c.fs], c_last = t.sb[c.fend - 1];
   const uint32_t qn = quotes_in(t, c.fs, c.fend);
@@ -1155,7 +1177,7 @@
       if (!(npairs && !t.double_quote)) {
         lens[c.r] = (b - a) - npairs;
         fstart[c.r] = (t.g0 + a) | (npairs ? 0x80000000u : 0u);
-        if (npairs) fstart[-1] = 1u;
+        if (npairs) *(t.colflags ? t.colflags + col : fstart - 1) = 1u;
         done = true;
       }
     }
@@ -1165,7 +1187,7 @@
 __device__ __forceinline__ void reg_cells_str(const RegTile &t, const CsvRun &run, uint32_t sbase, int wv, int lane) {
   for_slots(t, run, sbase, wv, lane, [&](const RegCell &c) {
     const uint32_t col = c.on ? c.col : (uint32_t)run.first;
-    reg_str_body(t, c, global_ptr<uint32_t>(t.colp0[col]), global_ptr<uint32_t>(t.colp1[col]));
+    reg_str_body(t, c, global_ptr<uint32_t>(t.colp0[col]), global_ptr<uint32_t>(t.colp1[col]), col);
   });
 }
 
@@ -1258,7 +1280,7 @@
   const uint32_t col = (uint32_t)k.first + (lc.live ? lc.g : 0u);
   const uint32_t colfield = t.colfield[col];
   uint32_t *const lens = global_ptr<uint32_t>(t.colp0[col]), *const fstart = global_ptr<uint32_t>(t.colp1[col]);
-  for (uint32_t jj0 = 0; jj0 < t.nr; jj0 += lc.P) reg_str_body(t, lane_cell(t, lc, jj0, colfield), lens, fstart);
+  for (uint32_t jj0 = 0; jj0 < t.nr; jj0 += lc.P) reg_str_body(t, lane_cell(t, lc, jj0, colfield), lens, fstart, col);
 }
 template <int KIND> __device__ __forceinline__ void task_cells_time(const RegTile &t, const CsvTask &k, int lane) {
   const LaneCol lc = lane_col(k, lane, t.col_mode);
@@ -1490,7 +1512,7 @@
 
   {
     RegTile t;
-    t.sb = sb; t.fposx = fposx; t.qmask = qmask; t.qpre = qpre; t.keeptab = keeptab; t.slowf = slowf; t.colp0 = colp0; t.colp1 = colp1; t.colfield = colfield;
+    t.sb = sb; t.fposx = fposx; t.qmask = qmask; t.qpre = qpre; t.keeptab = keeptab; t.slowf = slowf; t.colp0 = colp0; t.colp1 = colp1; t.colfield = colfield; t.colflags = p.colflags;
     t.nr = nr; t.NF = NF; t.step_q = 64u * CT_WAVES / nr; t.step_r = 64u * CT_WAVES - t.step_q * nr; t.inv_nr = __uint_as_float(__float_as_uint(1.0f / (float)nr) - 2u);
     t.row0 = (int32_t)((int64_t)line0 - p.skip_rows); t.g0 = (uint32_t)g0; t.quote = o.quote; t.double_quote = o.double_quote != 0; t.ablate = CSV_ABL(p); t.col_mode = p.col_lanes;
     if constexpr (COLS) {
@@ -1546,7 +1568,8 @@
             if (run.kind < 0) {
               const TCol tc = p.tcols[run.first + oi];
               CsvCol c{}; c.kind = tc.kind; c.width = tc.width; c.values = tc.p0; c.nanos = (int32_t *)tc.p1; c.lens = (uint32_t *)tc.p0; c.fstart = (uint32_t *)tc.p1;
-              store_default(c, r);
+              c.flag = p.colflags ? p.colflags + run.first + oi : (uint32_t *)tc.p1 - 1;
+              store_default(c, r, c.flag);
             } else slowf[jj] = 1;
           }
       }
@@ -1868,6 +1891,7 @@
     if (!g.sht.empty()) { CopyParams cp{g.src, nrows, ptr<CopyCol>(bsht), (int32_t)g.sht.size(), g.quote}; csv_copy_cells<<<dim3((unsigned)((nrows + 255) / 256), (unsigned)((g.sht.size() + CC_GROUP - 1) / CC_GROUP)), 256, 0, st>>>(cp); }
     if (!g.all.empty()) {
       CopyParams cp{g.src, nrows, ptr<CopyCol>(ball), (int32_t)g.all.size(), g.quote};
+      KernelTimer ts("csv_copy_special");
       csv_copy_special<<<dim3((unsigned)((nrows + 255) / 256), (unsigned)g.all.size()), 256, 0, st>>>(cp);
     }
   }
@@ -2138,6 +2162,30 @@
     cols[(size_t)i].next = field_first[(size_t)f];
     field_first[(size_t)f] = i;
   }
+  std::vector<int32_t> order((size_t)ncols);
+  for (int i = 0; i < ncols; i++) order[(size_t)i] = i;
+  std::stable_sort(order.begin(), order.end(), [&](int x, int y) {
+    const CsvCol &a = cols[(size_t)x], &b = cols[(size_t)y];
+    return a.kind != b.kind ? a.kind < b.kind : a.width != b.width ? a.width < b.width : a.field < b.field;
+  });
+  Buf src_block = staged ? staged : find_device_block(data);
+  static const bool ctl_blockers = [] {
+    for (const char *n : {"TFGPU_CSV_ABLATE", "TFGPU_CSV_PHASES", "TFGPU_CSV_LANES", "TFGPU_CSV_COL_LANES", "TFGPU_CSV_DEBUG", "TFGPU_CSV_EAGER", "TFGPU_CSV_SCAN_EAGER"}) { const char *e = std::getenv(n); if (e && e[0] && e[0] != '0') return true; }
+    return false;
+  }();
+  const bool use_ctl = !rowpath && !spec && !ctl_blockers && src_block && nlines > 0 && ncols <= CR_LCOLS && cx.csv_ctl;
+  if (use_ctl) cx.csv_ctl_set ^= 1;
+  uint32_t *const ctl = use_ctl ? static_cast<uint32_t *>(cx.csv_ctl) + cx.csv_ctl_set * CTL_SET_WORDS : nullptr;
+  uint32_t *const ctl_sum = use_ctl ? cx.pin_n<uint32_t>((size_t)(SUM_FLAGS + ncols)) : nullptr;
+  if (use_ctl && !ctl_sum) throw Error(TFGPU_ERR_NOMEM, "pinned read-back arena exhausted");
+  if (use_ctl) std::memset(ctl_sum, 0, (size_t)(SUM_FLAGS + ncols) * 4);
+  std::vector<int32_t> tpos((size_t)ncols, 0);
+  for (int i = 0; i < ncols; i++) {
+    CsvCol &c = cols[(size_t)order[(size_t)i]];
+    tpos[(size_t)order[(size_t)i]] = i;
+    c.tpos = i;
+    if ((c.kind == CK_STR || c.kind == CK_JSONNUM) && !ctl) c.flag = c.fstart - 1;
+  }
   std::vector<uint32_t> loff{0}; std::string ldata;
   auto add_list = [&](int n, const char *const *v) { for (int i = 0; i < n; i++) { ldata += v[i] ? v[i] : ""; loff.push_back((uint32_t)ldata.size()); } };
   add_list(opts->n_null_values, opts->null_values); add_list(opts->n_true_values, opts->true_values); add_list(opts->n_false_values, opts->false_values);
@@ -2183,7 +2231,7 @@
   pp.o.user_tp = GtSet{ptr<GtOp>(bgops), ptr<uint8_t>(bglits), ptr<uint16_t>(bgsu), opts->n_timestamp_parsers};
   pp.o.cast_tp = GtSet{ptr<GtOp>(bgops), ptr<uint8_t>(bglits), ptr<uint16_t>(bgsc), N_CAST_LAYOUTS};
   pp.o.dp = ptr<uint8_t>(bdp); pp.o.dp_len = (uint32_t)dp.size(); pp.o.multiline = multiline ? 1u : 0u;
-  pp.o.p128 = nullptr;
+  pp.o.p128 = nullptr; pp.o.flag_base = use_ctl ? ctl_sum + SUM_FLAGS : nullptr;
   for (auto &c : cols) if (c.kind == CK_F32) pp.o.p128 = reinterpret_cast<const uint64_t *>(pow10_table() + 632);
   pp.cols = ptr<CsvCol>(bcols); pp.ncols = ncols; pp.field_first = ptr<int32_t>(bff); pp.nfields_used = max_field + 1;
   pp.err = ptr<uint8_t>(err); pp.err_col = ptr<int32_t>(err_col); pp.nerr = ptr<uint32_t>(nerr);
@@ -2197,16 +2245,19 @@
   pp.gen_n = ptr<uint32_t>(gen); pp.gen_tile = ptr<uint32_t>(gen) + 1; pp.force_general = force_general ? 1 : 0;
   pp.spec = spec ? ptr<uint32_t>(spec_state) : nullptr; pp.cap_lines = cap_lines;
   Buf ahead_ovf;
-  if (ahead) { ahead_ovf = dalloc(4); pp.ovf = ptr<uint32_t>(ahead_ovf); }
-  csv_zero_flags<<<1, 64, 0, st>>>(ptr<uint32_t>(fstart_all), fstride, nstr, ptr<uint32_t>(slow), ptr<uint32_t>(gen), ptr<uint32_t>(nerr), pp.ovf);
+  if (use_ctl) {
+    pp.slow_n = ctl + CTL_SLOW_N; pp.last_end = ctl + CTL_LAST_END; pp.gen_n = ctl + CTL_GEN_N; pp.nerr = nullptr;
+    if (ahead) pp.ovf = ctl + CTL_OVF;
+    pp.ctl = ctl; pp.ctl_other = static_cast<uint32_t *>(cx.csv_ctl) + (cx.csv_ctl_set ^ 1) * CTL_SET_WORDS;
+    pp.colflags = ctl + CTL_FLAGS; pp.lines_total = ptr<uint32_t>(tile_counts) + ngran; pp.ctl_sum = ctl_sum;
+    if (cx.csv_ctl_dirty) TF_HIP(hipMemsetAsync(cx.csv_ctl, 0, 2 * CTL_SET_WORDS * 4, st));
+    cx.csv_ctl_dirty = true;
+  } else {
+    if (ahead) { ahead_ovf = dalloc(4); pp.ovf = ptr<uint32_t>(ahead_ovf); }
+    csv_zero_flags<<<1, 64, 0, st>>>(ptr<uint32_t>(fstart_all), fstride, nstr, ptr<uint32_t>(slow), ptr<uint32_t>(gen), ptr<uint32_t>(nerr), pp.ovf);
+  }
   pp.has_unmapped = 0;
   for (int f = 0; f <= max_field; f++) if (field_first[(size_t)f] < 0) pp.has_unmapped = 1;
-  std::vector<int32_t> order((size_t)ncols);
-  for (int i = 0; i < ncols; i++) order[(size_t)i] = i;
-  std::stable_sort(order.begin(), order.end(), [&](int x, int y) {
-    const CsvCol &a = cols[(size_t)x], &b = cols[(size_t)y];
-    return a.kind != b.kind ? a.kind < b.kind : a.width != b.width ? a.width < b.width : a.field < b.field;
-  });
   std::vector<TCol> tcols((size_t)ncols);
   for (int i = 0; i < ncols; i++) {
     const CsvCol &c = cols[(size_t)order[(size_t)i]];
@@ -2321,7 +2372,6 @@
     { KernelTimer t("csv_parse_tiles_general"); csv_parse_tiles_general<<<(unsigned)std::min<int64_t>(ntiles + rtiles, 2048), CT_THREADS, 0, st>>>(pp); }
     { KernelTimer t("csv_parse_listed"); csv_parse_listed<<<(unsigned)std::min<int64_t>(blocks_for(slow_cap, 64), 1024), 64, 0, st>>>(pp); }
   }
-  Buf src_block = staged ? staged : find_device_block(data);
   static const bool force_eager = [] { const char *e = std::getenv("TFGPU_CSV_EAGER"); return e && e[0] == '1'; }();
   static const bool scan_eager = [] { const char *e = std::getenv("TFGPU_CSV_SCAN_EAGER"); return e && e[0] == '1'; }();
   const bool lens_state = !rowpath && src_block && !force_eager && !scan_eager;
@@ -2332,15 +2382,19 @@
   } else if (nstr) {
     TF_HIP(hipMemsetAsync(lens_all->p, 0, (size_t)nstr * (size_t)seg_stride * 4, st));
   }
-  Buf summary = dalloc((size_t)(2 * nstr + 4) * 4);
-  csv_collect<<<1, 64, 0, st>>>(ptr<uint32_t>(nerr), rowpath ? ptr<uint32_t>(row_start) + nlines : pp.last_end, lens_state ? nullptr : ptr<uint32_t>(lens_all),
-                                seg_stride, nrows, nstr, ptr<uint32_t>(fstart_all), fstride, ptr<uint32_t>(summary), pp.spec, rtiles, skip,
-                                ptr<uint32_t>(tile_counts) + (spec ? 0 : ngran), pp.ovf);
-  const uint32_t *hsum = d2h_u32(summary->p, (size_t)(2 * nstr) + 4);
+  const uint32_t *hsum = pp.ctl_sum;
+  if (!use_ctl) {
+    Buf summary = dalloc((size_t)(2 * nstr + 4) * 4);
+    csv_collect<<<1, 64, 0, st>>>(ptr<uint32_t>(nerr), rowpath ? ptr<uint32_t>(row_start) + nlines : pp.last_end, lens_state ? nullptr : ptr<uint32_t>(lens_all),
+                                  seg_stride, nrows, nstr, ptr<uint32_t>(fstart_all), fstride, ptr<uint32_t>(summary), pp.spec, rtiles, skip,
+                                  ptr<uint32_t>(tile_counts) + (spec ? 0 : ngran), pp.ovf);
+    hsum = d2h_u32(summary->p, (size_t)(2 * nstr) + 4);
+  }
   tf::sync();
-  const uint32_t hnerr = hsum[0], last = hsum[1];
+  if (use_ctl) cx.csv_ctl_dirty = false;
+  const uint32_t hnerr = use_ctl ? hsum[SUM_NERR] : hsum[0], last = use_ctl ? hsum[SUM_LAST] : hsum[1];
   if (spec || ahead) {
-    const uint32_t nl_true = hsum[2 + 2 * nstr], overflow = hsum[3 + 2 * nstr];
+    const uint32_t nl_true = use_ctl ? hsum[SUM_LINES] : hsum[2 + 2 * nstr], overflow = use_ctl ? hsum[SUM_OVF] : hsum[3 + 2 * nstr];
     if (overflow || nl_true > cap_lines || (int64_t)nl_true < skip || (nl_true && !last)) { *retry = true; return TFGPU_OK; }
     nlines = nl_true; nlogical = nl_true; nrows = (int64_t)nl_true - skip;
     db->nrows = nrows;
@@ -2369,7 +2423,7 @@
     auto v = std::make_shared<TextView>();
     v->src = src_block ? src_block : nullptr;
     v->fstart = subbuf(fstart_all, ((size_t)s * (size_t)fstride + FS_HDR) * 4, (size_t)std::max<int64_t>(nrows, 1) * 4);
-    v->has_special = hsum[2 + nstr + s] != 0;
+    v->has_special = (use_ctl ? hsum[SUM_FLAGS + tpos[(size_t)str_col_index[(size_t)s]]] : hsum[2 + nstr + s]) != 0;
     v->quote = opts->quote_char; v->jsonnum = d.repr == TFGPU_R_JSONNUM;
     if (lens_state) v->lens = subbuf(lens_all, (size_t)s * (size_t)seg_stride * 4, (size_t)nrows * 4);
     d.view = std::move(v);
diff --git a/transferia_amd/csrc/tf_csv_lanes.inc b/transferia_amd/csrc/tf_csv_lanes.inc
--- a/transferia_amd/csrc/tf_csv_lanes.inc
+++ b/transferia_amd/csrc/tf_csv_lanes.inc
@@ -441,8 +441,8 @@
           case CK_TIMESTAMP: lane_cells_time<CK_TIMESTAMP>(t, p0, p1, x, y, row, slow); break;
           default:
             if (kind < 0) {
-              CsvCol c{}; c.kind = (int32_t)((meta >> 16) & 0xFFu); c.width = width; c.values = (void *)p0; c.nanos = (int32_t *)p1; c.lens = (uint32_t *)p0; c.fstart = (uint32_t *)p1;
-              store_default(c, (int64_t)row);
+              CsvCol c{}; c.kind = (int32_t)((meta >> 16) & 0xFFu); c.width = width; c.values = (void *)p0; c.nanos = (int32_t *)p1; c.lens = (uint32_t *)p0; c.fstart = (uint32_t *)p1; c.flag = (uint32_t *)p1 - 1;
+              store_default(c, (int64_t)row, c.flag);
             } else slow |= 0x80000000u;
         }
       }
diff --git a/transferia_amd/csrc/tf_rows.hip b/transferia_amd/csrc/tf_rows.hip
--- a/transferia_amd/csrc/tf_rows.hip
+++ b/transferia_amd/csrc/tf_rows.hip
@@ -280,18 +280,25 @@
   static const bool off = [] { const char *e = std::getenv("TFGPU_LAZY_ROWS"); return e && e[0] == '0'; }();
   return !off;
 }
-std::unique_ptr<tfgpu_dbatch> compact(const tfgpu_dbatch &in, Buf keep , bool lazy) {
+std::unique_ptr<tfgpu_dbatch> compact(const tfgpu_dbatch &in, Buf keep , bool lazy) { return compact(in, keep, lazy, nullptr, nullptr); }
+std::unique_ptr<tfgpu_dbatch> compact(const tfgpu_dbatch &in, Buf keep , bool lazy, const Buf &totals, uint32_t *failed) {
   int64_t n = in.nrows;
   Buf sel = dalloc((size_t)n * 4 + 4);
   const uint32_t *hm;
-  if (select_kept_u32(ptr<uint32_t>(keep), n, ptr<int32_t>(sel), ptr<uint32_t>(keep) + n)) hm = d2h_u32(ptr<uint32_t>(keep) + n);
+  if (totals) {
+    uint32_t *pair = ctx().pin_n<uint32_t>(2);
+    if (!pair) throw Error(TFGPU_ERR_NOMEM, "pinned read-back arena exhausted");
+    select_kept_totals_u32(ptr<uint32_t>(keep), n, ptr<int32_t>(sel), ptr<uint32_t>(totals), pair);
+    hm = pair;
+  } else if (select_kept_u32(ptr<uint32_t>(keep), n, ptr<int32_t>(sel), ptr<uint32_t>(keep) + n)) hm = d2h_u32(ptr<uint32_t>(keep) + n);
   else {
     exclusive_scan_u32(ptr<uint32_t>(keep), ptr<uint32_t>(keep), n, true);
     hm = d2h_u32(ptr<uint32_t>(keep) + n);
     if (n) build_selection_kernel<<<grid_for(n, 256), 256, 0, ctx().stream>>>(ptr<uint32_t>(keep), n, ptr<int32_t>(sel));
   }
   sync();
-  const uint32_t m = *hm;
+  const uint32_t m = hm[0];
+  if (totals && failed) *failed = hm[1];
   if ((int64_t)m == n) return shallow_copy(in);
   if (lazy && lazy_rows_on() && !in.pending && m) {
     auto out = std::make_unique<tfgpu_dbatch>();
diff --git a/transferia_amd/csrc/tf_rows.hpp b/transferia_amd/csrc/tf_rows.hpp
--- a/transferia_amd/csrc/tf_rows.hpp
+++ b/transferia_amd/csrc/tf_rows.hpp
@@ -4,6 +4,7 @@
 namespace tf {
 std::unique_ptr<tfgpu_dbatch> gather_rows(const tfgpu_dbatch &in, const Buf &sel, int64_t m);
 std::unique_ptr<tfgpu_dbatch> compact(const tfgpu_dbatch &in, Buf keep, bool lazy = false);
+std::unique_ptr<tfgpu_dbatch> compact(const tfgpu_dbatch &in, Buf keep, bool lazy, const Buf &totals, uint32_t *failed);
 std::unique_ptr<tfgpu_dbatch> compact_rows(const tfgpu_dbatch &in, Buf keep);
 std::unique_ptr<tfgpu_dbatch> partition_rows(const tfgpu_dbatch &in, int nparts, int64_t *counts);
 void refuse_absent(const tfgpu_dbatch &b);
diff --git a/transferia_amd/csrc/tf_runtime.hip b/transferia_amd/csrc/tf_runtime.hip
--- a/transferia_amd/csrc/tf_runtime.hip
+++ b/transferia_amd/csrc/tf_runtime.hip
@@ -44,6 +44,8 @@
   TF_HIP(hipStreamCreateWithFlags(&c->stream, hipStreamNonBlocking));
   c->pin_cap = 8u << 20;
   TF_HIP(hipHostMalloc(&c->pin_base, c->pin_cap, g_devices.size() > 1 ? hipHostMallocPortable : hipHostMallocDefault));
+  TF_HIP(hipMalloc(&c->csv_ctl, TF_CSV_CTL_BYTES));
+  TF_HIP(hipMemsetAsync(c->csv_ctl, 0, TF_CSV_CTL_BYTES, c->stream));
   return c;
 }
 int bind_lane(int lane) {
@@ -75,6 +77,7 @@
   c->consts.clear();
   c->blocks.trim();
   if (c->pin_base) hipHostFree(c->pin_base);
+  if (c->csv_ctl) hipFree(c->csv_ctl);
   hipStreamDestroy(c->stream);
   c.reset();
 }
diff --git a/transferia_amd/csrc/tf_scan.hip b/transferia_amd/csrc/tf_scan.hip
--- a/transferia_amd/csrc/tf_scan.hip
+++ b/transferia_amd/csrc/tf_scan.hip
@@ -45,8 +45,9 @@
 template <bool SELECT>
 __global__ void __launch_bounds__(SCAN_THREADS) scan_apply_kernel(const uint32_t *__restrict__ in, uint32_t *__restrict__ out,
                                                                  const uint32_t *__restrict__ block_base, int64_t n,
-                                                                 int64_t seg_stride, int64_t nblocks, int write_total, int raw_sums, uint32_t *__restrict__ count) {
-  __shared__ uint32_t lds[2][SCAN_WAVES];
+                                                                 int64_t seg_stride, int64_t nblocks, int write_total, int raw_sums, uint32_t *__restrict__ count,
+                                                                 const uint32_t *__restrict__ extra, int64_t nextra) {
+  __shared__ uint32_t lds[SELECT ? 3 : 2][SCAN_WAVES];
   const int lane = threadIdx.x & 63, w = threadIdx.x >> 6;
   const uint32_t *src = in + (int64_t)blockIdx.y * seg_stride;
   uint32_t *dst = out + (int64_t)blockIdx.y * seg_stride;
@@ -57,23 +58,35 @@
   uint32_t part = 0;
   if (block_base) {
     const uint32_t *bs = block_base + (int64_t)blockIdx.y * nblocks;
-    if (raw_sums) { for (int64_t i = threadIdx.x; i < (int64_t)blockIdx.x; i += SCAN_THREADS) part += bs[i]; }
+    if (raw_sums) { for (int64_t i = threadIdx.x; i < (int64_t)blockIdx.x * raw_sums; i += SCAN_THREADS) part += bs[i]; }
     else if (threadIdx.x == 0) part = bs[blockIdx.x];
   }
+  uint32_t epart = 0;
+  const bool sum_extra = SELECT && extra && (int64_t)blockIdx.x == nblocks - 1;
+  if (sum_extra) { for (int64_t i = threadIdx.x; i < nextra; i += SCAN_THREADS) epart += extra[i]; epart = wave_scan_add(epart); }
   uint32_t s = 0;
 #pragma unroll
   for (int i = 0; i < SCAN_ITEMS; i++) s += v[i];
   const uint32_t inc = wave_scan_add(s);
   part = wave_scan_add(part);
-  if (lane == 63) { lds[0][w] = inc; lds[1][w] = part; }
+  if (lane == 63) { lds[0][w] = inc; lds[1][w] = part; if constexpr (SELECT) lds[2][w] = epart; }
   __syncthreads();
   uint32_t ex = inc - s;
 #pragma unroll
   for (int i = 0; i < SCAN_WAVES; i++) { ex += lds[1][i]; if (i < w) ex += lds[0][i]; }
-  if (SELECT) {
+  if constexpr (SELECT) {
 #pragma unroll
     for (int i = 0; i < SCAN_ITEMS; i++) { const uint32_t t = v[i]; if (t) out[ex] = (uint32_t)(base + i); ex += t; }
-    if (base <= n - 1 && n - 1 < base + SCAN_ITEMS) *count = ex;
+    if (base <= n - 1 && n - 1 < base + SCAN_ITEMS) {
+      count[0] = ex;
+      if (extra) {
+        uint32_t e = 0;
+#pragma unroll
+        for (int i = 0; i < SCAN_WAVES; i++) e += lds[2][i];
+        count[1] = e;
+        __threadfence_system();
+      }
+    }
     return;
   }
 #pragma unroll
@@ -98,14 +111,14 @@
   int64_t nblocks = (n + SCAN_TILE - 1) / SCAN_TILE;
   dim3 grid((unsigned)nblocks, (unsigned)nseg);
   if (nblocks == 1) {
-    scan_apply_kernel<false><<<grid, SCAN_THREADS, 0, st>>>(in, out, nullptr, n, seg_stride, 1, with_total ? 1 : 0, 0, nullptr);
+    scan_apply_kernel<false><<<grid, SCAN_THREADS, 0, st>>>(in, out, nullptr, n, seg_stride, 1, with_total ? 1 : 0, 0, nullptr, nullptr, 0);
     return;
   }
   Buf sums = dalloc((size_t)nblocks * nseg * 4 + 4);
   scan_reduce_kernel<<<grid, SCAN_THREADS, 0, st>>>(in, ptr<uint32_t>(sums), n, seg_stride, nblocks);
   const bool raw = nblocks <= RAW_SUMS_MAX;
   if (!raw) scan_impl(ptr<uint32_t>(sums), ptr<uint32_t>(sums), nblocks, nblocks, nseg, false);
-  scan_apply_kernel<false><<<grid, SCAN_THREADS, 0, st>>>(in, out, ptr<uint32_t>(sums), n, seg_stride, nblocks, with_total ? 1 : 0, raw ? 1 : 0, nullptr);
+  scan_apply_kernel<false><<<grid, SCAN_THREADS, 0, st>>>(in, out, ptr<uint32_t>(sums), n, seg_stride, nblocks, with_total ? 1 : 0, raw ? 1 : 0, nullptr, nullptr, 0);
 }
 
 bool select_kept_u32(const uint32_t *keep, int64_t n, int32_t *sel, uint32_t *count) {
@@ -118,8 +131,15 @@
     sums = dalloc((size_t)nblocks * 4 + 4);
     scan_reduce_kernel<<<(unsigned)nblocks, SCAN_THREADS, 0, st>>>(keep, ptr<uint32_t>(sums), n, 0, nblocks);
   }
-  scan_apply_kernel<true><<<(unsigned)nblocks, SCAN_THREADS, 0, st>>>(keep, reinterpret_cast<uint32_t *>(sel), ptr<uint32_t>(sums), n, 0, nblocks, 0, 1, count);
+  scan_apply_kernel<true><<<(unsigned)nblocks, SCAN_THREADS, 0, st>>>(keep, reinterpret_cast<uint32_t *>(sel), ptr<uint32_t>(sums), n, 0, nblocks, 0, 1, count, nullptr, 0);
   return true;
+}
+bool kept_totals_fit(int64_t n) { return n > 0 && (n + SCAN_TILE - 1) / SCAN_TILE <= RAW_SUMS_MAX; }
+void select_kept_totals_u32(const uint32_t *keep, int64_t n, int32_t *sel, const uint32_t *totals, uint32_t *host_pair) {
+  static_assert(SCAN_TILE % KEPT_TOTALS_ROWS == 0, "a scan block is a whole number of the producer's workgroups");
+  const int64_t nblocks = (n + SCAN_TILE - 1) / SCAN_TILE, nt = (n + KEPT_TOTALS_ROWS - 1) / KEPT_TOTALS_ROWS;
+  KernelTimer t("scan_u32");
+  scan_apply_kernel<true><<<(unsigned)nblocks, SCAN_THREADS, 0, ctx().stream>>>(keep, reinterpret_cast<uint32_t *>(sel), totals, n, 0, nblocks, 0, SCAN_TILE / KEPT_TOTALS_ROWS, host_pair, totals + nt, nt);
 }
 
 __global__ void __launch_bounds__(SCAN_THREADS) sum_u64_kernel(const uint32_t *__restrict__ in, int64_t n, int64_t seg_stride, unsigned long long *totals) {
diff --git a/transferia_amd/csrc/tf_transform.hip b/transferia_amd/csrc/tf_transform.hip
--- a/transferia_amd/csrc/tf_transform.hip
+++ b/transferia_amd/csrc/tf_transform.hip
@@ -1,6 +1,7 @@
 #include "tf_plan.hpp"
 #include "tf_rows.hpp"
 #include "tf_devrow.hpp"
+#include "tf_wave.hpp"
 
 namespace tf {
 
@@ -53,6 +54,7 @@
   uint8_t *err;
   int32_t *err_term;
   uint32_t *nerr;
+  uint32_t *totals;
 };
 
 __device__ __forceinline__ int cmp_op_i(int64_t a, int64_t b, int op) {
@@ -199,9 +201,7 @@
   return -TFGPU_ROW_TYPE_PAIR;
 }
 
-__global__ void __launch_bounds__(256) filter_eval_kernel(FilterParams p) {
-  int64_t r = (int64_t)blockIdx.x * blockDim.x + threadIdx.x;
-  if (r >= p.nrows) return;
+__device__ __forceinline__ uint32_t filter_eval_row(const FilterParams &p, int64_t r) {
   int kind = p.kind ? p.kind[r] : TFGPU_K_INSERT;
   uint32_t keep = 0; int err = 0, eterm = -1;
   if (kind == TFGPU_K_UPDATE || kind == TFGPU_K_DELETE) err = TFGPU_ROW_UNSUPPORTED_KIND;
@@ -227,7 +227,25 @@
   }
   p.keep[r] = err ? 0 : keep;
   p.err[r] = (uint8_t)err;
-  if (err) { p.err_term[r] = eterm; atomicAdd(p.nerr, 1u); }
+  if (err) p.err_term[r] = eterm;
+  return err ? 1u << 16 : keep;
+}
+static constexpr int FE_THREADS = KEPT_TOTALS_ROWS;
+__global__ void __launch_bounds__(FE_THREADS) filter_eval_kernel(FilterParams p) {
+  __shared__ uint32_t wsum[FE_THREADS / 64];
+  const int64_t r = (int64_t)blockIdx.x * FE_THREADS + threadIdx.x;
+  uint32_t cnt = r < p.nrows ? filter_eval_row(p, r) : 0u;
+  if (!p.totals) { if (cnt >> 16) atomicAdd(p.nerr, cnt >> 16); return; }
+  cnt = wave_scan_add(cnt);
+  if ((threadIdx.x & 63) == 63) wsum[threadIdx.x >> 6] = cnt;
+  __syncthreads();
+  if (threadIdx.x == 0) {
+    uint32_t t = 0;
+#pragma unroll
+    for (int i = 0; i < FE_THREADS / 64; i++) t += wsum[i];
+    p.totals[blockIdx.x] = t & 0xFFFFu;
+    p.totals[gridDim.x + blockIdx.x] = t >> 16;
+  }
 }
 
 static void collect_row_errors(const Buf &err, const Buf &err_term, int64_t n, ApplyCtx &ax) {
@@ -286,7 +304,10 @@
   Buf bcols = up(cols.data(), cols.size() * sizeof(DCol)), bterms = up(terms.data(), terms.size() * sizeof(DTerm));
   Buf bexpr = up(expr_start.data(), expr_start.size() * 4), bints = up(ints.data(), ints.size() * 8), bfl = up(floats.data(), floats.size() * 8);
   Buf bsoff = up(soff.data(), soff.size() * 4), bsd = up(sdata.data(), sdata.size());
-  Buf keep = dalloc((size_t)(n + 1) * 4), err = dalloc((size_t)n + 1), eterm = dalloc((size_t)n * 4 + 4), nerr = dalloc_zero(4);
+  Buf keep = dalloc((size_t)(n + 1) * 4), err = dalloc((size_t)n + 1), eterm = dalloc((size_t)n * 4 + 4);
+  const bool with_totals = kept_totals_fit(n);
+  const unsigned groups = (unsigned)((n + KEPT_TOTALS_ROWS - 1) / KEPT_TOTALS_ROWS);
+  Buf totals = with_totals ? dalloc((size_t)groups * 8) : nullptr, nerr = with_totals ? nullptr : dalloc_zero(4);
   FilterParams fp;
   fp.cols = ptr<DCol>(bcols); fp.ncols = (int32_t)cols.size(); fp.terms = ptr<DTerm>(bterms); fp.expr_start = ptr<int32_t>(bexpr);
   fp.nexpr = table_applies ? (int32_t)p_exprs.size() : 0;
@@ -299,15 +320,21 @@
     for (auto &c : in.cols) { abs.push_back(ptr<uint8_t>(c.absent)); any = any || c.absent; }
     if (any) { babs = up(abs.data(), abs.size() * sizeof(const uint8_t *)); fp.absent = reinterpret_cast<const uint8_t *const *>(babs->p); }
   }
-  fp.kind = check_kinds ? ptr<uint8_t>(in.kind) : nullptr; fp.nrows = n; fp.keep = ptr<uint32_t>(keep); fp.err = ptr<uint8_t>(err); fp.err_term = ptr<int32_t>(eterm); fp.nerr = ptr<uint32_t>(nerr);
+  fp.kind = check_kinds ? ptr<uint8_t>(in.kind) : nullptr; fp.nrows = n; fp.keep = ptr<uint32_t>(keep); fp.err = ptr<uint8_t>(err); fp.err_term = ptr<int32_t>(eterm); fp.nerr = ptr<uint32_t>(nerr); fp.totals = ptr<uint32_t>(totals);
   if (!table_applies) fp.nexpr = -1;
   {
     KernelTimer t("filter_rows_eval");
-    if (n) filter_eval_kernel<<<grid_for(n, 256), 256, 0, st>>>(fp);
-  }
-  const uint32_t *hn = d2h_u32(nerr->p);
-  auto out = compact(in, keep, true);
-  if (*hn) collect_row_errors(err, eterm, n, ax);
+    if (n) filter_eval_kernel<<<groups, FE_THREADS, 0, st>>>(fp);
+  }
+  uint32_t failed = 0;
+  std::unique_ptr<tfgpu_dbatch> out;
+  if (with_totals) out = compact(in, keep, true, totals, &failed);
+  else {
+    const uint32_t *hn = d2h_u32(nerr->p);
+    out = compact(in, keep, true);
+    failed = *hn;
+  }
+  if (failed) collect_row_errors(err, eterm, n, ax);
   return out;
 }
 
```

Result: faster. 1.065 billion rows/s, median of 6 (+2.6%).
